# kenahm/se3-icp

Measured on AMD Instinct MI355X. Metric: ICP iterations/sec + pairs/sec, ~120k-pt KITTI clouds, 1/2/4/8 GPU, higher is better.
Workload: dtype f32 sweep + f64 certify/solve

## Files before the change

include/se3icp.h:

```cpp
#ifndef SE3ICP_H
#define SE3ICP_H

#include <stdint.h>

#ifdef __cplusplus
extern "C" {
#endif

#define SE3ICP_ABI_VERSION 4

typedef enum se3icp_status {
    SE3ICP_OK = 0,
    SE3ICP_ERR_INVALID_ARG = -1,
    SE3ICP_ERR_INVALID_METHOD = -2,
    SE3ICP_ERR_EMPTY_CLOUD = -3,
    SE3ICP_ERR_K_TOO_LARGE = -4,
    SE3ICP_ERR_NO_DEVICE = -5,
    SE3ICP_ERR_HIP = -6,
    SE3ICP_ERR_NONFINITE = -7,
    SE3ICP_ERR_OUT_OF_MEMORY = -8,
    SE3ICP_ERR_INTERNAL = -9
} se3icp_status;

typedef enum se3icp_method {
    SE3ICP_PT2PT = 0,
    SE3ICP_PT2PL = 1,
    SE3ICP_GICP = 2,
    SE3ICP_SE3_PT2PT = 3,
    SE3ICP_SE3_PT2PL = 4,
    SE3ICP_SE3_GICP = 5,
    SE3ICP_SE3_GICP_WITH_CF = 6,
    SE3ICP_SE3_PURE_PT2PT = 7,
    SE3ICP_SE3_PURE_PT2PL = 8,
    SE3ICP_SE3_PURE_GICP = 9,
    SE3ICP_NUM_METHODS = 10
} se3icp_method;

typedef struct se3icp_params {
    int32_t max_num_iterations;
    int32_t max_num_se3_iterations;
    int32_t number_of_nn_for_LRF;
    int32_t _reserved;
    double mse;
    double mse_switch_error;
    double estimated_overlap;
    double alpha_rot;
    double beta_transl;
    double scale_preprocessing;
} se3icp_params;

typedef struct se3icp_result {
    double T[16];
    int32_t num_iterations;
    int32_t num_pure_se3_iterations;
    int32_t status;
    int32_t num_rechecked;
    double scaling_factor;
    double time_setup_ms;
    double time_loop_ms;
    double time_se3_correspondence_search_ms;
    double time_before_pure_icp_ms;
} se3icp_result;

int se3icp_abi_version(void);
const char* se3icp_status_string(int status);
int se3icp_method_from_name(const char* name);
const char* se3icp_method_name(int method);
void se3icp_default_params(se3icp_params* p);
int se3icp_device_count(void);

typedef struct se3icp_registration se3icp_registration;

se3icp_registration* se3icp_registration_new(void);
void se3icp_registration_free(se3icp_registration* r);
int se3icp_set_source_cloud(se3icp_registration* r, const double* xyz, int64_t n);
int se3icp_set_target_cloud(se3icp_registration* r, const double* xyz, int64_t n);
se3icp_params* se3icp_params_of(se3icp_registration* r);
int se3icp_run_icp(se3icp_registration* r, const char* variant);
int se3icp_run_se3_icp(se3icp_registration* r, const char* variant);
int se3icp_run_se3_icp_with_cf(se3icp_registration* r);
int se3icp_run_se3_pure(se3icp_registration* r, const char* variant);
int se3icp_get_result(const se3icp_registration* r, se3icp_result* out);

int se3icp_register_batch(int device, int32_t n_pairs, const double* const* src_xyz, const int64_t* n_src,
                          const double* const* tgt_xyz, const int64_t* n_tgt, int method,
                          const se3icp_params* params, se3icp_result* results);

int se3icp_register_batch_device(int device, int32_t n_pairs, const double* d_src_xyz, const int64_t* src_off,
                                 const double* d_tgt_xyz, const int64_t* tgt_off, int method,
                                 const se3icp_params* params, se3icp_result* results, void* hip_stream);

int se3icp_register_sweep(int device, int32_t n_pairs, const double* const* src_xyz, const int64_t* n_src,
                          const double* const* tgt_xyz, const int64_t* n_tgt, int method, int32_t n_variants,
                          const se3icp_params* variants, int32_t max_group, se3icp_result* results);
int se3icp_register_sweep_device(int device, int32_t n_pairs, const double* d_src_xyz, const int64_t* src_off,
                                 const double* d_tgt_xyz, const int64_t* tgt_off, int method, int32_t n_variants,
                                 const se3icp_params* variants, int32_t max_group, se3icp_result* results,
                                 void* hip_stream);

int se3icp_register_graph(int device, int32_t n_clouds, const double* const* xyz, const int64_t* n_pts,
                          int32_t n_pairs, const int32_t* src_cloud, const int32_t* tgt_cloud, int method,
                          const se3icp_params* params, int32_t sharing, se3icp_result* results);
int se3icp_register_graph_device(int device, int32_t n_clouds, const double* d_xyz, const int64_t* off,
                                 int32_t n_pairs, const int32_t* src_cloud, const int32_t* tgt_cloud, int method,
                                 const se3icp_params* params, int32_t sharing, se3icp_result* results,
                                 void* hip_stream);
struct se3icp_report_options;
struct se3icp_report;
int se3icp_register_graph_report(int device, int32_t n_clouds, const double* const* xyz, const int64_t* n_pts,
                                 int32_t n_pairs, const int32_t* src_cloud, const int32_t* tgt_cloud, int method,
                                 const se3icp_params* params, int32_t sharing, se3icp_result* results,
                                 const struct se3icp_report_options* opts, struct se3icp_report* reports);
int se3icp_register_graph_report_device(int device, int32_t n_clouds, const double* d_xyz, const int64_t* off,
                                        int32_t n_pairs, const int32_t* src_cloud, const int32_t* tgt_cloud,
                                        int method, const se3icp_params* params, int32_t sharing,
                                        se3icp_result* results, void* hip_stream,
                                        const struct se3icp_report_options* opts, struct se3icp_report* reports);
#define SE3ICP_GRAPH_STATS_N 9
int se3icp_last_graph_stats(int device, int64_t* out, int n);

int se3icp_set_batch_sharing(int device, int level);

int se3icp_set_lrf_seeding(int device, int mode);
#define SE3ICP_SEED_STATS_N 4
int se3icp_last_seed_stats(int device, int64_t* out, int n);

int se3icp_set_tree_sharing(int device, int mode);
#define SE3ICP_TREE_STATS_N 4
int se3icp_last_tree_stats(int device, int64_t* out, int n);

typedef enum se3icp_stop_reason {
    SE3ICP_STOP_CONVERGED = 0,
    SE3ICP_STOP_MAX_ITERATIONS = 1,
    SE3ICP_STOP_MAX_SE3_ITERATIONS = 2,
    SE3ICP_STOP_RUNAWAY = 3
} se3icp_stop_reason;

typedef struct se3icp_report_options {
    double max_correspondence_distance;
    int32_t* corr_idx;
    double* corr_dist;
    int32_t outputs_on_device;
    int32_t _reserved;
} se3icp_report_options;

typedef struct se3icp_report {
    double fitness;
    double inlier_rmse;
    double information[36];
    double final_mse;
    double final_mse_change;
    int64_t n_inliers;
    int32_t switched;
    int32_t stop_reason;
} se3icp_report;

int se3icp_report_version(void);

int se3icp_register_batch_report(int device, int32_t n_pairs, const double* const* src_xyz, const int64_t* n_src,
                                 const double* const* tgt_xyz, const int64_t* n_tgt, int method,
                                 const se3icp_params* params, se3icp_result* results,
                                 const se3icp_report_options* opts, se3icp_report* reports);
int se3icp_register_batch_report_device(int device, int32_t n_pairs, const double* d_src_xyz, const int64_t* src_off,
                                        const double* d_tgt_xyz, const int64_t* tgt_off, int method,
                                        const se3icp_params* params, se3icp_result* results, void* hip_stream,
                                        const se3icp_report_options* opts, se3icp_report* reports);
int se3icp_register_sweep_report(int device, int32_t n_pairs, const double* const* src_xyz, const int64_t* n_src,
                                 const double* const* tgt_xyz, const int64_t* n_tgt, int method, int32_t n_variants,
                                 const se3icp_params* variants, int32_t max_group, se3icp_result* results,
                                 const se3icp_report_options* opts, se3icp_report* reports);
int se3icp_register_sweep_report_device(int device, int32_t n_pairs, const double* d_src_xyz, const int64_t* src_off,
                                        const double* d_tgt_xyz, const int64_t* tgt_off, int method,
                                        int32_t n_variants, const se3icp_params* variants, int32_t max_group,
                                        se3icp_result* results, void* hip_stream,
                                        const se3icp_report_options* opts, se3icp_report* reports);
int se3icp_request_report(se3icp_registration* r, const se3icp_report_options* opts);
int se3icp_get_report(const se3icp_registration* r, se3icp_report* out);

int se3icp_init_version(void);
int se3icp_register_graph_init(int device, int32_t n_clouds, const double* const* xyz, const int64_t* n_pts,
                               int32_t n_pairs, const int32_t* src_cloud, const int32_t* tgt_cloud,
                               const double* T_init , int method,
                               const se3icp_params* params, int32_t sharing, se3icp_result* results,
                               const se3icp_report_options* opts, se3icp_report* reports);
int se3icp_register_graph_init_device(int device, int32_t n_clouds, const double* d_xyz, const int64_t* off,
                                      int32_t n_pairs, const int32_t* src_cloud, const int32_t* tgt_cloud,
                                      const double* T_init , int method,
                                      const se3icp_params* params, int32_t sharing, se3icp_result* results,
                                      void* hip_stream, const se3icp_report_options* opts, se3icp_report* reports);
int se3icp_set_initial_transform(se3icp_registration* r, const double* T);
int se3icp_set_pose_seeding(int device, int mode);
#define SE3ICP_INIT_STATS_N 3
int se3icp_last_init_stats(int device, int64_t* out, int n);
int se3icp_transform_points(const double* T, const double* xyz, int64_t n, double* out);
int se3icp_transform_device(int device, int32_t n_clouds, const double* d_xyz, const int64_t* off, const double* T,
                            double* d_out, void* hip_stream);

int se3icp_register(int device, const double* src_xyz, int64_t n_src, const double* tgt_xyz, int64_t n_tgt,
                    int method, const se3icp_params* params, se3icp_result* result);


int se3icp_toldi_frames(int device, const double* xyz, int64_t n, int k, double* frames);
int se3icp_knn_self(int device, const double* xyz, int64_t n, int k, int32_t* idx);
int se3icp_estimate_normals(int device, const double* xyz, int64_t n, int k, double* normals);
int se3icp_nn(int device, const double* query, int64_t nq, const double* data, int64_t nd, int dim,
              int32_t* idx, double* d2, int32_t* num_rechecked);

int64_t se3icp_synthetic_pairs(int device, const double* base, int64_t n, int32_t n_cases, const double* T,
                               double ratio, double noise_var, uint64_t seed, double* src_out, double* tgt_out,
                               int outputs_on_device);

#define SE3ICP_GEN_ARGS_LTR 1
int64_t se3icp_synthetic_reference(const double* cloud, int64_t n, int32_t n_cases, double ratio, double noise_var,
                                   double t_range, double r_range, int32_t flags, double* src_out, double* tgt_out,
                                   double* T_out);
int64_t se3icp_synthetic_reference_device(int device, const double* cloud, int64_t n, int32_t n_cases, double ratio,
                                          double noise_var, double t_range, double r_range, int32_t flags,
                                          double* src_out, double* tgt_out, double* T_out, int outputs_on_device);
int64_t se3icp_random_downsample(const double* xyz, int64_t n, double ratio, uint32_t seed, double* out);

int se3icp_voxel_version(void);
int se3icp_voxel_downsample_device(int device, int32_t n_clouds, const double* d_xyz, const int64_t* off,
                                   const double* voxel_size, double* d_out, int64_t* out_off, int32_t* d_count,
                                   int32_t* d_first, void* hip_stream);
int64_t se3icp_voxel_downsample(int device, const double* xyz, int64_t n, double voxel_size, double* out,
                                int32_t* count, int32_t* first);

int se3icp_set_profiling(int device, int on);
int se3icp_last_kernel_times(int device, double* out);
#define SE3ICP_KERNEL_TIMES_N 26
int se3icp_last_kernel_times_n(int device, double* out, int n);

typedef struct se3icp_trace {
    int32_t pair;
    int32_t max_iters;
    int32_t* corr_idx;
    float* corr_dist;
    uint64_t* trim_key;
    double* T;
    double* mse;
    int32_t* phase;
    int32_t iters_recorded;
    int32_t _reserved;
} se3icp_trace;
int se3icp_set_trace(int device, se3icp_trace* trace);

int se3icp_set_lrf_exact(int device, int exact_only);

int se3icp_set_nn_events(int device, int on);

#ifdef __cplusplus
}
#endif
#endif
```

se3-icp_amd/csrc/capi.cpp:

```cpp
#include <hip/hip_runtime.h>

#include <cmath>
#include <cstdio>
#include <cstring>
#include <iostream>
#include <mutex>
#include <string>
#include <vector>

#include "engine.hpp"
#include "graph.hpp"
#include "pose.hpp"
#include "se3icp.h"

using se3icp::Engine;
using se3icp::engine_for;
using se3icp::graph_check;
using se3icp::GS_COUNT;

namespace {

const char* kMethodNames[SE3ICP_NUM_METHODS] = {"pt2pt",     "pt2pl",     "gicp",
                                                "se3_pt2pt", "se3_pt2pl", "se3_gicp",
                                                "se3_gicp_with_cf", "se3_pure_pt2pt", "se3_pure_pt2pl",
// ... 270 lines not shown
static int cloud_ranges(int32_t n_clouds, const double* d_xyz, const int64_t* off, std::vector<const double*>& x,
                        std::vector<int64_t>& n) {
    if (n_clouds <= 0 || !d_xyz || !off) return SE3ICP_ERR_INVALID_ARG;
    x.resize(n_clouds);
    n.resize(n_clouds);
    for (int32_t c = 0; c < n_clouds; ++c) {
        x[c] = d_xyz + 3 * off[c];
        n[c] = off[c + 1] - off[c];
    }
    return SE3ICP_OK;
}

int se3icp_register_graph(int device, int32_t n_clouds, const double* const* xyz, const int64_t* n_pts,
                          int32_t n_pairs, const int32_t* src_cloud, const int32_t* tgt_cloud, int method,
                          const se3icp_params* params, int32_t sharing, se3icp_result* results) {
    if (!xyz) return SE3ICP_ERR_INVALID_ARG;
    return graph_run(device, n_clouds, xyz, n_pts, false, n_pairs, src_cloud, tgt_cloud, method, params, sharing, results,
                     nullptr, false, nullptr, nullptr);
}

int se3icp_register_graph_device(int device, int32_t n_clouds, const double* d_xyz, const int64_t* off,
                                 int32_t n_pairs, const int32_t* src_cloud, const int32_t* tgt_cloud, int method,
                                 const se3icp_params* params, int32_t sharing, se3icp_result* results,
                                 void* hip_stream) {
    std::vector<const double*> x;
    std::vector<int64_t> n;
    const int rc = cloud_ranges(n_clouds, d_xyz, off, x, n);
    if (rc) return rc;
    return graph_run(device, n_clouds, x.data(), n.data(), true, n_pairs, src_cloud, tgt_cloud, method, params, sharing,
                     results, hip_stream, false, nullptr, nullptr);
}

int se3icp_register_graph_report(int device, int32_t n_clouds, const double* const* xyz, const int64_t* n_pts,
                                 int32_t n_pairs, const int32_t* src_cloud, const int32_t* tgt_cloud, int method,
                                 const se3icp_params* params, int32_t sharing, se3icp_result* results,
                                 const se3icp_report_options* opts, se3icp_report* reports) {
    if (!xyz) return SE3ICP_ERR_INVALID_ARG;
    return graph_run(device, n_clouds, xyz, n_pts, false, n_pairs, src_cloud, tgt_cloud, method, params, sharing, results,
                     nullptr, true, opts, reports);
}

int se3icp_register_graph_report_device(int device, int32_t n_clouds, const double* d_xyz, const int64_t* off,
                                        int32_t n_pairs, const int32_t* src_cloud, const int32_t* tgt_cloud, int method,
                                        const se3icp_params* params, int32_t sharing, se3icp_result* results,
                                        void* hip_stream, const se3icp_report_options* opts, se3icp_report* reports) {
    std::vector<const double*> x;
    std::vector<int64_t> n;
    const int rc = cloud_ranges(n_clouds, d_xyz, off, x, n);
    if (rc) return rc;
    return graph_run(device, n_clouds, x.data(), n.data(), true, n_pairs, src_cloud, tgt_cloud, method, params, sharing,
                     results, hip_stream, true, opts, reports);
}

int se3icp_init_version(void) { return 1; }

int se3icp_register_graph_init(int device, int32_t n_clouds, const double* const* xyz, const int64_t* n_pts,
                               int32_t n_pairs, const int32_t* src_cloud, const int32_t* tgt_cloud, const double* T_init,
                               int method, const se3icp_params* params, int32_t sharing, se3icp_result* results,
                               const se3icp_report_options* opts, se3icp_report* reports) {
    if (!xyz || (opts == nullptr) != (reports == nullptr)) return SE3ICP_ERR_INVALID_ARG;
    return graph_run(device, n_clouds, xyz, n_pts, false, n_pairs, src_cloud, tgt_cloud, method, params, sharing, results,
                     nullptr, opts != nullptr, opts, reports, T_init);
}

int se3icp_register_graph_init_device(int device, int32_t n_clouds, const double* d_xyz, const int64_t* off,
                                      int32_t n_pairs, const int32_t* src_cloud, const int32_t* tgt_cloud,
                                      const double* T_init, int method, const se3icp_params* params, int32_t sharing,
                                      se3icp_result* results, void* hip_stream, const se3icp_report_options* opts,
                                      se3icp_report* reports) {
    if ((opts == nullptr) != (reports == nullptr)) return SE3ICP_ERR_INVALID_ARG;
    std::vector<const double*> x;
    std::vector<int64_t> n;
    const int rc = cloud_ranges(n_clouds, d_xyz, off, x, n);
    if (rc) return rc;
    return graph_run(device, n_clouds, x.data(), n.data(), true, n_pairs, src_cloud, tgt_cloud, method, params, sharing,
                     results, hip_stream, opts != nullptr, opts, reports, T_init);
}

int se3icp_set_pose_seeding(int device, int mode) {
    if (mode < se3icp::kPoseSeedingMin || mode > se3icp::kPoseSeedingMax) return SE3ICP_ERR_INVALID_ARG;
    Engine* e = usable_engine(device);
    if (!e) return SE3ICP_ERR_NO_DEVICE;
    std::lock_guard<std::mutex> lk(e->mutex());
    e->set_pose_seeding(mode);
    return SE3ICP_OK;
}

int se3icp_last_init_stats(int device, int64_t* out, int n) {
    if (!out || n < se3icp::IS_COUNT) return SE3ICP_ERR_INVALID_ARG;
    Engine* e = usable_engine(device);
    if (!e) return SE3ICP_ERR_NO_DEVICE;
    std::lock_guard<std::mutex> lk(e->mutex());
    for (int k = 0; k < se3icp::IS_COUNT; ++k) out[k] = e->init_stats()[k];
    return SE3ICP_OK;
}

int se3icp_transform_points(const double* T, const double* xyz, int64_t n, double* out) {
    if (!T || n < 0 || (n > 0 && (!xyz || !out)) || !se3icp::pose_is_valid(T)) return SE3ICP_ERR_INVALID_ARG;
    for (int64_t i = 0; i < n; ++i) se3icp::apply_pose(T, xyz + 3 * i, out + 3 * i);
    return SE3ICP_OK;
}

int se3icp_transform_device(int device, int32_t n_clouds, const double* d_xyz, const int64_t* off, const double* T,
                            double* d_out, void* hip_stream) {
    if (n_clouds <= 0 || n_clouds > 65535 || !d_xyz || !off || !T || !d_out) return SE3ICP_ERR_INVALID_ARG;
    for (int32_t c = 0; c < n_clouds; ++c)
        if (off[c + 1] < off[c] || !se3icp::pose_is_valid(T + 16 * (size_t)c)) return SE3ICP_ERR_INVALID_ARG;
    if (d_out != d_xyz) {
        const double* lo = d_xyz + 3 * off[0];
        const double* hi = d_xyz + 3 * off[n_clouds];
        const double* olo = d_out + 3 * off[0];
        const double* ohi = d_out + 3 * off[n_clouds];
        if (olo < hi && lo < ohi) return SE3ICP_ERR_INVALID_ARG;
    }
    Engine* e = usable_engine(device);
    if (!e) return SE3ICP_ERR_NO_DEVICE;
    std::lock_guard<std::mutex> lk(e->mutex());
    return e->transform_device(n_clouds, d_xyz, off, T, d_out, (hipStream_t)hip_stream);
}

int se3icp_last_graph_stats(int device, int64_t* out, int n) {
    if (!out || n < GS_COUNT) return SE3ICP_ERR_INVALID_ARG;
    Engine* e = usable_engine(device);
    if (!e) return SE3ICP_ERR_NO_DEVICE;
    std::lock_guard<std::mutex> lk(e->mutex());
    for (int k = 0; k < GS_COUNT; ++k) out[k] = e->graph_stats()[k];
    return SE3ICP_OK;
}

int se3icp_set_batch_sharing(int device, int level) {
    if (level < se3icp::kBatchSharingMin || level > se3icp::kBatchSharingMax) return SE3ICP_ERR_INVALID_ARG;
    Engine* e = usable_engine(device);
    if (!e) return SE3ICP_ERR_NO_DEVICE;
    std::lock_guard<std::mutex> lk(e->mutex());
    e->set_batch_sharing(level);
    return SE3ICP_OK;
}

int se3icp_set_lrf_seeding(int device, int mode) {
    if (mode < se3icp::kLrfSeedingMin || mode > se3icp::kLrfSeedingMax) return SE3ICP_ERR_INVALID_ARG;
    Engine* e = usable_engine(device);
    if (!e) return SE3ICP_ERR_NO_DEVICE;
    std::lock_guard<std::mutex> lk(e->mutex());
    e->set_lrf_seeding(mode);
    return SE3ICP_OK;
}

int se3icp_last_seed_stats(int device, int64_t* out, int n) {
    if (!out || n < 4) return SE3ICP_ERR_INVALID_ARG;
    Engine* e = usable_engine(device);
    if (!e) return SE3ICP_ERR_NO_DEVICE;
    std::lock_guard<std::mutex> lk(e->mutex());
    for (int k = 0; k < 4; ++k) out[k] = e->seed_stats()[k];
    return SE3ICP_OK;
}

int se3icp_set_tree_sharing(int device, int mode) {
    if (mode < se3icp::kTreeSharingMin || mode > se3icp::kTreeSharingMax) return SE3ICP_ERR_INVALID_ARG;
    Engine* e = usable_engine(device);
    if (!e) return SE3ICP_ERR_NO_DEVICE;
    std::lock_guard<std::mutex> lk(e->mutex());
    e->set_tree_sharing(mode);
    return SE3ICP_OK;
}

int se3icp_last_tree_stats(int device, int64_t* out, int n) {
    if (!out || n < 4) return SE3ICP_ERR_INVALID_ARG;
    Engine* e = usable_engine(device);
    if (!e) return SE3ICP_ERR_NO_DEVICE;
    std::lock_guard<std::mutex> lk(e->mutex());
    for (int k = 0; k < 4; ++k) out[k] = e->tree_stats()[k];
    return SE3ICP_OK;
}

int se3icp_register(int device, const double* src_xyz, int64_t n_src, const double* tgt_xyz, int64_t n_tgt,
                    int method, const se3icp_params* params, se3icp_result* result) {
    return se3icp_register_batch(device, 1, &src_xyz, &n_src, &tgt_xyz, &n_tgt, method, params, result);
}

se3icp_registration* se3icp_registration_new(void) {
    auto* r = new (std::nothrow) se3icp_registration;
    if (!r) return nullptr;
    se3icp_default_params(&r->prm);
    std::memset(&r->res, 0, sizeof(r->res));
    for (int i = 0; i < 4; ++i) r->res.T[i * 4 + i] = 1.0;
    r->res.num_pure_se3_iterations = -1;
    return r;
}

void se3icp_registration_free(se3icp_registration* r) { delete r; }

int se3icp_set_source_cloud(se3icp_registration* r, const double* xyz, int64_t n) {
    if (!r || (n > 0 && !xyz) || n < 0) return SE3ICP_ERR_INVALID_ARG;
    r->src.insert(r->src.end(), xyz, xyz + 3 * n);
    return 0;
}

int se3icp_set_target_cloud(se3icp_registration* r, const double* xyz, int64_t n) {
    if (!r || (n > 0 && !xyz) || n < 0) return SE3ICP_ERR_INVALID_ARG;
    r->tgt.insert(r->tgt.end(), xyz, xyz + 3 * n);
    return 0;
}

se3icp_params* se3icp_params_of(se3icp_registration* r) { return r ? &r->prm : nullptr; }

static int run_object(se3icp_registration* r, int method) {
    const int64_t ns = (int64_t)r->src.size() / 3, nt = (int64_t)r->tgt.size() / 3;
    if (ns <= 0 || nt <= 0) return SE3ICP_ERR_EMPTY_CLOUD;
    const double* s = r->src.data();
    const double* t = r->tgt.data();
    se3icp_result res;
    se3icp_report rep;
    if (r->have_init) {
        const double* const xyz[2] = {s, t};
        const int64_t n[2] = {ns, nt};
        const int32_t es = 0, et = 1;
        const int rc = se3icp_register_graph_init(current_device(), 2, xyz, n, 1, &es, &et, r->init, method, &r->prm, 0,
                                                  &res, r->want_report ? &r->ropts : nullptr,
                                                  r->want_report ? &rep : nullptr);
        if (rc == SE3ICP_OK || rc == SE3ICP_ERR_NONFINITE) {
            r->res = res;
            r->have_report = r->want_report;
            if (r->want_report) r->rep = rep;
        }
        return rc;
    }
    int rc = r->want_report ? se3icp_register_batch_report(current_device(), 1, &s, &ns, &t, &nt, method, &r->prm, &res,
                                                           &r->ropts, &rep)
                            : se3icp_register_batch(current_device(), 1, &s, &ns, &t, &nt, method, &r->prm, &res);
    if (rc == SE3ICP_OK || rc == SE3ICP_ERR_NONFINITE) {
        r->res = res;
        r->have_report = r->want_report;
        if (r->want_report) r->rep = rep;
    }
    return rc;
}

int se3icp_run_icp(se3icp_registration* r, const char* variant) {
    if (!r) return SE3ICP_ERR_INVALID_ARG;
    const int v = variant_index(variant);
    if (v < 0) {
        std::cerr << "Invalid ICP variant name. Valid names are pt2pt, pt2pl and gicp.\n";
        return SE3ICP_ERR_INVALID_METHOD;
    }
    return run_object(r, SE3ICP_PT2PT + v);
}

int se3icp_run_se3_icp(se3icp_registration* r, const char* variant) {
    if (!r) return SE3ICP_ERR_INVALID_ARG;
    const int v = variant_index(variant);
    if (v < 0) {
        std::cerr << "Invalid variant name. Choose one of: pt2pt, pt2pl, gicp \n";
        std::cout << "Unknown optimization strategy for SE(3) \n";
        const int64_t ns = (int64_t)r->src.size() / 3, nt = (int64_t)r->tgt.size() / 3;
        if (ns <= 0 || nt <= 0) return SE3ICP_ERR_EMPTY_CLOUD;
        double cs[3] = {0, 0, 0}, ct[3] = {0, 0, 0};
        for (int64_t i = 0; i < ns; ++i)
            for (int a = 0; a < 3; ++a) cs[a] += r->src[3 * i + a];
        for (int64_t i = 0; i < nt; ++i)
            for (int a = 0; a < 3; ++a) ct[a] += r->tgt[3 * i + a];
        std::memset(r->res.T, 0, sizeof(r->res.T));
        for (int a = 0; a < 4; ++a) r->res.T[a * 4 + a] = 1.0;
        for (int a = 0; a < 3; ++a) r->res.T[a * 4 + 3] = ct[a] / (double)nt - cs[a] / (double)ns;
        r->res.num_iterations = 1;
        r->res.num_pure_se3_iterations = 1;
        r->res.status = SE3ICP_ERR_INVALID_METHOD;
        return SE3ICP_ERR_INVALID_METHOD;
    }
    return run_object(r, SE3ICP_SE3_PT2PT + v);
}

int se3icp_run_se3_icp_with_cf(se3icp_registration* r) {
    if (!r) return SE3ICP_ERR_INVALID_ARG;
    const int rc = run_object(r, SE3ICP_SE3_GICP_WITH_CF);
    if (rc == SE3ICP_OK || rc == SE3ICP_ERR_NONFINITE)
        std::cout << "### scaling factor = " << r->res.scaling_factor << std::endl;
    return rc;
}

int se3icp_run_se3_pure(se3icp_registration* r, const char* variant) {
    if (!r) return SE3ICP_ERR_INVALID_ARG;
    const int v = variant_index(variant);
    if (v < 0) {
        std::cerr << "Invalid variant name. Choose one of: pt2pt, pt2pl, gicp \n";
        return SE3ICP_ERR_INVALID_METHOD;
    }
    const int rc = run_object(r, SE3ICP_SE3_PURE_PT2PT + v);
    if (rc == SE3ICP_OK || rc == SE3ICP_ERR_NONFINITE) std::cout << "pure se3 finished" << std::endl;
    return rc;
}

int se3icp_set_initial_transform(se3icp_registration* r, const double* T) {
    if (!r) return SE3ICP_ERR_INVALID_ARG;
    if (!T) {
        r->have_init = false;
        return 0;
    }
    if (!se3icp::pose_is_valid(T)) return SE3ICP_ERR_INVALID_ARG;
    std::memcpy(r->init, T, sizeof(r->init));
    r->have_init = true;
    return 0;
}

int se3icp_get_result(const se3icp_registration* r, se3icp_result* out) {
    if (!r || !out) return SE3ICP_ERR_INVALID_ARG;
    *out = r->res;
// ... 157 lines not shown
```

se3-icp_amd/csrc/common.hpp:

```cpp
#pragma once
#include <stdint.h>

namespace se3icp {

constexpr int kSmallK = 128;
constexpr int kBlock = 256;
constexpr int kRedVals = 28;
constexpr int kStatCols = 17;
constexpr int kStatUseSe3 = 15, kStatUseR3 = 16;
constexpr int kSeedStatCol = 14;
constexpr int kHist = 256;
constexpr int kTrimList = 4096;
constexpr int kTrimBlocks = 32;
constexpr int kChunkQ = 1024;

enum Phase : int32_t { PHASE_IDLE = 0, PHASE_SE3 = 1, PHASE_R3 = 2 };
enum Estimator : int32_t { EST_PT2PT = 0, EST_PT2PL = 1, EST_GICP = 2 };

struct CloudDev {
    int32_t off;
    int32_t n;
};

struct PairDev {
    double T[12];
    double f32_center[3];
    int32_t src, tgt;
    int32_t phase;
    int32_t est;
    int32_t cf;
    int32_t trim;
    int32_t nkeep;
    int32_t iter;
    float tgt_norm12;
    float tgt_norm3;
    int32_t phase_start;
    int32_t _pad;
};

constexpr int kRedThreads = 256;
constexpr int kRedPer = 1;
constexpr int kRedQ = kRedThreads * kRedPer;

struct BlockWork {
    int32_t pair;
    int32_t q0, q1;
    int32_t s_off, t_off;
    int32_t _pad[3];
};

}
```

se3-icp_amd/csrc/engine.cpp:

```cpp
#include "engine.hpp"

#include <algorithm>
#include <chrono>
#include <cmath>
#include <cstdio>
#include <cstdlib>
#include <cstring>
#include <map>
#include <memory>

#include "graph.hpp"
#include "pose.hpp"
#include "report.hpp"
#include "sweep.hpp"
#include "tree.hpp"

namespace se3icp {

namespace {

#define HIPCHK(x)                                                                                   \
    do {                                                                                            \
        hipError_t e_ = (x);                                                                        \
        if (e_ != hipSuccess) {                                                                     \
// ... 302 lines not shown
        if (tab->host.reserve(words) || !ensure<int32_t>(tab->dev, words)) return SE3ICP_ERR_OUT_OF_MEMORY;
        int32_t* h = tab->host;
        size_t at = (size_t)nclouds_;
        for (int c = 0; c < nclouds_; ++c) h[c] = (*role)[c];
        for (int c = 0; c < nclouds_; ++c)
            if ((*role)[c] == kTreeBuilds) h[at++] = c;
        for (int c = 0; c < nclouds_; ++c)
            if ((*role)[c] >= 0) h[at++] = c;
        HIPCHK(hipMemcpyAsync(tab->dev.p, h, sizeof(int32_t) * words, hipMemcpyHostToDevice, s));
        t.role = (const int32_t*)tab->dev.p;
        t.list = t.role + nclouds_;
        t.nbuild = nbuild;
        t.nadopt = nadopt;
    }
    tree_stats_[D == 12 ? 2 : 0] += nbuild;
    tree_stats_[D == 12 ? 3 : 1] += nadopt;
    if (build_trees(t, d_sort_tmp_.p, d_sort_tmp_.bytes, (uint32_t*)d_keys0_.p, (int32_t*)d_vals1_.p, s) != 0)
        return SE3ICP_ERR_HIP;
    return 0;
}

int Engine::upload_clouds(const std::vector<CloudReq>& clouds, bool on_device, hipStream_t s) {
    nclouds_ = (int)clouds.size();
    h_clouds_.assign(nclouds_, CloudDev{});
    h_setup_.resize(nclouds_);
    h_chunks_.clear();
    h_inptr_.assign(nclouds_, nullptr);
    int64_t off = 0;
    int max_n = 1;
    for (int c = 0; c < nclouds_; ++c) {
        h_clouds_[c].off = (int32_t)off;
        h_clouds_[c].n = (int32_t)clouds[c].n;
        h_setup_[c] = clouds[c].st;
        max_n = std::max<int>(max_n, (int)clouds[c].n);
        for (int64_t p0 = 0; p0 < clouds[c].n; p0 += kChunk) h_chunks_.push_back(ChunkWork{c, (int32_t)p0});
        off += clouds[c].n;
    }
    tree_L_ = tree_depth_for(max_n);
    double* d_in = (double*)d_in_.p;
    for (int c = 0; c < nclouds_; ++c) {
        if (on_device) {
            h_inptr_[c] = clouds[c].in;
        } else {
            double* dst = d_in + 3 * (size_t)h_clouds_[c].off;
            HIPCHK(hipMemcpyAsync(dst, clouds[c].in, sizeof(double) * 3 * clouds[c].n, hipMemcpyHostToDevice, s));
            h_inptr_[c] = dst;
        }
    }
    const int nch = (int)h_chunks_.size();
    if (!ensure<CloudDev>(d_clouds_, nclouds_) || !ensure<CloudSetup>(d_setup_, nclouds_) ||
        !ensure<ChunkWork>(d_chunks_, nch) || !ensure<const double*>(d_inptr_, nclouds_) ||
        !ensure<double>(d_partial_, (size_t)nch * 9) || !ensure<double>(d_centers_, 3 * (size_t)nclouds_))
        return SE3ICP_ERR_OUT_OF_MEMORY;
    if (h_partial_.reserve((size_t)nch * 9 + 8)) return SE3ICP_ERR_OUT_OF_MEMORY;
    HIPCHK(hipMemcpyAsync(d_clouds_.p, h_clouds_.data(), sizeof(CloudDev) * nclouds_, hipMemcpyHostToDevice, s));
    HIPCHK(hipMemcpyAsync(d_setup_.p, h_setup_.data(), sizeof(CloudSetup) * nclouds_, hipMemcpyHostToDevice, s));
    HIPCHK(hipMemcpyAsync(d_chunks_.p, h_chunks_.data(), sizeof(ChunkWork) * nch, hipMemcpyHostToDevice, s));
    HIPCHK(hipMemcpyAsync(d_inptr_.p, h_inptr_.data(), sizeof(double*) * nclouds_, hipMemcpyHostToDevice, s));
    return 0;
}

int Engine::host_centroids(hipStream_t s, std::vector<double>* cen) {
    const int nch = (int)h_chunks_.size();
    HIPCHK(hipMemcpyAsync(h_partial_, d_partial_.p, sizeof(double) * 9 * nch, hipMemcpyDeviceToHost, s));
    SYNC_STREAM(s);
    std::vector<double> sum(3 * (size_t)nclouds_, 0.0);
    for (int k = 0; k < nch; ++k)
        for (int a = 0; a < 3; ++a) sum[3 * (size_t)h_chunks_[k].cloud + a] += h_partial_[9 * (size_t)k + a];
    cen->assign(3 * (size_t)nclouds_, 0.0);
    for (int c = 0; c < nclouds_; ++c)
        for (int a = 0; a < 3; ++a)
            (*cen)[3 * (size_t)c + a] = h_clouds_[c].n > 0 ? sum[3 * (size_t)c + a] / (double)h_clouds_[c].n : 0.0;
    return 0;
}

int Engine::setup_clouds(const std::vector<CloudReq>& clouds, bool on_device, bool pairs, bool normalize,
                         double scale_pre, hipStream_t s) {
    int rc = upload_clouds(clouds, on_device, s);
    if (rc) return rc;
    const int nch = (int)h_chunks_.size();
    View v = view();

    launch_ingest(v, (const ChunkWork*)d_chunks_.p, nch, (double*)d_partial_.p, s);
    HIPCHK(hipGetLastError());
    if (normalize) {
        if (!ensure<double>(d_scales_, std::max(1, nclouds_ / 2))) return SE3ICP_ERR_OUT_OF_MEMORY;
        launch_pair_centers(v, (const ChunkWork*)d_chunks_.p, nch, (const double*)d_partial_.p, (double*)d_centers_.p,
                            s);
        launch_radius(v, (const ChunkWork*)d_chunks_.p, nch, (const double*)d_centers_.p, (double*)d_partial_.p, s);
        launch_pair_scales(v, (const ChunkWork*)d_chunks_.p, nch, (const double*)d_partial_.p,
                           (const double*)d_centers_.p, scale_pre, (double*)d_scales_.p, s);
        HIPCHK(hipGetLastError());
        for (int c = 0; c < nclouds_; ++c)
            for (int a = 0; a < 3; ++a) h_setup_[c].f32_center[a] = 0.0;
    } else {
        std::vector<double> cen;
        rc = host_centroids(s, &cen);
        if (rc) return rc;
        for (int c = 0; c < nclouds_; ++c) {
            const int cc = pairs ? (c | 1) : c;
            for (int a = 0; a < 3; ++a) {
                h_setup_[c].norm_center[a] = 0.0;
                h_setup_[c].f32_center[a] = cen[3 * cc + a];
            }
            h_setup_[c].norm_scale = 1.0;
        }
        HIPCHK(hipMemcpyAsync(d_setup_.p, h_setup_.data(), sizeof(CloudSetup) * nclouds_, hipMemcpyHostToDevice, s));
    }

    launch_normalize(v, (const ChunkWork*)d_chunks_.p, nch, (double*)d_partial_.p, s);
    HIPCHK(hipGetLastError());

    rc = build_tree(3, (const float*)d_xyz32_.p, s, (const double*)d_xyz64_.p);
    if (rc) return rc;
    rc = setup_knn(s);
    if (rc) return rc;
    HIPCHK(hipGetLastError());
    return 0;
}

int Engine::setup_knn(hipStream_t s) {
    const View v = view();
    bool any_knn = false;
    for (int c = 0; c < nclouds_; ++c) any_knn |= h_setup_[c].k_knn > 0;
    if (any_knn) {
        HIPCHK(hipMemsetAsync(d_stats_.p, 0, sizeof(unsigned long long) * kStatCols * kStatSlots, s));
        HIPCHK(hipEventRecord(ev_[6], s));
        int kw_big = 0, n_big = 0;
        for (int c = 0; c < nclouds_; ++c) {
            const int kw = std::min<int>(h_setup_[c].k_knn, h_clouds_[c].n);
            if (kw > kSmallK || lrf_exact_only_ == 2) {
                kw_big = std::max(kw_big, kw);
                n_big += h_clouds_[c].n;
            }
        }
        int big_cap = 0, big_blocks = 0;
        if (n_big > 0) {
            big_cap = knn_big_cap(kw_big);
            big_blocks = knn_big_blocks(big_cap, n_big);
            if (!ensure<double>(d_big_d_, (size_t)big_blocks * big_cap) || !ensure<int32_t>(d_big_i_, (size_t)big_blocks * big_cap))
                return SE3ICP_ERR_OUT_OF_MEMORY;
        }
        auto big = [&](const int32_t* qlist, const int32_t* qcount, int k_min) {
            if (n_big > 0)
                launch_knn_big(v, knn_list_ ? 1 : 0, k_min, qlist, qcount, big_blocks, (double*)d_big_d_.p,
                               (int32_t*)d_big_i_.p, big_cap, s);
        };
        if (lrf_exact_only_ == 2) {
            big(nullptr, nullptr, 0);
        } else if (knn_list_ || lrf_exact_only_ == 1) {
            launch_lrf(v, knn_list_ ? 1 : 0, s);
            big(nullptr, nullptr, kSmallK);
        } else {
            const bool seeding = seed_on_;
            const int nt = nclouds_ + 1;
            std::vector<int32_t> wb(2 * (size_t)nt, 0);
            for (int c = 0; c < nclouds_; ++c) {
                const int waves = h_setup_[c].k_knn > 0 ? (h_clouds_[c].n + 7) / 8 : 0;
                const bool sd = seeding && seed_ref_[c].load >= 0;
                wb[c + 1] = wb[c] + (sd ? 0 : waves);
                wb[nt + c + 1] = wb[nt + c] + (sd ? waves : 0);
            }
            const int nw = wb[nclouds_], nw_sd = wb[nt + nclouds_];
            if (!ensure<int32_t>(d_lrf_fb_, (size_t)8 * (nw + nw_sd) + 64) || !ensure<int32_t>(d_lrf_fbn_, 2 + 2 * (size_t)nt))
                return SE3ICP_ERR_OUT_OF_MEMORY;
            int32_t* d_wb = (int32_t*)d_lrf_fbn_.p + 2;
            int32_t* fb = (int32_t*)d_lrf_fb_.p;
            int32_t* fbn = (int32_t*)d_lrf_fbn_.p;
            HIPCHK(hipMemsetAsync(fbn, 0, 2 * sizeof(int32_t), s));
            HIPCHK(hipMemcpyAsync(d_wb, wb.data(), sizeof(int32_t) * 2 * nt, hipMemcpyHostToDevice, s));
            if (seeding) {
                if (!ensure<float>(d_seed_, (size_t)seed_floats_) || !ensure<SeedRef>(d_seed_ref_, nclouds_))
                    return SE3ICP_ERR_OUT_OF_MEMORY;
                HIPCHK(hipMemsetAsync(d_seed_.p, 0xff, sizeof(float) * (size_t)seed_floats_, s));
                HIPCHK(hipMemcpyAsync(d_seed_ref_.p, seed_ref_.data(), sizeof(SeedRef) * nclouds_, hipMemcpyHostToDevice, s));
                launch_lrf8(v, d_wb, 0, nw, fb, fbn, s, (const SeedRef*)d_seed_ref_.p, (float*)d_seed_.p, false, lrf_seeding_);
                launch_lrf8(v, d_wb + nt, 0, nw_sd, fb, fbn, s, (const SeedRef*)d_seed_ref_.p, (float*)d_seed_.p, true,
                            lrf_seeding_);
            } else {
                launch_lrf8(v, d_wb, 0, nw, fb, fbn, s);
            }
            launch_lrf_list(v, fb, fbn, s);
            big(fb, fbn, kSmallK);
        }
        HIPCHK(hipEventRecord(ev_[7], s));
        HIPCHK(hipGetLastError());
        if (h_lrf_stats_.reserve((size_t)kStatCols * kStatSlots)) return SE3ICP_ERR_OUT_OF_MEMORY;
        HIPCHK(hipMemcpyAsync(h_lrf_stats_, d_stats_.p, sizeof(unsigned long long) * kStatCols * kStatSlots,
                              hipMemcpyDeviceToHost, s));
        lrf_stats_pending_ = true;
    }
    return 0;
}

int Engine::read_lrf_stats() {
    if (!lrf_stats_pending_) return 0;
    lrf_stats_pending_ = false;
    double sum[kStatCols] = {};
    for (int i = 0; i < kStatSlots; ++i)
        for (int k = 0; k < kStatCols; ++k) sum[k] += (double)h_lrf_stats_[kStatCols * i + k];
    float ms = 0;
    HIPCHK(hipEventElapsedTime(&ms, ev_[6], ev_[7]));
    ktimes_.lrf_ms = ms;
    ktimes_.lrf_queries = sum[0];
    ktimes_.lrf_leaves = sum[1];
    ktimes_.lrf_merges = sum[2];
    ktimes_.lrf_box_tests = sum[3];
    ktimes_.lrf_candidates = sum[4];
    ktimes_.lrf_fallback = sum[6];
    for (int k = 0; k < 3; ++k) {
        unsigned long long q = 0;
        for (int i = 0; i < kStatSlots; ++i) q += h_lrf_stats_[kStatCols * i + kSeedStatCol + k];
        seed_stats_[1 + k] = (int64_t)q;
    }
#ifdef SE3ICP_PROF
    tree_prof_report();
    std::fprintf(stderr, "[prof] k_lrf cycles/query: knn|scan %.0f sort|tighten %.0f sums|final+sums %.0f finish %.0f "
                 "(queries %.0f, wave cycles summed over the kernel's waves)\n",
                 sum[8] / sum[0], sum[9] / sum[0], sum[10] / sum[0], sum[11] / sum[0], sum[0]);
    std::fprintf(stderr, "[prof] k_lrf8 per query: tightenings %.3f (overflow %.3f, final %.3f), leaf scans %.3f\n",
                 sum[2] / sum[0], sum[3] / sum[0], sum[7] / sum[0], sum[1] / sum[0]);
    {
        unsigned long long f = 0;
        for (int i = 0; i < kStatSlots; ++i) f += h_lrf_stats_[kStatCols * i + 5];
        std::fprintf(stderr, "[prof] k_lrf8 hand-overs: waves with the leaf table full %llu, no room %llu, > 128 at the end %llu; "
                     "queries with f32-equal f64-distinct ranks %llu\n",
                     f & 0xffff, (f >> 16) & 0xffff, (f >> 32) & 0xffff, f >> 48);
    }
#endif
    return 0;
}

int Engine::sync_stream(hipStream_t s) {
    HIPCHK(hipEventRecord(ev_[15], s));
    HIPCHK(spin_wait(ev_[15]));
    return read_lrf_stats();
}

int Engine::setup_chunks(int npairs, hipStream_t s) {
    chunk_level_ = std::max(0, tree_L_ - 4);
    nchunks_ = npairs << chunk_level_;
    if (!ensure<int32_t>(d_qlist_, (size_t)nchunks_ * kChunkQ) || !ensure<int32_t>(d_qcount_, (size_t)nchunks_ * (kChunkQ / 64)) ||
        !ensure<double>(d_hist_, (size_t)kHist * npairs * 12) || !ensure<uint32_t>(d_gcost_, (size_t)nchunks_ * 16) ||
        !ensure<int32_t>(d_cls_, nn_cls_words(nchunks_)))
        return SE3ICP_ERR_OUT_OF_MEMORY;
    if (h_hist_.reserve((size_t)npairs * 12)) return SE3ICP_ERR_OUT_OF_MEMORY;
    HIPCHK(hipMemsetAsync(d_cert_.p, 0xff, sizeof(NNCert) * ld_, s));
    HIPCHK(hipMemsetAsync(d_gcost_.p, 0, sizeof(uint32_t) * nchunks_ * 16, s));
    HIPCHK(hipMemsetAsync(d_cls_.p, 0, sizeof(int32_t) * 2 * 8 * 16, s));
    return 0;
}

int Engine::open_call(int args, int64_t nslots, int rest, hipStream_t user_stream, Call* c) {
    if (!ok_) return SE3ICP_ERR_NO_DEVICE;
    se3icp_trace* tr = c->tr = trace_;
    trace_ = nullptr;
    pose_raw_.clear();
    pose_rigid_.clear();
    if (args) return args;
    if (tr && (tr->pair < 0 || (int64_t)tr->pair >= nslots || tr->max_iters < 0)) return SE3ICP_ERR_INVALID_ARG;
    if (tr) tr->iters_recorded = 0;
    if (rest) return rest;
    HIPCHK(hipSetDevice(dev_));
    c->s = user_stream ? user_stream : stream_;
    ktimes_ = KernelTimes{};
    for (int64_t& x : seed_stats_) x = 0;
    for (int64_t& x : tree_stats_) x = 0;
    tree_donor_.clear();
    HIPCHK(hipEventRecord(ev_[12], c->s));
    return 0;
}

int Engine::run_pairs(const MethodPlan& mp, int npairs, const int64_t* ns, const int64_t* nt,
                      const se3icp_params* vprm, int pairs_per_variant, bool sweep, const Call& c, se3icp_result* out,
                      const se3icp_report_options* ropts, se3icp_report* reports) {
    hipStream_t s = c.s;
    int rc = 0;
    const bool adopt12 = (int)tree_donor_.size() == nclouds_;
    if (mp.se3)
        rc = build_tree(12, (const float*)d_fr32_.p, s, (const double*)d_fr64_.p, adopt12 ? &tree_donor_ : nullptr,
                        &tree_tab_12_);
    if (rc) return rc;
    rc = prepare_pairs(npairs, ns, nt, s);
    if (rc) return rc;
    rc = setup_chunks(npairs, s);
    if (rc) return rc;
    HIPCHK(hipMemsetAsync(d_corr_idx_.p, 0xff, sizeof(int32_t) * ld_, s));
    HIPCHK(hipMemsetAsync(d_stats_.p, 0, sizeof(unsigned long long) * kStatCols * kStatSlots, s));
    for (double& t : trace_prev_) t = 0;
    HIPCHK(hipEventRecord(ev_[13], s));
    const ReportReq rq{ropts, reports};
    return run_loop(npairs, ns, mp.kind, mp.est, vprm, pairs_per_variant, sweep, c.tr, out, s,
                    (ropts && reports) ? &rq : nullptr);
}

int Engine::register_batch(int npairs, const double* const* src, const int64_t* ns, const double* const* tgt,
                           const int64_t* nt, bool on_device, int method, const se3icp_params& prm,
                           se3icp_result* out, hipStream_t user_stream, const se3icp_report_options* ropts,
                           se3icp_report* reports) {
    const int args = (npairs <= 0 || !src || !tgt || !ns || !nt || !out) ? SE3ICP_ERR_INVALID_ARG : 0;
    MethodPlan mp{};
    const int rest = args ? 0 : plan_pairs(method, prm.number_of_nn_for_LRF, npairs, src, ns, tgt, nt, &mp);
    Call call;
    int rc = open_call(args, npairs, rest, user_stream, &call);
    if (rc) return rc;

    npairs_ = npairs;
    int64_t ntot = 0;
    for (int p = 0; p < npairs; ++p) ntot += ns[p] + nt[p];
    rc = alloc_points(ntot, mp.kmax);
    if (rc) return rc;
    std::vector<CloudReq> clouds(2 * npairs);
    for (int p = 0; p < npairs; ++p)
        for (int side = 0; side < 2; ++side)
            clouds[2 * p + side] = CloudReq{side == 0 ? src[p] : tgt[p], side == 0 ? ns[p] : nt[p],
                                            cloud_setup(mp, side, prm.alpha_rot, prm.beta_transl, true)};
    bool look = false;
    if (on_device && batch_sharing_ != 1) {
        std::vector<int64_t> n(clouds.size());
        for (size_t u = 0; u < clouds.size(); ++u) n[u] = clouds[u].n;
        look = clouds.size() <= kShareMaxSlots && share_any_equal_n((int32_t)n.size(), n.data());
        for (int64_t& g : graph_stats_) g = 0;
        graph_stats_[GS_CLOUDS] = graph_stats_[GS_USES] = graph_stats_[GS_CLASSES] = (int64_t)clouds.size();
        for (const CloudReq& c : clouds) graph_stats_[GS_FULL] += c.st.k_knn > 0;
    }
    rc = look ? setup_pairs_shared(clouds, mp, prm.scale_preprocessing, call.s)
              : setup_clouds(clouds, on_device, true, mp.se3, prm.scale_preprocessing, call.s);
    if (rc) return rc;
    return run_pairs(mp, npairs, ns, nt, &prm, npairs, false, call, out, ropts, reports);
}

int Engine::setup_pairs_shared(const std::vector<CloudReq>& clouds, const MethodPlan& mp, double scale_pre,
                               hipStream_t s) {
    const int U = (int)clouds.size();
    const bool se3 = mp.se3;
    int rc = upload_clouds(clouds, true, s);
    if (rc) return rc;
    const int nch = (int)h_chunks_.size();
    if (!ensure<uint64_t>(d_share_hash_, U) || !ensure<SharePair>(d_share_pairs_, U) ||
        !ensure<int32_t>(d_share_same_, U) || h_share_hash_.reserve(U) || h_share_same_.reserve(U) ||
        h_share_setup_.reserve(U))
        return SE3ICP_ERR_OUT_OF_MEMORY;
    View v = view();
    HIPCHK(hipMemsetAsync(d_share_hash_.p, 0, sizeof(uint64_t) * U, s));
    launch_share_hash(v, (unsigned long long*)d_share_hash_.p, s);
    HIPCHK(hipMemcpyAsync(h_share_hash_, d_share_hash_.p, sizeof(uint64_t) * U, hipMemcpyDeviceToHost, s));
    launch_ingest(v, (const ChunkWork*)d_chunks_.p, nch, (double*)d_partial_.p, s);
    HIPCHK(hipGetLastError());
    if (se3) {
        if (!ensure<double>(d_scales_, std::max(1, nclouds_ / 2))) return SE3ICP_ERR_OUT_OF_MEMORY;
        launch_pair_centers(v, (const ChunkWork*)d_chunks_.p, nch, (const double*)d_partial_.p, (double*)d_centers_.p,
                            s);
        launch_radius(v, (const ChunkWork*)d_chunks_.p, nch, (const double*)d_centers_.p, (double*)d_partial_.p, s);
        launch_pair_scales(v, (const ChunkWork*)d_chunks_.p, nch, (const double*)d_partial_.p,
                           (const double*)d_centers_.p, scale_pre, (double*)d_scales_.p, s);
        HIPCHK(hipGetLastError());
        HIPCHK(hipMemcpyAsync(h_share_setup_, d_setup_.p, sizeof(CloudSetup) * U, hipMemcpyDeviceToHost, s));
        HIPCHK(hipEventRecord(ev_[10], s));
        for (int c = 0; c < nclouds_; ++c)
            for (int a = 0; a < 3; ++a) h_setup_[c].f32_center[a] = 0.0;
    } else {
        std::vector<double> cen;
        rc = host_centroids(s, &cen);
        if (rc) return rc;
        for (int c = 0; c < nclouds_; ++c) {
            for (int a = 0; a < 3; ++a) {
                h_setup_[c].norm_center[a] = 0.0;
                h_setup_[c].f32_center[a] = cen[3 * (c | 1) + a];
            }
            h_setup_[c].norm_scale = 1.0;
        }
        HIPCHK(hipMemcpyAsync(d_setup_.p, h_setup_.data(), sizeof(CloudSetup) * nclouds_, hipMemcpyHostToDevice, s));
    }
    launch_normalize(v, (const ChunkWork*)d_chunks_.p, nch, (double*)d_partial_.p, s);
    HIPCHK(hipGetLastError());
    const bool adopt = tree_sharing_ != 1;
    if (!adopt) {
        rc = build_tree(3, (const float*)d_xyz32_.p, s, (const double*)d_xyz64_.p);
        if (rc) return rc;
    }
    if (se3) HIPCHK(spin_wait(ev_[10]));

    std::vector<int64_t> n(U);
    for (int u = 0; u < U; ++u) n[u] = clouds[u].n;
    std::vector<int32_t> first, cloud;
    const int ncand = share_candidates(U, n.data(), h_share_hash_, &first);
    int nc = U;
    if (ncand > 0) {
        share_pairs_.clear();
        for (int u = 0; u < U; ++u)
            if (first[u] != u) share_pairs_.push_back(SharePair{u, first[u]});
        HIPCHK(hipMemcpyAsync(d_share_pairs_.p, share_pairs_.data(), sizeof(SharePair) * ncand, hipMemcpyHostToDevice, s));
        HIPCHK(hipMemsetAsync(d_share_same_.p, 1, sizeof(int32_t) * U, s));
        launch_share_compare(v, (const SharePair*)d_share_pairs_.p, ncand, (int32_t*)d_share_same_.p, s);
        HIPCHK(hipGetLastError());
        HIPCHK(hipMemcpyAsync(h_share_same_, d_share_same_.p, sizeof(int32_t) * U, hipMemcpyDeviceToHost, s));
        HIPCHK(hipEventRecord(ev_[11], s));
        std::vector<int32_t> role(U);
        if (adopt) {
            for (int u = 0; u < U; ++u) role[u] = first[u] == u ? kTreeBuilds : kTreeAbsent;
            rc = build_tree(3, (const float*)d_xyz32_.p, s, (const double*)d_xyz64_.p, &role, &tree_tab_a_);
            if (rc) return rc;
        }
        HIPCHK(spin_wait(ev_[11]));
        nc = share_clouds(U, first.data(), h_share_same_, &cloud);
        if (adopt) {
            std::vector<int32_t> donor;
            const int nad = graph_plan_trees(U, cloud.data(), n.data(), true, &donor);
            for (int u = 0; u < U; ++u) role[u] = first[u] == u ? kTreeAbsent : donor[u];
            rc = build_tree(3, (const float*)d_xyz32_.p, s, (const double*)d_xyz64_.p, &role, &tree_tab_b_);
            if (rc) return rc;
            if (nad > 0) tree_donor_ = donor;
        }
    } else if (adopt) {
        rc = build_tree(3, (const float*)d_xyz32_.p, s, (const double*)d_xyz64_.p);
        if (rc) return rc;
    }
    if (nc == U) return setup_knn(s);

    const CloudSetup* dev_table = se3 ? (const CloudSetup*)h_share_setup_ : h_setup_.data();
    share_setup_.assign(dev_table, dev_table + U);
    std::vector<GraphUse> use(U);
    for (int u = 0; u < U; ++u) {
        const CloudSetup& st = share_setup_[u];
        use[u].cloud = cloud[u];
        use[u].k_nrm = st.k_nrm;
        use[u].norm_scale = st.norm_scale;
        for (int a = 0; a < 3; ++a) {
            use[u].norm_center[a] = st.norm_center[a];
            use[u].f32_center[a] = st.f32_center[a];
        }
    }
    GraphPlan plan;
    graph_plan_uses(U, use.data(), se3, true, &plan);
    graph_stats_[GS_CLOUDS] = nc;
    graph_stats_[GS_CLASSES] = (int64_t)plan.classes.size();
    return select_by_class(plan, share_setup_, mp, s);
}

int Engine::select_by_class(const GraphPlan& plan, const std::vector<CloudSetup>& batch, const MethodPlan& mp,
                            hipStream_t s) {
    const int U = (int)batch.size(), K = (int)plan.classes.size();
    const bool se3 = mp.se3;
    std::vector<int32_t> home(K, -1);
    for (int u = 0; u < U; ++u)
        if (home[plan.use_class[u]] < 0) home[plan.use_class[u]] = u;
    sel_batch_ = batch;
    sel_run_ = sel_batch_;
    sel_chunks_.clear();
    sel_seg_.assign(U, GraphSeg{});
    graph_stats_[GS_FULL] = 0;
    for (int u = 0; u < U; ++u) {
        const int k = plan.use_class[u];
        const GraphClass& gc = plan.classes[k];
        CloudSetup& st = sel_run_[u];
        const bool is_home = home[k] == u;
        st.k_lrf = is_home ? mp.k_lrf : 0;
        st.k_nrm = (is_home && gc.nrm_from == k) ? gc.k_nrm : 0;
        st.k_knn = std::max(st.k_lrf, st.k_nrm);
        graph_stats_[GS_FULL] += st.k_knn > 0;
        const int hf = home[k], hn = home[gc.nrm_from];
        sel_seg_[u] = GraphSeg{h_clouds_[hf].off, hf, h_clouds_[hn].off, (hf != u && se3) ? 1 : 0};
        if ((hf != u && se3) || hn != u)
            for (int64_t p0 = 0; p0 < h_clouds_[u].n; p0 += kChunk) sel_chunks_.push_back(ChunkWork{u, (int32_t)p0});
    }
    const int nchS = (int)sel_chunks_.size();
    if (!ensure<ChunkWork>(g_chunks_, nchS) || !ensure<GraphSeg>(g_seg_, U)) return SE3ICP_ERR_OUT_OF_MEMORY;
    seed_ref_.clear();
    seed_floats_ = 0;
    if (lrf_seeding_ != 1 && lrf_exact_only_ == 0 && !knn_list_) {
        std::vector<int32_t> kk(K);
        std::vector<int64_t> nn(K);
        for (int k = 0; k < K; ++k) {
            kk[k] = sel_run_[home[k]].k_knn;
            nn[k] = h_clouds_[home[k]].n;
        }
        std::vector<SeedClass> sc;
        int32_t cross = 0;
        const int seeded = pose_raw_.empty()
                               ? graph_plan_seeds(plan, kk.data(), nn.data(), &sc)
                               : graph_plan_seeds_posed(plan, kk.data(), nn.data(), pose_raw_.data(), pose_rigid_.data(),
                                                        pose_seeding_ == 0, &sc, &cross);
        int64_t total = 0;
        for (int k = 0; k < K; ++k)
            if (sc[k].from >= 0) total += nn[k];
        if (seeded > 0 && total <= INT32_MAX) {
            seed_ref_.assign(U, SeedRef{-1, -1, 1.0});
            for (int k = 0; k < K; ++k) {
                if (sc[k].from < 0) continue;
                SeedRef& src = seed_ref_[home[sc[k].from]];
                if (src.store < 0) {
                    src.store = (int32_t)seed_floats_;
                    seed_floats_ += nn[k];
                }
                seed_ref_[home[k]].load = src.store;
                seed_ref_[home[k]].rho2 = sc[k].rho2;
            }
            seed_stats_[0] = seeded;
            init_stats_[IS_CROSS_SEEDED] = cross;
            seed_on_ = true;
        }
    }
    h_setup_ = sel_run_;
    HIPCHK(hipMemcpyAsync(d_setup_.p, sel_run_.data(), sizeof(CloudSetup) * U, hipMemcpyHostToDevice, s));
    const int rc = setup_knn(s);
    seed_on_ = false;
    if (rc) return rc;
    HIPCHK(hipGetLastError());
    h_setup_ = sel_batch_;
    HIPCHK(hipMemcpyAsync(d_setup_.p, sel_batch_.data(), sizeof(CloudSetup) * U, hipMemcpyHostToDevice, s));
    if (nchS > 0) {
        HIPCHK(hipMemcpyAsync(g_chunks_.p, sel_chunks_.data(), sizeof(ChunkWork) * nchS, hipMemcpyHostToDevice, s));
        HIPCHK(hipMemcpyAsync(g_seg_.p, sel_seg_.data(), sizeof(GraphSeg) * U, hipMemcpyHostToDevice, s));
        launch_graph_share(view(), (const ChunkWork*)g_chunks_.p, nchS, (const GraphSeg*)g_seg_.p, s);
        HIPCHK(hipGetLastError());
    }
    return 0;
}

int Engine::prepare_pairs(int npairs, const int64_t* ns, const int64_t* nt, hipStream_t s) {
    int64_t soff = 0;
    h_work_.clear();
    h_wb_.assign(npairs, 0);
    h_wn_.assign(npairs, 0);
    for (int p = 0; p < npairs; ++p) {
        h_wb_[p] = (int32_t)h_work_.size();
        for (int64_t q0 = 0; q0 < ns[p]; q0 += kRedQ)
            h_work_.push_back(BlockWork{p, (int32_t)q0, (int32_t)std::min<int64_t>(q0 + kRedQ, ns[p]), (int32_t)soff,
                                        (int32_t)(soff + ns[p]), {0, 0, 0}});
        soff += ns[p] + nt[p];
        h_wn_[p] = (int32_t)h_work_.size() - h_wb_[p];
    }
    nwork_ = (int)h_work_.size();
    if (!ensure<PairDev>(d_pairs_, npairs) || !ensure<BlockWork>(d_work_, nwork_) || !ensure<int32_t>(d_wb_, npairs) ||
        !ensure<int32_t>(d_wn_, npairs) || !ensure<uint64_t>(d_trim_key_, 2 * (size_t)npairs) ||
        !ensure<unsigned long long>(d_trim_cand_, (size_t)npairs * kTrimList) || !ensure<unsigned>(d_trim_ctr_, 4 * (size_t)npairs) ||
        !ensure<unsigned>(d_trim_hist_, 4096 * (size_t)npairs) ||
        !ensure<double>(d_red_partial_, (size_t)nwork_ * kRedVals) || !ensure<double>(d_red_out_, (size_t)npairs * kRedVals) ||
        !ensure<int32_t>(d_rechecked_, npairs))
        return SE3ICP_ERR_OUT_OF_MEMORY;
    if (h_pairs_.reserve(npairs) || h_red_.reserve((size_t)npairs * kRedVals) || h_rechecked_.reserve(npairs))
        return SE3ICP_ERR_OUT_OF_MEMORY;
    HIPCHK(hipMemcpyAsync(d_work_.p, h_work_.data(), sizeof(BlockWork) * nwork_, hipMemcpyHostToDevice, s));
    HIPCHK(hipMemcpyAsync(d_wb_.p, h_wb_.data(), sizeof(int32_t) * npairs, hipMemcpyHostToDevice, s));
    HIPCHK(hipMemcpyAsync(d_wn_.p, h_wn_.data(), sizeof(int32_t) * npairs, hipMemcpyHostToDevice, s));
    HIPCHK(hipMemsetAsync(d_rechecked_.p, 0, sizeof(int32_t) * npairs, s));
    return 0;
}

int Engine::run_loop(int npairs, const int64_t* ns, int kind, int est, const se3icp_params* vprm,
                     int pairs_per_variant, bool sweep, se3icp_trace* tr, se3icp_result* out, hipStream_t s,
                     const ReportReq* rq) {
    const MethodInfo mi{(Kind)kind, est};
    const bool se3 = mi.kind != KIND_ICP;
    int rc = 0;

    if (!ensure<PairState>(d_state_, npairs) || h_state_.reserve(npairs))
        return SE3ICP_ERR_OUT_OF_MEMORY;
    if (h_phase_cap_ < (size_t)npairs * kLoopRing) {
        if (h_phase_) (void)hipHostFree(h_phase_);
        h_phase_ = nullptr;
        h_phase_cap_ = 0;
        const size_t want = std::max<size_t>((size_t)npairs * kLoopRing, 64);
        if (hipHostMalloc((void**)&h_phase_, want * sizeof(int32_t), hipHostMallocMapped | hipHostMallocCoherent) !=
                hipSuccess ||
            hipHostGetDevicePointer((void**)&d_phase_, h_phase_, 0) != hipSuccess)
            return SE3ICP_ERR_OUT_OF_MEMORY;
        h_phase_cap_ = want;
    }
    int se3_limit = 0;
    for (int k = 0; k * pairs_per_variant < npairs; ++k) {
        const int m = vprm[k].max_num_se3_iterations;
        se3_limit = (m < 1 || se3_limit < 0) ? -1 : std::max(se3_limit, m);
    }
    int n_se3 = 0, n_r3 = 0;
    bool any_trim = false;
    for (int p = 0; p < npairs; ++p) {
        const se3icp_params& prm = vprm[p / pairs_per_variant];
        const float ratio = std::min(1.0f, std::max(0.0f, (float)prm.estimated_overlap));
        PairState& S = h_state_[p];
        std::memset(&S, 0, sizeof(S));
        S.T = M4::eye();
        S.mse_prev = S.mse_cur = S.rel = 1e7;
        S.sf = 1.0;
        S.mse = prm.mse;
        S.mse_switch = prm.mse_switch_error;
        S.kind = mi.kind;
        S.max_iter = prm.max_num_iterations;
        S.max_se3 = prm.max_num_se3_iterations;
        S.phase = PHASE_IDLE;
        S.phase_start = 1;
        const unsigned nv = (unsigned)std::floor(ratio * (float)ns[p]);
        const bool trim = (int64_t)nv < ns[p];
        S.K = trim ? (double)nv : (double)ns[p];
        PairDev& P = h_pairs_[p];
        std::memset(&P, 0, sizeof(P));
        P.src = 2 * p;
        P.tgt = 2 * p + 1;
        P.est = mi.est;
        P.cf = mi.kind == KIND_CF;
        P.trim = trim;
        P.nkeep = (int)nv;
        for (int a = 0; a < 3; ++a) P.f32_center[a] = h_setup_[2 * p].f32_center[a];
        pair_open_iteration(S, P);
        std::memcpy(h_hist_ + 12 * (size_t)p, P.T, sizeof(P.T));
        n_se3 += P.phase == PHASE_SE3;
        n_r3 += P.phase == PHASE_R3;
        any_trim |= trim;
    }
    HIPCHK(hipMemcpyAsync(d_pairs_.p, h_pairs_, sizeof(PairDev) * npairs, hipMemcpyHostToDevice, s));
    HIPCHK(hipMemcpyAsync(d_state_.p, h_state_, sizeof(PairState) * npairs, hipMemcpyHostToDevice, s));
    HIPCHK(hipMemcpyAsync((double*)d_hist_.p + (size_t)(1 % kHist) * npairs * 12, h_hist_, sizeof(double) * 12 * npairs,
                          hipMemcpyHostToDevice, s));
    HIPCHK(hipMemsetAsync(d_flag_count_.p, 0, 3 * sizeof(int32_t), s));
    launch_pair_norms(view(), 2 << t3_.L, se3 ? 2 << t12_.L : 0, se3 ? (const double*)d_scales_.p : nullptr,
                      (double*)((char*)d_state_.p + offsetof(PairState, sf)), (int)(sizeof(PairState) / sizeof(double)),
                      s);
    HIPCHK(hipGetLastError());
    HIPCHK(hipMemsetAsync((uint64_t*)d_trim_key_.p + npairs, 0, sizeof(uint64_t) * npairs, s));
    HIPCHK(hipMemsetAsync(d_trim_ctr_.p, 0, sizeof(unsigned) * 4 * npairs, s));
    launch_geo_rows(view(), s);
    HIPCHK(hipMemsetAsync(d_trim_hist_.p, 0, sizeof(unsigned) * 4096 * npairs, s));
    View v = view();
    double nn_ms = 0;
    const int lag = (nn_trace_ || tr) ? 0 : 1;
    int trace_phase = tr ? h_pairs_[tr->pair].phase : 0;
    auto enqueue = [&](int it) -> int {
        hipEvent_t* ev = &loop_ev_[(it % kLoopRing) * kLoopEv];
        for (int p = 0; p < npairs; ++p) h_phase_[(size_t)(it % kLoopRing) * npairs + p] = -1;
        const bool do_se3 =
            n_se3 > 0 && (se3_limit < 1 || it <= se3_limit);
        const bool do_r3 = n_r3 > 0 || (mi.kind != KIND_ICP && mi.kind != KIND_PURE && it >= 2);
        const bool detail = profile_ || nn_trace_;
        const bool t_se3 = detail || (do_se3 && nn_events_);
        if (detail) HIPCHK(hipEventRecord(ev[0], s));
        launch_nn_prep(v, (lag == 1 && it >= 2) ? d_phase_ + (size_t)((it - 1) % kLoopRing) * npairs : nullptr, s);
        if (t_se3) HIPCHK(hipEventRecord(ev[1], s));
        if (do_se3) launch_nn(v, 12, s);
        if (t_se3) HIPCHK(hipEventRecord(ev[2], s));
        if (do_r3) launch_nn(v, 3, s);
        if (detail) HIPCHK(hipEventRecord(ev[3], s));
        if (detail) HIPCHK(hipEventRecord(ev[4], s));
        if (any_trim) launch_trim(v, s);
        if (detail) HIPCHK(hipEventRecord(ev[5], s));
        launch_reduce(v, (const int32_t*)d_wb_.p, (const int32_t*)d_wn_.p, (PairState*)d_state_.p, (double*)d_hist_.p,
                      lag == 0 ? d_phase_ + (size_t)(it % kLoopRing) * npairs : nullptr, s);
        HIPCHK(hipGetLastError());
        if (detail) HIPCHK(hipEventRecord(ev[6], s));
        loop_detail_[it % kLoopRing] = detail;
        loop_flags_[it % kLoopRing] = (do_se3 ? 1 : 0) | (do_r3 ? 2 : 0) | (t_se3 ? 4 : 0);
        return 0;
    };
    auto finish = [&](int it, bool last) -> int {
        hipEvent_t* ev = &loop_ev_[(it % kLoopRing) * kLoopEv];
        if (loop_detail_[it % kLoopRing]) HIPCHK(spin_wait(ev[6]));
        if (last && lag == 1) {
            if (!loop_detail_[it % kLoopRing]) {
                HIPCHK(hipEventRecord(ev_[15], s));
                HIPCHK(spin_wait(ev_[15]));
// ... 959 lines not shown
```

se3-icp_amd/csrc/engine.hpp:

```cpp
#pragma once
#include <hip/hip_runtime.h>

#include <mutex>
#include <stdint.h>
#include <vector>

#include "graph.hpp"
#include "pairmath.hpp"
#include "pose.hpp"
#include "se3icp.h"
#include "view.hpp"
#include "voxel.hpp"

namespace se3icp {

void launch_voxel(const VoxelArgs& a, int max_chunks, int64_t n_points, int64_t n_slots, hipStream_t s);

struct DevBuf {
    void* p = nullptr;
    size_t bytes = 0;
    explicit DevBuf(std::vector<DevBuf*>& owner) { owner.push_back(this); }
};
struct PinnedMem {
    void* mem = nullptr;
    size_t cap = 0;
};
template <class T>
struct Pinned : PinnedMem {
    explicit Pinned(std::vector<PinnedMem*>& owner) { owner.push_back(this); }
    operator T*() const { return static_cast<T*>(mem); }
    int reserve(size_t count) {
        if (cap >= count && mem) return 0;
        if (mem) (void)hipHostFree(mem);
        mem = nullptr;
        cap = 0;
        const size_t want = count > 16 ? count : 16;
        if (hipHostMalloc(&mem, want * sizeof(T), hipHostMallocDefault) != hipSuccess) return SE3ICP_ERR_OUT_OF_MEMORY;
        cap = want;
        return 0;
    }
};

struct KernelTimes {
    double nn_se3_ms = 0, nn_r3_ms = 0, recheck_ms = 0, trim_ms = 0, reduce_ms = 0;
    double setup_ms = 0;
    int64_t nn_se3_launches = 0, nn_r3_launches = 0;
    double se3_dist_evals = 0, se3_box_tests = 0, r3_dist_evals = 0, r3_box_tests = 0;
    double se3_useful_evals = 0, r3_useful_evals = 0;
    double lrf_ms = 0, lrf_queries = 0, lrf_leaves = 0, lrf_merges = 0, lrf_box_tests = 0, lrf_candidates = 0;
    double lrf_fallback = 0;
    double nn_prep_ms = 0, se3_queries = 0, se3_searched = 0, r3_queries = 0, r3_searched = 0;
};

struct MethodPlan {
    Kind kind;
    int est;
    bool se3;
    int k_lrf, k_nrm_s, k_nrm_t, kmax;
};

class Engine {
  public:
    explicit Engine(int device);
    ~Engine();
    Engine(const Engine&) = delete;
    Engine& operator=(const Engine&) = delete;

    int device() const { return dev_; }
    std::mutex& mutex() { return mu_; }
    void set_profiling(bool on) { profile_ = on; }
    void set_trace(se3icp_trace* t) { trace_ = t; }
    void set_lrf_exact(int mode) { lrf_exact_only_ = mode; }
    void set_nn_events(bool on) { nn_events_ = on; }
    void set_batch_sharing(int level) { batch_sharing_ = level; }
    void set_lrf_seeding(int mode) { lrf_seeding_ = mode; }
    void set_tree_sharing(int mode) { tree_sharing_ = mode; }
    const KernelTimes& kernel_times() const { return ktimes_; }

    int register_batch(int npairs, const double* const* src, const int64_t* ns, const double* const* tgt,
                       const int64_t* nt, bool on_device, int method, const se3icp_params& prm,
                       se3icp_result* out, hipStream_t user_stream, const se3icp_report_options* ropts = nullptr,
                       se3icp_report* reports = nullptr);
    int register_sweep(int npairs, const double* const* src, const int64_t* ns, const double* const* tgt,
                       const int64_t* nt, bool on_device, int method, int nvariants, const se3icp_params* variants,
                       int max_group, se3icp_result* out, hipStream_t user_stream,
                       const se3icp_report_options* ropts = nullptr, se3icp_report* reports = nullptr);

    int register_graph(int nclouds, const double* const* xyz, const int64_t* npts, int npairs, const int32_t* src,
                       const int32_t* tgt, bool on_device, int method, const se3icp_params& prm, int sharing,
                       se3icp_result* out, hipStream_t user_stream, const se3icp_report_options* ropts = nullptr,
                       se3icp_report* reports = nullptr, const double* T_init = nullptr);
    const int64_t* init_stats() const { return init_stats_; }
    void set_pose_seeding(int mode) { pose_seeding_ = mode; }
    int transform_device(int nclouds, const double* d_xyz, const int64_t* off, const double* T, double* d_out,
                         hipStream_t user_stream);
    const int64_t* graph_stats() const { return graph_stats_; }
    const int64_t* seed_stats() const { return seed_stats_; }
    const int64_t* tree_stats() const { return tree_stats_; }

    int knn_self(const double* xyz, int64_t n, int k, int32_t* idx);
    int toldi_frames(const double* xyz, int64_t n, int k, double* frames);
    int estimate_normals(const double* xyz, int64_t n, int k, double* normals);
    int nn(const double* query, int64_t nq, const double* data, int64_t nd, int dim, int32_t* idx, double* d2,
           int32_t* num_rechecked);

    int voxel_downsample(int nclouds, const double* d_xyz, const int64_t* off, const double* vs, double* d_out,
                         int64_t* out_off, int32_t* d_count, int32_t* d_first, hipStream_t user_stream);
    int voxel_downsample_host(const double* xyz, int64_t n, double vs, double* out, int32_t* count, int32_t* first,
                              int64_t* n_out);

  private:
    struct CloudReq {
        const double* in = nullptr;
        int64_t n = 0;
        CloudSetup st{};
    };
    struct TreeBufs {
        DevBuf perm, pos, vec, vec64, vec64a, blo, bhi, lo, hi, scr, vecT;
        int L = 0;
        explicit TreeBufs(std::vector<DevBuf*>& o)
            : perm(o), pos(o), vec(o), vec64(o), vec64a(o), blo(o), bhi(o), lo(o), hi(o), scr(o), vecT(o) {}
    };
    int init();
    template <class T>
    T* ensure(DevBuf& b, size_t count);
    int alloc_points(int64_t ntot, int kmax, bool knn_list = false);
    struct TreeTab {
        Pinned<int32_t> host;
        DevBuf dev;
        TreeTab(std::vector<PinnedMem*>& p, std::vector<DevBuf*>& o) : host(p), dev(o) {}
    };
    int build_tree(int D, const float* vec, hipStream_t s, const double* vec64 = nullptr,
                   const std::vector<int32_t>* role = nullptr, TreeTab* tab = nullptr);
    struct Call {
        se3icp_trace* tr = nullptr;
        hipStream_t s = nullptr;
    };
    int open_call(int args, int64_t nslots, int rest, hipStream_t user_stream, Call* c);
    int upload_clouds(const std::vector<CloudReq>& clouds, bool on_device, hipStream_t s);
    int host_centroids(hipStream_t s, std::vector<double>* cen);
    int setup_clouds(const std::vector<CloudReq>& clouds, bool on_device, bool pairs, bool normalize, double scale_pre,
                     hipStream_t s);
    int setup_knn(hipStream_t s);
    int setup_pairs_shared(const std::vector<CloudReq>& clouds, const MethodPlan& mp, double scale_pre, hipStream_t s);
    int select_by_class(const GraphPlan& plan, const std::vector<CloudSetup>& batch, const MethodPlan& mp,
                        hipStream_t s);
    int setup_chunks(int npairs, hipStream_t s);
    int run_pairs(const MethodPlan& mp, int npairs, const int64_t* ns, const int64_t* nt,
                  const se3icp_params* vprm, int pairs_per_variant, bool sweep, const Call& c, se3icp_result* out,
                  const se3icp_report_options* ropts, se3icp_report* reports);
    int prepare_pairs(int npairs, const int64_t* ns, const int64_t* nt, hipStream_t s);
    struct ReportReq {
        const se3icp_report_options* opts;
        se3icp_report* out;
    };
    int run_loop(int npairs, const int64_t* ns, int kind, int est, const se3icp_params* vprm, int pairs_per_variant,
                 bool sweep, se3icp_trace* tr, se3icp_result* out, hipStream_t s, const ReportReq* rq = nullptr);
    int queue_report(int npairs, const int64_t* ns, const ReportReq& rq, hipStream_t s);
    int read_lrf_stats();
    int sync_stream(hipStream_t s);
    View view() const;

    int dev_;
    bool ok_ = false;
    bool profile_ = false;
    std::mutex mu_;
    hipStream_t stream_ = nullptr;
    KernelTimes ktimes_;

    int nclouds_ = 0, npairs_ = 0;
    int64_t ntot_ = 0;
    int ld_ = 0, kmax_ = 1, nwork_ = 0, tree_L_ = 0;
    int chunk_level_ = 0, nchunks_ = 0;
    bool knn_list_ = false;
    bool nn_trace_ = false;
    int lrf_exact_only_ = 0;
    bool nn_events_ = true;
    int batch_sharing_ = 0;
    int lrf_seeding_ = 0;
    int tree_sharing_ = 0;
    se3icp_trace* trace_ = nullptr;
    int record_trace(se3icp_trace* tr, int it, int& phase_of_it, hipStream_t s);
    double trace_prev_[kStatCols] = {};
    std::vector<CloudDev> h_clouds_;
    std::vector<CloudSetup> h_setup_;
    std::vector<BlockWork> h_work_;
    std::vector<int32_t> h_wb_, h_wn_;
    std::vector<ChunkWork> h_chunks_;
    std::vector<const double*> h_inptr_;

    std::vector<DevBuf*> bufs_;
    std::vector<PinnedMem*> pins_;
    DevBuf d_clouds_{bufs_}, d_setup_{bufs_}, d_pairs_{bufs_}, d_cloud_of_{bufs_}, d_inptr_{bufs_}, d_in_{bufs_},
        d_xyz64_{bufs_}, d_xyz32_{bufs_}, d_fr64_{bufs_}, d_fr32_{bufs_}, d_nrm64_{bufs_}, d_tgeo_{bufs_},
        d_conf64_{bufs_}, d_knn_{bufs_}, d_corr_idx_{bufs_}, d_corr_dist_{bufs_}, d_flag_count_{bufs_},
        d_gcost_{bufs_}, d_cls_{bufs_}, d_trim_key_{bufs_}, d_red_partial_{bufs_}, d_red_out_{bufs_}, d_work_{bufs_},
        d_wb_{bufs_}, d_wn_{bufs_}, d_chunks_{bufs_}, d_partial_{bufs_}, d_centers_{bufs_}, d_rechecked_{bufs_},
        d_keys0_{bufs_}, d_vals1_{bufs_}, d_sort_tmp_{bufs_}, d_stats_{bufs_}, d_qlist_{bufs_}, d_qcount_{bufs_},
        d_hist_{bufs_}, d_cert_{bufs_}, d_sqlist_{bufs_}, d_state_{bufs_}, d_trim_cand_{bufs_}, d_trim_ctr_{bufs_},
        d_scales_{bufs_}, d_trim_hist_{bufs_},
        d_lrf_fb_{bufs_}, d_lrf_fbn_{bufs_},
        d_big_d_{bufs_}, d_big_i_{bufs_},
        d_raw_{bufs_}, d_sweep_w_{bufs_},
        d_rep_partial_{bufs_}, d_rep_out_{bufs_}, d_rep_off_{bufs_}, d_rep_idx_{bufs_}, d_rep_dist_{bufs_};
    TreeBufs t3_{bufs_}, t12_{bufs_};
    DevBuf g_raw_xyz_{bufs_}, g_raw_conf_{bufs_}, g_seg_{bufs_}, g_chunks_{bufs_};
    DevBuf d_share_hash_{bufs_}, d_share_pairs_{bufs_}, d_share_same_{bufs_};
    Pinned<uint64_t> h_share_hash_{pins_};
    Pinned<int32_t> h_share_same_{pins_};
    Pinned<CloudSetup> h_share_setup_{pins_};
    std::vector<SharePair> share_pairs_;
    std::vector<CloudSetup> share_setup_;
    std::vector<CloudSetup> sel_batch_, sel_run_;
    std::vector<ChunkWork> sel_chunks_;
    std::vector<GraphSeg> sel_seg_;
    int64_t graph_stats_[9] = {};
    bool seed_on_ = false;
    std::vector<SeedRef> seed_ref_;
    int64_t seed_floats_ = 0;
    DevBuf d_seed_{bufs_}, d_seed_ref_{bufs_};
    int64_t seed_stats_[4] = {};
    std::vector<int32_t> tree_donor_;
    TreeTab tree_tab_a_{pins_, bufs_}, tree_tab_b_{pins_, bufs_}, tree_tab_12_{pins_, bufs_};
    int64_t tree_stats_[4] = {};
    std::vector<int32_t> pose_of_, pose_raw_, pose_rigid_;
    std::vector<double> pose_tab_;
    DevBuf d_pose_of_{bufs_}, d_pose_tab_{bufs_};
    int pose_seeding_ = 0;
    int64_t init_stats_[3] = {};
    Pinned<PoseCloud> h_tf_clouds_{pins_};
    Pinned<double> h_tf_poses_{pins_};
    DevBuf d_tf_clouds_{bufs_}, d_tf_poses_{bufs_};
    DevBuf v_clouds_{bufs_}, v_grids_{bufs_}, v_minmax_{bufs_}, v_sums_{bufs_}, v_table_{bufs_},
        v_vid_{bufs_}, v_members_{bufs_}, v_recs_{bufs_}, v_big_{bufs_}, v_flags_{bufs_},
        v_out_off_{bufs_}, v_in_{bufs_}, v_out_{bufs_}, v_oc_{bufs_}, v_of_{bufs_};
    Pinned<VoxelCloud> h_vclouds_{pins_};
    Pinned<long long> h_vout_{pins_};
    Pinned<int32_t> h_vflags_{pins_};
    Pinned<PairDev> h_pairs_{pins_};
    Pinned<double> h_red_{pins_}, h_partial_{pins_};
    Pinned<int32_t> h_rechecked_{pins_};
    Pinned<double> h_hist_{pins_};
    Pinned<double> h_rep_{pins_};
    std::vector<int64_t> h_rep_off_;
    Pinned<PairState> h_state_{pins_};
    int32_t* h_phase_ = nullptr;
    int32_t* d_phase_ = nullptr;
    size_t h_phase_cap_ = 0;
    Pinned<unsigned long long> h_lrf_stats_{pins_};
    Pinned<unsigned long long> h_loop_stats_{pins_};
    bool lrf_stats_pending_ = false;
    hipEvent_t ev_[16];
    static constexpr int kLoopRing = 4, kLoopEv = 7;
    hipEvent_t loop_ev_[kLoopRing * kLoopEv];
    int loop_flags_[kLoopRing] = {};
    bool loop_detail_[kLoopRing] = {};
};

Engine* engine_for(int device);

}
```

se3-icp_amd/csrc/graph.hpp:

```cpp
#pragma once
#include <hip/hip_runtime.h>
#include <stdint.h>

#include <cmath>
#include <cstring>
#include <map>
#include <utility>
#include <vector>

namespace se3icp {

constexpr int kGraphSharingMin = 0, kGraphSharingMax = 3;
enum GraphStat : int {
    GS_CLOUDS = 0,
    GS_USES,
    GS_CLASSES,
    GS_FULL,
    GS_ADOPTED,
    GS_REJ_ORDER,
    GS_REJ_GAP,
    GS_NO_LIST,
    GS_BYTES_UPLOADED,
    GS_COUNT
};

inline double graph_pair_scale(double scale_pre, double r_src, double r_tgt) {
    const double rmax = std::fmax(r_src, r_tgt);
    return scale_pre * (1.0 / rmax);
}

struct GraphClass {
    int32_t cloud;
    int32_t k_nrm;
    int32_t n_uses;
    int32_t nrm_from;
    double norm_center[3];
    double norm_scale;
    double f32_center[3];
};

struct GraphPlan {
    std::vector<int32_t> use_class;
    std::vector<GraphClass> classes;
    bool normalize = false, dedupe = false;
};

struct GraphUse {
    int32_t cloud;
    int32_t k_nrm;
    double norm_center[3];
    double norm_scale;
    double f32_center[3];
};

inline void graph_plan_uses(int32_t n_uses, const GraphUse* use, bool normalize, bool dedupe, GraphPlan* plan) {
    struct Key {
        int32_t cloud;
        uint64_t b[7];
        bool operator<(const Key& o) const {
            if (cloud != o.cloud) return cloud < o.cloud;
            return std::memcmp(b, o.b, sizeof(b)) < 0;
        }
    };
    std::map<Key, int32_t> seen;
    plan->use_class.assign((size_t)n_uses, -1);
    plan->classes.clear();
    plan->normalize = normalize;
    plan->dedupe = dedupe;
    for (int32_t u = 0; u < n_uses; ++u) {
        GraphClass g{};
        g.cloud = use[u].cloud;
        g.k_nrm = use[u].k_nrm;
        g.n_uses = 1;
        g.norm_scale = use[u].norm_scale;
        for (int a = 0; a < 3; ++a) {
            g.norm_center[a] = use[u].norm_center[a];
            g.f32_center[a] = use[u].f32_center[a];
        }
        Key k{};
        k.cloud = g.cloud;
        std::memcpy(&k.b[0], &g.norm_scale, 8);
        std::memcpy(&k.b[1], g.f32_center, 24);
        std::memcpy(&k.b[4], g.norm_center, 24);
        int32_t id = -1;
        if (dedupe) {
            auto it = seen.find(k);
            if (it != seen.end()) id = it->second;
        }
        if (id < 0) {
            id = (int32_t)plan->classes.size();
            plan->classes.push_back(g);
            if (dedupe) seen[k] = id;
        } else {
            GraphClass& h = plan->classes[id];
            h.k_nrm = h.k_nrm > g.k_nrm ? h.k_nrm : g.k_nrm;
            h.n_uses++;
        }
        plan->use_class[u] = id;
    }
    std::map<int32_t, int32_t> owner;
    for (int32_t k = 0; k < (int32_t)plan->classes.size(); ++k) {
        GraphClass& g = plan->classes[k];
        g.nrm_from = k;
        if (normalize || !dedupe || g.k_nrm <= 0) continue;
        auto it = owner.find(g.cloud);
        if (it == owner.end()) owner[g.cloud] = k;
        else if (plan->classes[it->second].k_nrm == g.k_nrm) g.nrm_from = it->second;
    }
}

constexpr int kLrfSeedingMin = 0, kLrfSeedingMax = 3;
struct SeedClass {
    int32_t from;
    double rho2;
};
inline int32_t graph_plan_seeds(const GraphPlan& plan, const int32_t* k_knn, const int64_t* n_pts,
                                std::vector<SeedClass>* seed) {
    const int32_t K = (int32_t)plan.classes.size();
    seed->assign((size_t)K, SeedClass{-1, 1.0});
    if (!plan.normalize || !plan.dedupe) return 0;
    auto uncentred = [](const GraphClass& g) { return g.f32_center[0] == 0.0 && g.f32_center[1] == 0.0 && g.f32_center[2] == 0.0; };
    std::map<int32_t, int32_t> source;
    int32_t seeded = 0;
    for (int32_t k = 0; k < K; ++k) {
        if (k_knn[k] <= 0) continue;
        const GraphClass& g = plan.classes[k];
        auto it = source.find(g.cloud);
        if (it == source.end()) {
            source[g.cloud] = k;
            continue;
        }
        const int32_t a = it->second;
        const GraphClass& ga = plan.classes[a];
        const int64_t kw = k_knn[k] < n_pts[k] ? k_knn[k] : n_pts[k], kwa = k_knn[a] < n_pts[a] ? k_knn[a] : n_pts[a];
        const double rho = g.norm_scale / ga.norm_scale;
        if (std::memcmp(g.norm_center, ga.norm_center, sizeof(g.norm_center)) != 0 || !uncentred(g) || !uncentred(ga) ||
            n_pts[k] != n_pts[a] || kw > kwa || !(rho > 0.0) || !std::isfinite(rho * rho))
            continue;
        (*seed)[k] = SeedClass{a, rho * rho};
        ++seeded;
    }
    return seeded;
}

constexpr int kPoseSeedingMin = 0, kPoseSeedingMax = 1;
enum InitStat : int { IS_EDGES = 0, IS_VARIANTS, IS_CROSS_SEEDED, IS_COUNT };
struct VariantPlan {
    std::vector<int32_t> edge_src, edge_tgt;
    std::vector<int32_t> cloud;
    std::vector<int32_t> pose_edge;
    int32_t posed_edges = 0, posed_variants = 0;
};
inline void graph_plan_variants(int32_t n_pairs, const int32_t* src, const int32_t* tgt, const double* T_init,
                                VariantPlan* vp) {
    static const double ident[16] = {1, 0, 0, 0, 0, 1, 0, 0, 0, 0, 1, 0, 0, 0, 0, 1};
    struct Key {
        int32_t cloud;
        int32_t posed;
        uint64_t b[16];
        bool operator<(const Key& o) const {
            if (cloud != o.cloud) return cloud < o.cloud;
            if (posed != o.posed) return posed < o.posed;
            return std::memcmp(b, o.b, sizeof(b)) < 0;
        }
    };
    std::map<Key, int32_t> seen;
    vp->edge_src.assign((size_t)n_pairs, -1);
    vp->edge_tgt.assign((size_t)n_pairs, -1);
    vp->cloud.clear();
    vp->pose_edge.clear();
    vp->posed_edges = vp->posed_variants = 0;
    for (int32_t p = 0; p < n_pairs; ++p)
        for (int side = 0; side < 2; ++side) {
            Key k{};
            k.cloud = side == 0 ? src[p] : tgt[p];
            const double* M = (side == 0 && T_init) ? T_init + 16 * (size_t)p : nullptr;
            if (M && std::memcmp(M, ident, sizeof(ident)) == 0) M = nullptr;
            if (M) {
                k.posed = 1;
                std::memcpy(k.b, M, sizeof(k.b));
                vp->posed_edges++;
            }
            auto it = seen.find(k);
            int32_t id;
            if (it == seen.end()) {
                id = (int32_t)vp->cloud.size();
                seen[k] = id;
                vp->cloud.push_back(k.cloud);
                vp->pose_edge.push_back(M ? p : -1);
                vp->posed_variants += M ? 1 : 0;
            } else {
                id = it->second;
            }
            (side == 0 ? vp->edge_src : vp->edge_tgt)[p] = id;
        }
}

inline int32_t graph_plan_seeds_posed(const GraphPlan& plan, const int32_t* k_knn, const int64_t* n_pts,
                                      const int32_t* raw, const int32_t* rigid, bool cross,
                                      std::vector<SeedClass>* seed, int32_t* n_cross) {
    const int32_t K = (int32_t)plan.classes.size();
    seed->assign((size_t)K, SeedClass{-1, 1.0});
    if (n_cross) *n_cross = 0;
    if (!plan.normalize || !plan.dedupe) return 0;
    auto uncentred = [](const GraphClass& g) { return g.f32_center[0] == 0.0 && g.f32_center[1] == 0.0 && g.f32_center[2] == 0.0; };
    std::map<std::pair<int32_t, int32_t>, int32_t> source;
    int32_t seeded = 0;
    for (int32_t k = 0; k < K; ++k) {
        if (k_knn[k] <= 0) continue;
        const GraphClass& g = plan.classes[k];
        const int32_t v = g.cloud;
        const std::pair<int32_t, int32_t> key{raw[v], (cross && rigid[v]) ? -1 : v};
        auto it = source.find(key);
        if (it == source.end()) {
            source[key] = k;
            continue;
        }
        const int32_t a = it->second;
        const GraphClass& ga = plan.classes[a];
        const int64_t kw = k_knn[k] < n_pts[k] ? k_knn[k] : n_pts[k], kwa = k_knn[a] < n_pts[a] ? k_knn[a] : n_pts[a];
        const double rho = g.norm_scale / ga.norm_scale;
        const bool same_variant = ga.cloud == v;
        if ((same_variant && std::memcmp(g.norm_center, ga.norm_center, sizeof(g.norm_center)) != 0) || !uncentred(g) ||
            !uncentred(ga) || n_pts[k] != n_pts[a] || kw > kwa || !(rho > 0.0) || !std::isfinite(rho * rho))
            continue;
        (*seed)[k] = SeedClass{a, rho * rho};
        ++seeded;
        if (!same_variant && n_cross) ++*n_cross;
    }
    return seeded;
}

constexpr int kTreeSharingMin = 0, kTreeSharingMax = 1;
inline int32_t graph_plan_trees(int32_t n_slots, const int32_t* cloud, const int64_t* n_pts, bool share,
                                std::vector<int32_t>* donor) {
    donor->assign((size_t)n_slots, -1);
    if (!share) return 0;
    std::map<int32_t, int32_t> first;
    int32_t adopters = 0;
    for (int32_t u = 0; u < n_slots; ++u) {
        if (cloud[u] < 0) continue;
        auto it = first.find(cloud[u]);
        if (it == first.end()) {
            first[cloud[u]] = u;
        } else if (n_pts[it->second] == n_pts[u]) {
            (*donor)[u] = it->second;
            ++adopters;
        }
    }
    return adopters;
}

inline void graph_plan(int32_t n_pairs, const int32_t* src, const int32_t* tgt, bool normalize, double scale_pre,
                       const double* center, const double* radius, int k_nrm_src, int k_nrm_tgt, bool dedupe,
                       GraphPlan* plan) {
    std::vector<GraphUse> use(2 * (size_t)n_pairs);
    for (int32_t p = 0; p < n_pairs; ++p) {
        const double scale = normalize ? graph_pair_scale(scale_pre, radius[src[p]], radius[tgt[p]]) : 1.0;
        for (int side = 0; side < 2; ++side) {
            const int32_t c = side == 0 ? src[p] : tgt[p];
            GraphUse& g = use[2 * (size_t)p + side];
            g.cloud = c;
            g.k_nrm = side == 0 ? k_nrm_src : k_nrm_tgt;
            g.norm_scale = scale;
            for (int a = 0; a < 3; ++a) {
                g.norm_center[a] = normalize ? center[3 * c + a] : 0.0;
                g.f32_center[a] = normalize ? 0.0 : center[3 * tgt[p] + a];
            }
        }
    }
    graph_plan_uses(2 * n_pairs, use.data(), normalize, dedupe, plan);
}

constexpr int kBatchSharingMin = 0, kBatchSharingMax = 2;

inline bool share_any_equal_n(int32_t n_slots, const int64_t* n) {
    std::map<int64_t, int32_t> seen;
    for (int32_t u = 0; u < n_slots; ++u)
        if (++seen[n[u]] > 1) return true;
    return false;
}

inline int32_t share_candidates(int32_t n_slots, const int64_t* n, const uint64_t* hash, std::vector<int32_t>* first) {
    std::map<std::pair<int64_t, uint64_t>, int32_t> seen;
    first->assign((size_t)n_slots, -1);
    int32_t cand = 0;
    for (int32_t u = 0; u < n_slots; ++u) {
        auto it = seen.find({n[u], hash[u]});
        if (it == seen.end()) {
            seen[{n[u], hash[u]}] = u;
            (*first)[u] = u;
        } else {
            (*first)[u] = it->second;
            ++cand;
        }
// ... 41 lines not shown
```

se3-icp_amd/csrc/k_lrf8.hip:

```cpp
#include <hip/hip_runtime.h>

#include <cfloat>
#include <climits>

#include "devmath.hpp"
#include "knn_util.hpp"
#include "tree.hpp"
#include "view.hpp"
#include "wave.hpp"

namespace se3icp {

namespace {

using namespace knn;

#ifndef SE3ICP_LRF8_WAVES
#define SE3ICP_LRF8_WAVES 4
#endif
constexpr int kW = SE3ICP_LRF8_WAVES;
constexpr int kQ = 8;
#ifndef SE3ICP_LRF8_CAP
#define SE3ICP_LRF8_CAP 192
#endif
constexpr int kCap = SE3ICP_LRF8_CAP;
#ifndef SE3ICP_LRF8_FILL
#define SE3ICP_LRF8_FILL SE3ICP_LRF8_CAP
#endif
constexpr int kFill = SE3ICP_LRF8_FILL;
constexpr int kStride = kCap + 4;
static_assert(((kStride / 4) & 1) == 1, "an odd number of 16-B slots per list");
constexpr int kLeaves = 64;
constexpr unsigned kIdBits = 0xfffu;
constexpr unsigned kAll = 0x7f7fffffu;
constexpr unsigned kPad = 0xffffffffu;

enum Park8 {
    P8_SUM = 0,
    P8_R = 21, P8_KK = 22, P8_GP = 23, P8_FLAGS = 24, P8_K = 25, P8_NTOP = 26, P8_ZN = 27,
    P8_W = 30,
    P8_N = 31
};
constexpr int kParkAt = 128;
static_assert(kCap >= kParkAt + 2 * P8_N && kStride >= kCap, "the park overlays the list tail");

__device__ __forceinline__ unsigned gx(unsigned x, int m) {
    switch (m) {
    case 1: return (unsigned)__builtin_amdgcn_mov_dpp((int)x, 0xB1, 0xF, 0xF, true);
    case 2: return (unsigned)__builtin_amdgcn_mov_dpp((int)x, 0x4E, 0xF, 0xF, true);
    case 3: return (unsigned)__builtin_amdgcn_mov_dpp((int)x, 0x1B, 0xF, 0xF, true);
    case 4: return (unsigned)__builtin_amdgcn_ds_swizzle((int)x, 0x101F);
    case 7: return (unsigned)__builtin_amdgcn_mov_dpp((int)x, 0x141, 0xF, 0xF, true);
    default: return (unsigned)__shfl_xor((int)x, m, 64);
    }
}
__device__ __forceinline__ double gxd(double x, int m) {
    const unsigned long long u = (unsigned long long)__double_as_longlong(x);
    const unsigned lo = gx((unsigned)u, m), hi = gx((unsigned)(u >> 32), m);
    return __longlong_as_double((long long)(((unsigned long long)hi << 32) | lo));
}

__device__ __forceinline__ unsigned med3u(unsigned a, unsigned b, unsigned x) {
    unsigned r;
    asm("v_med3_u32 %0, %1, %2, %3" : "=v"(r) : "v"(a), "v"(b), "v"(x));
    return r;
}

template <int PER, int KK, int JD>
__device__ __forceinline__ void stage8(unsigned (&k)[PER], int l) {
    if constexpr (JD == 0) {
        if constexpr (KK <= PER) {
#pragma unroll
            for (int s = 0; s < PER; ++s) {
                const int t = s ^ (KK - 1);
                if (s < t) {
                    const unsigned a = k[s], b = k[t];
                    k[s] = min(a, b);
                    k[t] = max(a, b);
                }
            }
        } else {
            constexpr int lm = KK / PER - 1;
            const unsigned x = (l & (KK / PER / 2)) == 0 ? 0u : ~0u;
#pragma unroll
            for (int s = 0; s < PER / 2; ++s) {
                const int t = PER - 1 - s;
                const unsigned a = gx(k[t], lm), b = gx(k[s], lm);
                k[s] = med3u(k[s], a, x);
                k[t] = med3u(k[t], b, x);
            }
        }
    } else if constexpr (JD < PER) {
#pragma unroll
        for (int s = 0; s < PER; ++s) {
            if ((s & JD) == 0) {
                const int t = s | JD;
                const unsigned a = k[s], b = k[t];
                k[s] = min(a, b);
                k[t] = max(a, b);
            }
        }
    } else {
        constexpr int lm = JD / PER;
        const unsigned x = (l & lm) == 0 ? 0u : ~0u;
#pragma unroll
        for (int s = 0; s < PER; ++s) k[s] = med3u(k[s], gx(k[s], lm), x);
    }
}
template <int PER, int N, int KK = 2, int JD = 0>
__device__ __forceinline__ void net8(unsigned (&k)[PER], int l) {
    stage8<PER, KK, JD>(k, l);
    constexpr int next_jd = JD == 0 ? KK / 4 : JD / 2;
    if constexpr (next_jd > 0) net8<PER, N, KK, next_jd>(k, l);
    else if constexpr (KK < N) net8<PER, N, KK * 2, 0>(k, l);
}
template <int PER>
__device__ __forceinline__ void sort8(unsigned (&k)[PER], int l) {
    net8<PER, 8 * PER>(k, l);
}

template <int PER>
__device__ __forceinline__ void load_head(const unsigned* list, int len, int l, unsigned (&k)[PER]) {
#pragma unroll
    for (int q = 0; q < PER / 4; ++q) {
        const int e0 = l * PER + 4 * q;
        uint4 x = make_uint4(kPad, kPad, kPad, kPad);
        if (e0 < len) x = *reinterpret_cast<const uint4*>(list + e0);
        k[4 * q] = x.x;
        k[4 * q + 1] = e0 + 1 < len ? x.y : kPad;
        k[4 * q + 2] = e0 + 2 < len ? x.z : kPad;
        k[4 * q + 3] = e0 + 3 < len ? x.w : kPad;
    }
}
template <int PER>
__device__ __forceinline__ void store_head(unsigned* list, int len, int l, const unsigned (&k)[PER], unsigned add = 0u) {
#pragma unroll
    for (int q = 0; q < PER / 4; ++q) {
        const int e0 = l * PER + 4 * q;
        if (e0 < len)
            *reinterpret_cast<uint4*>(list + e0) =
                make_uint4(k[4 * q] + add, k[4 * q + 1] + add, k[4 * q + 2] + add, k[4 * q + 3] + add);
    }
}
template <int PER = 16>
__device__ __forceinline__ void sort_head(unsigned* list, int len, int l) {
    unsigned k[PER];
    load_head<PER>(list, len, l, k);
    sort8<PER>(k, l);
    __builtin_amdgcn_wave_barrier();
    store_head<PER>(list, len, l, k);
    __builtin_amdgcn_wave_barrier();
}
template <int PER = 16>
__device__ __forceinline__ void sort_run(unsigned* list, int len, int l) {
    unsigned k[PER];
#pragma unroll
    for (int s = 0; s < PER; ++s) {
        const int e = l * PER + s;
        k[s] = e < len ? list[e] : kPad;
    }
    sort8<PER>(k, l);
    __builtin_amdgcn_wave_barrier();
#pragma unroll
    for (int s = 0; s < PER; ++s) {
        const int e = l * PER + s;
        if (e < len) list[e] = k[s];
    }
    __builtin_amdgcn_wave_barrier();
}
__device__ __forceinline__ float f32_err3(float d, float S) {
    const float u = 5.9604645e-08f;
    return 1.25f * (2.f * u * S * sqrtf(fmaxf(d, 0.f)) + 6.f * u * d + 4.f * u * u * S * S) + 1e-30f;
}
__device__ __forceinline__ unsigned widen_bound(unsigned t, float S) {
    if (t >= 0x7f800000u) return kAll;
    const float b = __uint_as_float(t);
    return min((__float_as_uint(fmaf(2.02f, f32_err3(b, S), b)) + 2u) | kIdBits, kAll);
}
__device__ __forceinline__ int upper_count(const unsigned* A, int n, unsigned t) {
    int lo = 0, hi = n;
    while (lo < hi) {
        const int m = (lo + hi) >> 1;
        if (A[m] <= t) lo = m + 1; else hi = m;
    }
    return lo;
}
__device__ __forceinline__ unsigned kth_of_two(const unsigned* A, int na, const unsigned* B, int nb, int r) {
    int lo = max(0, r + 1 - nb), hi = min(r + 1, na);
    while (lo < hi) {
        const int i = (lo + hi) >> 1;
        if (A[i] < B[r - i]) lo = i + 1; else hi = i;
    }
    const int j = r + 1 - lo;
    return max(lo > 0 ? A[lo - 1] : 0u, j > 0 ? B[j - 1] : 0u);
}
__device__ __forceinline__ uint3 tighten_group_sorted(unsigned* lists, int g, int l, int nbg, int mv, int nmax, int Kw,
                                                      bool presort, int tail_per, float S) {
    unsigned* list = lists + g * kStride;
    if (presort) {
        mv = min(nbg, 128);
        sort_head<16>(list, mv, l);
    }
    const int nb = nbg - mv;
    unsigned* B = list + mv;
    if (tail_per == 8) sort_run<8>(B, nb, l);
    else if (tail_per == 16) sort_run<16>(B, nb, l);
    const unsigned tg = nbg >= Kw ? widen_bound(kth_of_two(list, mv, B, nb, Kw - 1) | kIdBits, S) : kAll;
    const int ka = upper_count(list, mv, tg), kb = upper_count(B, nb, tg);
    const int kept = ka + kb;
    if (presort && tail_per == 0) return make_uint3(tg, (unsigned)ka, (unsigned)ka);
    if (__ballot(kept > 128) == 0ull) {
        unsigned k[16];
        load_head<16>(list, ka, l, k);
#pragma unroll
        for (int s = 0; s < 16; ++s) {
            const int e = l * 16 + s;
            if (e >= 128 - kb) k[s] = B[127 - e];
        }
        __builtin_amdgcn_wave_barrier();
        stage8<16, 128, 64>(k, l);
        stage8<16, 128, 32>(k, l);
        stage8<16, 128, 16>(k, l);
        stage8<16, 128, 8>(k, l);
        stage8<16, 128, 4>(k, l);
        stage8<16, 128, 2>(k, l);
        stage8<16, 128, 1>(k, l);
        store_head<16>(list, kept, l, k);
        __builtin_amdgcn_wave_barrier();
        return make_uint3(tg, (unsigned)kept, (unsigned)kept);
    }
    unsigned keep_n = 0;
    for (int r0 = 0; r0 < nmax; r0 += 8) {
        const int e = r0 + l;
        const unsigned ent = e < nbg ? list[e] : kPad;
        const bool keep = ent <= tg;
        const unsigned long long m = __ballot(keep);
        const unsigned gm = (unsigned)(m >> (8 * g)) & 0xffu;
        __builtin_amdgcn_wave_barrier();
        if (keep) list[(int)keep_n + __popc(gm & ((1u << l) - 1u))] = ent;
        keep_n += (unsigned)__popc(gm);
        __builtin_amdgcn_wave_barrier();
    }
    return make_uint3(tg, keep_n, 0u);
}

struct p3 { double x, y, z; };
__device__ __forceinline__ p3 ld3(const double4* __restrict__ P4, int i) {
    const double2 xy = *reinterpret_cast<const double2*>(P4 + i);
    const double z = reinterpret_cast<const double*>(P4 + i)[2];
    return p3{xy.x, xy.y, z};
}

__device__ __forceinline__ bool final_group(unsigned* lists, const int* leaf_slot, const double4* __restrict__ P4,
                                            const int32_t* __restrict__ perm, double qx, double qy, double qz, int off,
                                            int g, int l, int nbg, int mv, int fmode, int lim) {
    unsigned* list = lists + g * kStride;
    unsigned long long k[16];
    bool unsorted = false;
    {
        unsigned k32[16];
        if (fmode == 0) {
            load_head<16>(list, nbg, l, k32);
            sort8<16>(k32, l);
        } else {
            const int nb = nbg - mv;
            unsigned* B = list + mv;
            if (fmode == 1) sort_run<8>(B, nb, l);
            load_head<16>(list, mv, l, k32);
            if (fmode == 1) {
#pragma unroll
                for (int s = 0; s < 16; ++s) {
                    const int e = l * 16 + s;
                    if (e >= 128 - nb) k32[s] = B[127 - e];
                }
                __builtin_amdgcn_wave_barrier();
                stage8<16, 128, 64>(k32, l);
                stage8<16, 128, 32>(k32, l);
                stage8<16, 128, 16>(k32, l);
                stage8<16, 128, 8>(k32, l);
                stage8<16, 128, 4>(k32, l);
                stage8<16, 128, 2>(k32, l);
                stage8<16, 128, 1>(k32, l);
            }
        }
#pragma unroll
        for (int s = 0; s < 16; ++s) {
            const int e = l * 16 + s;
            unsigned long long x = ~0ull;
            if (e < nbg) {
                const unsigned id = k32[s] & kIdBits;
                const int slot = leaf_slot[id >> 6] + (int)(id & 63u);
                const p3 p = ld3(P4, slot);
                const unsigned key = __float_as_uint((float)l2_3(qx, qy, qz, p.x, p.y, p.z));
                x = ((unsigned long long)key << 32) | (unsigned)(slot - off);
            }
            k[s] = x;
        }
    }
    auto ce = [](unsigned long long& a, unsigned long long& b) __attribute__((always_inline)) {
        const bool sw = b < a;
        const unsigned long long lo = sw ? b : a, hi = sw ? a : b;
        a = lo;
        b = hi;
    };
    const int me = (int)(threadIdx.x & 63);
    auto next_first = [&]() __attribute__((always_inline)) {
        return ((unsigned long long)(unsigned)__shfl((int)(unsigned)(k[0] >> 32), me + 1, 64) << 32) |
               (unsigned)__shfl((int)(unsigned)k[0], me + 1, 64);
    };
#pragma unroll
    for (int s = 0; s < 16; s += 2) ce(k[s], k[s + 1]);
    {
#pragma unroll
        for (int s = 1; s + 1 < 16; s += 2) ce(k[s], k[s + 1]);
        const unsigned long long nx = next_first();
        const unsigned long long pv = ((unsigned long long)(unsigned)__shfl((int)(unsigned)(k[15] >> 32), me - 1, 64) << 32) |
                                      (unsigned)__shfl((int)(unsigned)k[15], me - 1, 64);
        if (l < 7 && nx < k[15]) k[15] = nx;
        if (l > 0 && k[0] < pv) k[0] = pv;
    }
#pragma unroll
    for (int s = 0; s < 16; s += 2) ce(k[s], k[s + 1]);
    const unsigned long long nx = next_first();
#pragma unroll
    for (int s = 0; s + 1 < 16; ++s) unsorted |= k[s + 1] < k[s];
    unsorted |= (l < 7) && nx < k[15];
    unsigned tall = 0u;
#pragma unroll
    for (int s = 0; s + 1 < 16; ++s) {
        const int e = l * 16 + s;
        if ((int)(e + 1 < nbg) & (int)((unsigned)(k[s] >> 32) == (unsigned)(k[s + 1] >> 32))) tall |= 1u << s;
    }
    {
        const int e = l * 16 + 15;
        if ((int)(l < 7) & (int)(e + 1 < nbg) & (int)((unsigned)(k[15] >> 32) == (unsigned)(nx >> 32))) tall |= 1u << 15;
    }
    const int nlim = lim - 1 - l * 16;
    unsigned tied = tall & (nlim >= 16 ? 0xffffu : nlim > 0 ? (1u << nlim) - 1u : 0u);
    const unsigned tprev = (unsigned)__shfl((int)tall, me - 1, 64), tnext = (unsigned)__shfl((int)tall, me + 1, 64);
    const unsigned tall_lo = (tall << 1) | (l > 0 ? (tprev >> 15) & 1u : 0u);
    const unsigned tall_hi = (tall >> 1) | (l < 7 ? (tnext & 1u) << 15 : 0u);
    const unsigned isolated = ~(tall_lo | tall_hi);
    __builtin_amdgcn_wave_barrier();
    {
        unsigned sl[16];
#pragma unroll
        for (int s = 0; s < 16; ++s) sl[s] = (unsigned)k[s];
        store_head<16>(list, nbg, l, sl, (unsigned)off);
    }
    __builtin_amdgcn_wave_barrier();
    bool bad = unsorted;
    while (tied) {
        const int sb = __builtin_ctz(tied);
        const int e = l * 16 + sb;
        tied &= tied - 1u;
        const int a = (int)list[e], b = (int)list[e + 1];
        const p3 pa = ld3(P4, a), pb = ld3(P4, b);
        const double da = l2_3(qx, qy, qz, pa.x, pa.y, pa.z), db = l2_3(qx, qy, qz, pb.x, pb.y, pb.z);
        const bool wrong = (bool)((int)(da > db) | ((int)(da == db) & (int)(perm[a] > perm[b])));
        bad |= (bool)((int)(e + 2 >= lim) & (int)((tall_hi >> sb) & 1u));
        if (wrong) {
            if ((isolated >> sb) & 1u) {
                list[e] = (unsigned)b;
                list[e + 1] = (unsigned)a;
            } else {
                bad = true;
            }
        } else if (!((isolated >> sb) & 1u)) {
            bad |= da != db;
        }
    }
    const bool ok = !(bool)(unsigned)((__ballot(bad) >> (8 * g)) & 0xffull);
    return ok;
}

#ifdef SE3ICP_PROF
#define PROF8_NOW(t) const unsigned long long t = __builtin_readcyclecounter()
#define PROF8_ADD(acc, a, b) acc += (b) - (a)
#else
#define PROF8_NOW(t) do {} while (0)
#define PROF8_ADD(acc, a, b) do {} while (0)
#endif

static_assert(kW >= 2 && kW * kQ <= 64, "the per-block epilogue: waves 0 and 1, a lane per query");

template <bool SD, bool ST>
__global__ __launch_bounds__(64 * kW) __attribute__((amdgpu_waves_per_eu(kCap <= 192 ? 6 : (kCap <= 224 ? 5 : 4)))) void k_lrf8(
    View v, const int32_t* __restrict__ cloud_of, const CloudSetup* __restrict__ setup,
    const CloudDev* __restrict__ clouds, const float* __restrict__ tlo, const float* __restrict__ thi,
    const double4* __restrict__ P4, const int32_t* __restrict__ wave_base, int w_lo, int nwaves,
    int32_t* __restrict__ fb_list, int32_t* __restrict__ fb_count, const SeedRef* __restrict__ seed,
    float* __restrict__ seedbuf, int seed_mode) {
    __shared__ __attribute__((aligned(16))) unsigned s_list[kW][kQ][kStride];
    auto park_of = [&](int w, int j) __attribute__((always_inline)) {
        return reinterpret_cast<double*>(&s_list[w][j][kParkAt]);
    };
    __shared__ int s_leaf[kW][kLeaves];
    __shared__ __attribute__((aligned(16))) float s_q[kW][3 * kQ];
    const int lane = threadIdx.x & 63, wid = __builtin_amdgcn_readfirstlane(threadIdx.x >> 6);
    const int g = lane >> 3, l = lane & 7;
    const int bid = xcd_block(blockIdx.x, gridDim.x);
    const TreeRef T = v.t3;
    const int first_leaf = (1 << T.L) - 1;
    unsigned* lists = &s_list[wid][0][0];
    int* leaves = s_leaf[wid];
    unsigned n_leaves = 0, n_sel = 0, n_cand = 0, n_q = 0;
#ifdef SE3ICP_PROF
    unsigned long long c_scan = 0, c_tight = 0, c_sums = 0, c_epi = 0;
    unsigned n_tover = 0, n_tend = 0;
    unsigned long long fb_cause = 0;
#define PROF8_FB(field) fb_cause += 1ull << (16 * (field))
#else
#define PROF8_FB(field) do {} while (0)
#endif
    PROF8_NOW(t_a0);

    const int wv = __builtin_amdgcn_readfirstlane(w_lo + bid * kW + wid);
    int mode = 0, c = 0, w0 = 0, qn = 0;
    CloudSetup st{};
    CloudDev cl{0, 0};
    int K = 0, Kw = 0;
    if (wv < nwaves) {
        int lo = 0, hi = v.nclouds - 1;
        while (lo < hi) {
            const int mid = (lo + hi + 1) >> 1;
            if (wave_base[mid] <= wv) lo = mid; else hi = mid - 1;
        }
        c = lo;
        cl = clouds[c];
        st = setup[c];
        K = st.k_knn;
        w0 = cl.off + kQ * (wv - wave_base[c]);
        qn = min(kQ, cl.off + cl.n - w0);
        if (K > 0 && qn > 0) {
            Kw = min(K, cl.n);
            mode = (qn == kQ && Kw <= 128) ? 1 : 2;
        }
    }
    bool fb_wave = mode == 2;
    unsigned Tq[kQ], nbq[kQ];
#pragma unroll
    for (int j = 0; j < kQ; ++j) { Tq[j] = kAll; nbq[j] = 0u; }
    auto group_len = [&]() __attribute__((always_inline)) {
        int x = 0;
#pragma unroll
        for (int j = 0; j < kQ; ++j) asm volatile("v_writelane_b32 %0, %1, %2" : "+v"(x) : "s"(nbq[j]), "n"(8 * j));
        return (unsigned)__shfl(x, lane & ~7, 64);
    };
    int mvv = 0;
    float* qv = s_q[wid];
    float fqlo[3] = {0.f, 0.f, 0.f}, fqhi[3] = {0.f, 0.f, 0.f};
    int nlist = 0;
    const int n = cl.n;
    float s_norm = 0.f;
    if (mode == 1) {
        const float fx = lane < kQ ? T.tvec[w0 + lane] : 0.f;
        const float fy = lane < kQ ? T.tvec[v.ld + w0 + lane] : 0.f;
        const float fz = lane < kQ ? T.tvec[2 * (size_t)v.ld + w0 + lane] : 0.f;
        if (lane < kQ) {
            qv[lane] = fx;
            qv[kQ + lane] = fy;
            qv[2 * kQ + lane] = fz;
        }
        {
            const float* rlo = tlo + (size_t)c * T.nnodes * 3;
            const float* rhi = thi + (size_t)c * T.nnodes * 3;
            float r2 = 0.f;
#pragma unroll
            for (int a = 0; a < 3; ++a) r2 += fmaxf(rlo[a] * rlo[a], rhi[a] * rhi[a]);
            s_norm = 2.f * sqrtf(r2) * 1.0001f;
        }
        __builtin_amdgcn_wave_barrier();
        fqlo[0] = fqhi[0] = __shfl(fx, 0, 64);
        fqlo[1] = fqhi[1] = __shfl(fy, 0, 64);
        fqlo[2] = fqhi[2] = __shfl(fz, 0, 64);
#pragma unroll
        for (int j = 1; j < kQ; ++j) {
            const float a = __shfl(fx, j, 64), b = __shfl(fy, j, 64), d = __shfl(fz, j, 64);
            fqlo[0] = fminf(fqlo[0], a); fqhi[0] = fmaxf(fqhi[0], a);
            fqlo[1] = fminf(fqlo[1], b); fqhi[1] = fmaxf(fqhi[1], b);
            fqlo[2] = fminf(fqlo[2], d); fqhi[2] = fmaxf(fqhi[2], d);
        }
        n_q = kQ;
    }
    bool sd_open = false, sd_close = false, t_cert = true;
    unsigned n_sdq = 0, n_sda = 0, n_sdf = 0;
    if constexpr (SD) {
        if (mode == 2) n_sda = (unsigned)qn;
        if (mode == 1) {
            const SeedRef sr = seed[c];
            float sv = 0.f;
            if (lane < kQ) sv = seedbuf[sr.load + T.perm[w0 + lane]];
            if (seed_mode == 2) sv *= 0.5f;
            if (seed_mode == 3) sv *= 4.f;
            if (__ballot(!(bool)((int)(sv >= 0.f) & (int)(sv < INFINITY))) == 0ull) {
                const unsigned t0 = f32_up_bits((double)sv * sr.rho2 * (1.0 + 0x1p-20)) | kIdBits;
                const unsigned tb = widen_bound(widen_bound(t0, s_norm), s_norm);
#pragma unroll
                for (int j = 0; j < kQ; ++j) Tq[j] = (unsigned)__builtin_amdgcn_readlane((int)tb, j);
                sd_open = true;
                n_sdq = kQ;
            } else {
                n_sda = kQ;
            }
        }
    }

    auto tighten = [&]() __attribute__((always_inline)) {
        ++n_sel;
        unsigned nmax = 0;
#pragma unroll
        for (int j = 0; j < kQ; ++j) nmax = max(nmax, nbq[j]);
        __builtin_amdgcn_wave_barrier();
        int dmax = 0;
        bool anyz = false;
#pragma unroll
        for (int j = 0; j < kQ; ++j) {
            const int mj = __builtin_amdgcn_readlane(mvv, 8 * j);
            dmax = max(dmax, (int)nbq[j] - mj);
            anyz |= mj == 0;
        }
        const bool presort = anyz || dmax > 128;
        const int tail_per = presort ? (nmax <= 128 ? 0 : (nmax <= 192 ? 8 : 16)) : (dmax == 0 ? 0 : dmax <= 64 ? 8 : 16);
        const uint3 r3 = tighten_group_sorted(lists, g, l, (int)group_len(), mvv, (int)nmax, Kw, presort, tail_per, s_norm);
        mvv = (int)r3.z;
        __builtin_amdgcn_wave_barrier();
        if constexpr (SD) {
            bool cert = true;
#pragma unroll
            for (int j = 0; j < kQ; ++j) {
                const unsigned tn = (unsigned)__builtin_amdgcn_readlane((int)r3.x, 8 * j);
                cert &= tn <= Tq[j];
                Tq[j] = min(Tq[j], tn);
                nbq[j] = (unsigned)__builtin_amdgcn_readlane((int)r3.y, 8 * j);
            }
            t_cert = cert;
        } else {
#pragma unroll
            for (int j = 0; j < kQ; ++j) {
                Tq[j] = (unsigned)__builtin_amdgcn_readlane((int)r3.x, 8 * j);
                nbq[j] = (unsigned)__builtin_amdgcn_readlane((int)r3.y, 8 * j);
            }
        }
    };

    auto scan_leaf = [&](int i, int part) __attribute__((always_inline)) -> bool {
        if (nlist >= kLeaves) { fb_wave = true; PROF8_FB(0); return true; }
        const int li = nlist++;
        ++n_leaves;
        const int a = __builtin_amdgcn_readfirstlane(tree_first(n, T.L, i));
        const int b = __builtin_amdgcn_readfirstlane(tree_first(n, T.L, i + 1));
        if (lane == 0) leaves[li] = cl.off + a;
        const bool valid = (bool)((int)(lane < b - a) & (int)(part == 0 || (part == 1) == (lane < 32)));
        const int slot = cl.off + a + (valid ? lane : 0);
        const unsigned id = (unsigned)((li << 6) | lane);
        unsigned ent[kQ];
        unsigned long long m[kQ];
        bool over = false;
        float dq[kQ];
        {
            typedef float f2 __attribute__((ext_vector_type(2)));
            const float px = valid ? T.tvec[slot] : INFINITY;
            const float py = valid ? T.tvec[v.ld + slot] : INFINITY;
            const float pz = valid ? T.tvec[2 * (size_t)v.ld + slot] : INFINITY;
            const f2* qf2 = reinterpret_cast<const f2*>(qv);
            const f2 pxx = f2{px, px}, pyy = f2{py, py}, pzz = f2{pz, pz};
            auto pk_sub = [](f2 a, f2 b) __attribute__((always_inline)) {
                f2 r;
                asm("v_pk_add_f32 %0, %1, %2 neg_lo:[0,1] neg_hi:[0,1]" : "=v"(r) : "v"(a), "v"(b));
                return r;
            };
#pragma unroll
            for (int jp = 0; jp < kQ / 2; ++jp) {
                const f2 ex = pk_sub(qf2[jp], pxx), ey = pk_sub(qf2[kQ / 2 + jp], pyy), ez = pk_sub(qf2[kQ + jp], pzz);
                f2 s2 = ex * ex;
                s2 = __builtin_elementwise_fma(ey, ey, s2);
                s2 = __builtin_elementwise_fma(ez, ez, s2);
                dq[2 * jp] = s2.x;
                dq[2 * jp + 1] = s2.y;
            }
        }
#pragma unroll
        for (int j = 0; j < kQ; ++j) {
            ent[j] = (__float_as_uint(dq[j]) & ~kIdBits) | id;
            m[j] = __ballot(ent[j] <= Tq[j]);
            over |= nbq[j] + (unsigned)__popcll(m[j]) > (unsigned)kCap;
        }
        if (over) {
            --nlist;
            --n_leaves;
            return false;
        }
#pragma unroll
        for (int j = 0; j < kQ; ++j) {
            if (ent[j] <= Tq[j]) {
                const int at = (int)nbq[j] + __builtin_amdgcn_mbcnt_hi((unsigned)(m[j] >> 32), __builtin_amdgcn_mbcnt_lo((unsigned)m[j], 0u));
                lists[j * kStride + at] = ent[j];
            }
            nbq[j] += (unsigned)__popcll(m[j]);
        }
        __builtin_amdgcn_wave_barrier();
        return true;
    };

    if (mode == 1) {
        const int lf0 = tree_node_of(w0 - cl.off, n, T.L), lf1 = tree_node_of(w0 + kQ - 1 - cl.off, n, T.L);
        const int nleaf = 1 << T.L;
        int s_lo = lf0, s_hi = lf1;
        auto thr_f = [&]() __attribute__((always_inline)) {
            unsigned tm = 0u;
#pragma unroll
            for (int j = 0; j < kQ; ++j) tm = max(tm, Tq[j]);
            return __uint_as_float(f32_up_bits((double)__uint_as_float(tm) * (1.0 + 2e-6)));
        };
        auto box_lb = [&](int h) __attribute__((always_inline)) {
            const float* lo = tlo + ((size_t)c * T.nnodes + h) * 3;
            const float* hi = thi + ((size_t)c * T.nnodes + h) * 3;
            float s = 0.f;
#pragma unroll
            for (int a = 0; a < 3; ++a) {
                const float e = fmaxf(fmaxf(lo[a] - fqhi[a], fqlo[a] - hi[a]), 0.f);
                s += e * e;
            }
            return s;
        };
        const int sh = T.L > 6 ? 6 : T.L;
        const int nA = 1 << (T.L - sh), firstA = nA - 1;
        int stage = 0, nxt = lf0, c0 = 0, l0 = 0;
        bool up = true, haveA = false;
        float lbA = INFINITY, lbL = INFINITY;
        OutwardBits itA(0ull, 0), itL(0ull, 0);
        int cur = -1, part = 0;
        bool do_tighten = false, retried = false;
        float tf = INFINITY;
        if constexpr (SD) {
            if (sd_open) tf = thr_f();
        }
        while (!fb_wave) {
            if (do_tighten) {
                PROF8_NOW(t_t0);
                tighten();
                PROF8_NOW(t_t1);
                PROF8_ADD(c_tight, t_t0, t_t1);
                do_tighten = false;
                if constexpr (SD) {
                    if (sd_close) {
                        sd_close = false;
                        if (!t_cert) {
                            fb_wave = true;
                            n_sdf = kQ;
                            continue;
                        }
                    }
                }
                tf = thr_f();
#if defined(SE3ICP_LRF8_CUT) && SE3ICP_LRF8_CUT == 4
                if (stage == 2) break;
#endif
            }
            if (cur >= 0) {
#if defined(SE3ICP_LRF8_CUT) && SE3ICP_LRF8_CUT == 5
                if (stage >= 2) { cur = -1; part = 0; ++n_leaves; continue; }
#endif
                if (scan_leaf(cur, part)) {
                    if (part == 1) part = 2;
                    else { cur = -1; part = 0; }
                    retried = false;
                } else if (!retried && (int)nbq[0] >= Kw) {
                    do_tighten = true;
                    retried = true;
#ifdef SE3ICP_PROF
                    ++n_tover;
#endif
                } else if (part == 0) {
                    part = 1;
                    retried = false;
                } else {
                    fb_wave = true;
                    PROF8_FB(1);
                }
                continue;
            }
            int leaf = -1;
            if (stage == 0) {
                leaf = nxt++;
                if (nxt > lf1) stage = (SD && sd_open) ? 2 : 1;
            } else if (stage == 1) {
                const bool more_hi = s_hi < nleaf - 1, more_lo = s_lo > 0;
                const int cand = (more_hi && (up || !more_lo)) ? s_hi + 1 : s_lo - 1;
                const int csz = (more_hi || more_lo) ? tree_first(n, T.L, cand + 1) - tree_first(n, T.L, cand) : 0;
                if ((more_hi || more_lo) && ((int)nbq[0] < Kw || (int)nbq[0] + csz <= kFill)) {
                    leaf = cand;
                    if (cand > s_hi) s_hi = cand; else s_lo = cand;
                    up = !up;
                } else {
                    do_tighten = true;
                    stage = 2;
                    continue;
                }
            } else if (stage == 2) {
                if (!haveA) {
                    if (c0 >= nA) {
                        if constexpr (SD) {
                            if (sd_open) {
                                sd_open = false;
                                sd_close = true;
                                do_tighten = true;
                                retried = true;
                                continue;
                            }
                        }
                        unsigned nmax = 0;
#pragma unroll
                        for (int j = 0; j < kQ; ++j) nmax = max(nmax, nbq[j]);
                        if (nmax > 128 && !retried) {
#ifdef SE3ICP_PROF
                            ++n_tend;
#endif
                            do_tighten = true;
                            retried = true;
                            continue;
                        }
                        if (nmax > 128) { fb_wave = true; PROF8_FB(2); }
                        break;
                    }
                    const int ai = c0 + lane;
                    lbA = ai < nA ? box_lb(firstA + ai) : INFINITY;
                    itA = OutwardBits(__ballot(lbA <= tf), (lf0 >> sh) - c0);
                    haveA = true;
                }
                const int j = itA.next();
                if (j < 0) { haveA = false; c0 += 64; continue; }
                if (!(__int_as_float(__builtin_amdgcn_readlane(__float_as_int(lbA), j)) <= tf)) continue;
                l0 = (c0 + j) << sh;
                const int li = l0 + lane;
                lbL = INFINITY;
                if ((int)(lane < (1 << sh)) & ((int)(li < s_lo) | (int)(li > s_hi))) lbL = box_lb(first_leaf + li);
                itL = OutwardBits(__ballot(lbL <= tf), lf0 - l0);
                stage = 3;
                continue;
            } else {
                const int t = itL.next();
                if (t < 0) { stage = 2; continue; }
                if (!(__int_as_float(__builtin_amdgcn_readlane(__float_as_int(lbL), t)) <= tf)) continue;
                leaf = l0 + t;
            }
            cur = leaf;
        }
    }
    __builtin_amdgcn_wave_barrier();

    PROF8_NOW(t_a1);
#if defined(SE3ICP_LRF8_CUT) && (SE3ICP_LRF8_CUT == 1 || SE3ICP_LRF8_CUT == 4 || SE3ICP_LRF8_CUT == 5)
    if (lane == 0 && n_leaves == 12345u) v.stats[0] = nlist;
    return;
#endif
    PROF8_ADD(c_scan, t_a0, t_a1);
    const int kl = st.k_lrf, kn_want = st.k_nrm;
    const bool want_t = kl > 0, want_n = kn_want > 0;
    bool fb_q = fb_wave;
    const int nbg = (int)group_len();
    const int nTop = min(Kw, nbg);
    const int kk = min(kl, nTop), kn = min(kn_want, nTop);
    const int wq = w0 + g;
    p3 qg{0.0, 0.0, 0.0};
    if (mode == 1) qg = ld3(P4, wq);
    if (mode == 1 && !fb_wave) {
        __builtin_amdgcn_wave_barrier();
        int fmode = 0;
        {
            int dmax = 0;
            bool anyz = false;
#pragma unroll
            for (int j = 0; j < kQ; ++j) {
                const int mj = __builtin_amdgcn_readlane(mvv, 8 * j);
                dmax = max(dmax, (int)nbq[j] - mj);
                anyz |= mj == 0;
            }
            fmode = anyz || dmax > 64 ? 0 : dmax == 0 ? 2 : 1;
        }
        const bool exact = final_group(lists, leaves, P4, T.perm, qg.x, qg.y, qg.z, cl.off, g, l, nbg, mvv, fmode,
                                       min(nbg, max(kk, kn) + 1));
        fb_q = (bool)((int)!exact | (int)(nTop < Kw));
        n_cand += (unsigned)nbg;
#ifdef SE3ICP_PROF
        fb_cause += (unsigned long long)__popcll(__ballot((int)fb_q & (int)(l == 0) & (int)(g < qn))) << 48;
#endif
    }
    if ((int)(mode != 0) & (int)fb_q & (int)(l == 0) & (int)(g < qn)) {
        const int at = atomicAdd(fb_count, 1);
        fb_list[at] = wq;
        atomicAdd(v.stats + kStatCols * (wv & 63) + 6, 1ull);
    }
    const bool mine = (bool)((int)(mode == 1) & (int)!fb_q);

#if defined(SE3ICP_LRF8_CUT) && SE3ICP_LRF8_CUT == 2
    if (lane == 0 && n_cand == 12345u) v.stats[0] = n_cand;
    return;
#endif
    const unsigned* rl = lists + g * kStride;
    double* pj = park_of(wid, g);
    if constexpr (ST) {
        if (mode == 1) {
            const int so = seed[c].store;
            if ((int)(so >= 0) & (int)mine & (int)(l == 0)) {
                const p3 f = ld3(P4, (int)rl[Kw - 1]);
                seedbuf[so + T.perm[wq]] = (float)l2_3(qg.x, qg.y, qg.z, f.x, f.y, f.z);
            }
        }
    }
    {
        double x[12];
#pragma unroll
        for (int i = 0; i < 12; ++i) x[i] = 0.0;
        double Rf = 0.0;
        if ((int)mine & (int)want_t) {
            const int rz = kk / 3;
            const int hi = min(rz, kk - 1);
            p3 pn = ld3(P4, (int)rl[max(min(1 + l, hi), 0)]);
            for (int rk = 1 + l; rk <= hi; rk += 8) {
                const p3 p = pn;
                pn = ld3(P4, (int)rl[min(rk + 8, hi)]);
                const double vx = p.x - qg.x, vy = p.y - qg.y, vz = p.z - qg.z;
                if (rk < rz) { x[0] += vx; x[1] += vy; x[2] += vz; }
                x[3] += vx; x[4] += vy; x[5] += vz;
                x[6] += vx * vx; x[7] += vx * vy; x[8] += vx * vz;
                x[9] += vy * vy; x[10] += vy * vz; x[11] += vz * vz;
            }
            if (l == 0) {
                const p3 f = ld3(P4, (int)rl[kk - 1]);
                const double fdx = qg.x - f.x, fdy = qg.y - f.y, fdz = qg.z - f.z;
                Rf = sqrt(fdx * fdx + fdy * fdy + fdz * fdz);
            }
        }
#pragma unroll
        for (int i = 0; i < 12; ++i) {
            x[i] += gxd(x[i], 1);
            x[i] += gxd(x[i], 2);
            x[i] += gxd(x[i], 4);
        }
        __builtin_amdgcn_wave_barrier();
        if ((int)(l == 0) & (int)mine) {
#pragma unroll
            for (int i = 0; i < 12; ++i) pj[P8_SUM + i] = x[i];
            pj[P8_R] = Rf;
        }
    }
    {
        double x[9];
#pragma unroll
        for (int i = 0; i < 9; ++i) x[i] = 0.0;
        if ((int)mine & (int)want_n) {
            p3 pn = ld3(P4, (int)rl[max(min(l, kn - 1), 0)]);
            for (int r = l; r < kn; r += 8) {
                const p3 p = pn;
                pn = ld3(P4, (int)rl[min(r + 8, kn - 1)]);
                const double px = p.x, py = p.y, pz = p.z;
                x[0] += px; x[1] += py; x[2] += pz;
                x[3] += px * px; x[4] += px * py; x[5] += px * pz;
                x[6] += py * py; x[7] += py * pz; x[8] += pz * pz;
            }
        }
#pragma unroll
        for (int i = 0; i < 9; ++i) {
            x[i] += gxd(x[i], 1);
            x[i] += gxd(x[i], 2);
            x[i] += gxd(x[i], 4);
        }
        __builtin_amdgcn_wave_barrier();
        if (l == 0) {
            const int flags = mine ? ((want_t ? 1 : 0) | (want_n ? 2 : 0)) : 0;
            pj[P8_FLAGS] = (double)flags;
            if (mine) {
#pragma unroll
                for (int i = 0; i < 9; ++i) pj[P8_SUM + 12 + i] = x[i];
                pj[P8_KK] = (double)kk;
                pj[P8_GP] = (double)(cl.off + T.perm[wq]);
                pj[P8_K] = (double)K;
                pj[P8_NTOP] = (double)nTop;
                pj[P8_W] = (double)wq;
            }
        }
        __builtin_amdgcn_wave_barrier();
    }
    PROF8_NOW(t_a2);
    PROF8_ADD(c_sums, t_a1, t_a2);
    unsigned long long* ctr = v.stats + kStatCols * (wv & 63);
    if (lane == 0) {
        atomicAdd(ctr + 0, (unsigned long long)n_q);
        atomicAdd(ctr + 1, (unsigned long long)n_leaves);
        atomicAdd(ctr + 2, (unsigned long long)n_sel);
        atomicAdd(ctr + 4, (unsigned long long)n_cand);
        if constexpr (SD) {
            if (n_sdq) atomicAdd(ctr + kSeedStatCol, (unsigned long long)n_sdq);
            if (n_sda) atomicAdd(ctr + kSeedStatCol + 1, (unsigned long long)n_sda);
            if (n_sdf) atomicAdd(ctr + kSeedStatCol + 2, (unsigned long long)n_sdf);
        }
    }

#if defined(SE3ICP_LRF8_CUT) && SE3ICP_LRF8_CUT == 3
    return;
#endif
    auto toldi_eig = [&](double* pb) __attribute__((always_inline)) {
        const p3 q = ld3(P4, (int)pb[P8_W]);
        const double rz = (double)((int)pb[P8_KK] / 3);
        const double q3[3] = {q.x, q.y, q.z};
        double cq[3], S[3];
#pragma unroll
        for (int a = 0; a < 3; ++a) {
            cq[a] = (pb[P8_SUM + a] - q3[a]) / rz;
            S[a] = pb[P8_SUM + 3 + a];
        }
        const double* M = pb + P8_SUM + 6;
        const int ia[6] = {0, 0, 0, 1, 1, 2}, ib[6] = {0, 1, 2, 1, 2, 2};
        double c6[6];
#pragma unroll
        for (int k = 0; k < 6; ++k)
            c6[k] = M[k] - S[ia[k]] * cq[ib[k]] - cq[ia[k]] * S[ib[k]] + rz * cq[ia[k]] * cq[ib[k]];
        const d3 zn = jacobi_smallest_evec(c6[0], c6[1], c6[2], c6[3], c6[4], c6[5]);
        pb[P8_ZN] = zn.x;
        pb[P8_ZN + 1] = zn.y;
        pb[P8_ZN + 2] = zn.z;
    };
    auto normal_eig = [&](const double* pb) __attribute__((always_inline)) {
        const int wb = (int)pb[P8_W];
        const int cc = cloud_of[wb];
        const int knb = min(setup[cc].k_nrm, (int)pb[P8_NTOP]);
        double n6[6] = {1, 0, 0, 1, 0, 1};
        if (knb >= 3) {
            double cu[9];
#pragma unroll
            for (int i = 0; i < 9; ++i) cu[i] = pb[P8_SUM + 12 + i] / (double)knb;
            n6[0] = cu[3] - cu[0] * cu[0];
            n6[1] = cu[4] - cu[0] * cu[1];
            n6[2] = cu[5] - cu[0] * cu[2];
            n6[3] = cu[6] - cu[1] * cu[1];
            n6[4] = cu[7] - cu[1] * cu[2];
            n6[5] = cu[8] - cu[2] * cu[2];
        }
        d3 nm = fast_eigen3x3(n6[0], n6[1], n6[2], n6[3], n6[4], n6[5]);
        if (sqrt(dot3(nm, nm)) == 0.0) nm = d3{0, 0, 1};
        const int gp = (int)pb[P8_GP];
        v.nrm64[gp] = nm.x;
        v.nrm64[v.ld + gp] = nm.y;
        v.nrm64[2 * (size_t)v.ld + gp] = nm.z;
    };
    __syncthreads();
    if (wid <= 1) {
        double* pb = park_of(lane < kW * kQ ? lane / kQ : 0, lane % kQ);
        const int b_flags = lane < kW * kQ ? (int)pb[P8_FLAGS] : 0;
        if ((b_flags & 1) && wid == 0) toldi_eig(pb);
        if ((b_flags & 2) && wid == 1) normal_eig(pb);
    }
    __syncthreads();

    {
        const int flags = (int)pj[P8_FLAGS];
        double x6[6] = {0.0, 0.0, 0.0, 0.0, 0.0, 0.0};
        if (flags & 1) {
            const double nx = pj[P8_ZN], ny = pj[P8_ZN + 1], nz = pj[P8_ZN + 2];
            const double R = pj[P8_R];
            const int kkq = (int)pj[P8_KK];
            p3 pn = ld3(P4, (int)rl[max(min(1 + l, kkq - 1), 0)]);
            for (int r = 1 + l; r < kkq; r += 8) {
                const p3 p = pn;
                pn = ld3(P4, (int)rl[min(r + 8, kkq - 1)]);
                const double vx = p.x - qg.x, vy = p.y - qg.y, vz = p.z - qg.z;
                x6[0] += vx; x6[1] += vy; x6[2] += vz;
                const double an = nx * vx + ny * vy + nz * vz;
                const double rr = R - sqrt(vx * vx + vy * vy + vz * vz);
                const double wgt = (rr * rr) * (an * an);
                x6[3] += wgt * vx; x6[4] += wgt * vy; x6[5] += wgt * vz;
            }
        }
#pragma unroll
        for (int i = 0; i < 6; ++i) {
            x6[i] += gxd(x6[i], 1);
            x6[i] += gxd(x6[i], 2);
            x6[i] += gxd(x6[i], 4);
        }
        __builtin_amdgcn_wave_barrier();
        if ((int)(l == 0) & (int)((flags & 1) != 0)) {
#pragma unroll
            for (int i = 0; i < 6; ++i) pj[P8_SUM + i] = x6[i];
        }
    }
    __syncthreads();
    if (wid == 0) {
        const double* pb = park_of(lane < kW * kQ ? lane / kQ : 0, lane % kQ);
        const int b_flags = lane < kW * kQ ? (int)pb[P8_FLAGS] : 0;
        if (b_flags & 1) {
            const int w = (int)pb[P8_W];
            const CloudSetup sw = setup[cloud_of[w]];
            const p3 q = ld3(P4, w);
            d3 nrm{pb[P8_ZN], pb[P8_ZN + 1], pb[P8_ZN + 2]};
            if (nrm.x * pb[P8_SUM] + nrm.y * pb[P8_SUM + 1] + nrm.z * pb[P8_SUM + 2] < 0.0)
                nrm = d3{-nrm.x, -nrm.y, -nrm.z};
            const d3 zax = nrm;
            const d3 accs{pb[P8_SUM + 3], pb[P8_SUM + 4], pb[P8_SUM + 5]};
            d3 xax = accs - dot3(accs, zax) * zax;
            xax = (1.0 / sqrt(dot3(xax, xax))) * xax;
            const d3 yax = cross3(zax, xax);
            const double al = sw.alpha, be = sw.beta;
            const double f12[12] = {al * xax.x, al * xax.y, al * xax.z, al * yax.x, al * yax.y, al * yax.z,
                                    al * zax.x, al * zax.y, al * zax.z, be * q.x, be * q.y, be * q.z};
            store_frame_rows(v.fr64, v.fr32, (int)pb[P8_GP], f12, sw.cf_target, q.x, q.y, q.z);
        }
    }
#ifdef SE3ICP_PROF
    PROF8_NOW(t_a3);
    PROF8_ADD(c_epi, t_a2, t_a3);
    if (lane == 0) {
        atomicAdd(ctr + 8, c_scan - c_tight);
        atomicAdd(ctr + 9, c_tight);
        atomicAdd(ctr + 10, c_sums);
        atomicAdd(ctr + 11, c_epi);
        atomicAdd(ctr + 3, (unsigned long long)n_tover);
        atomicAdd(ctr + 7, (unsigned long long)n_tend);
        atomicAdd(ctr + 5, fb_cause);
    }
#endif
}

}

void launch_lrf8(const View& v, const int32_t* wave_base, int w_lo, int w_hi, int32_t* fb_list, int32_t* fb_count,
                 hipStream_t s, const SeedRef* seed, float* seedbuf, bool seeded, int seed_mode) {
    const int nb = (w_hi - w_lo + kW - 1) / kW;
    if (nb <= 0) return;
    if (seeded)
        hipLaunchKernelGGL((k_lrf8<true, false>), dim3(nb), dim3(64 * kW), 0, s, v, v.cloud_of, v.setup, v.clouds, v.t3.lo,
                           v.t3.hi, v.t3.tpt64, wave_base, w_lo, w_hi, fb_list, fb_count, seed, seedbuf, seed_mode);
    else if (seed != nullptr)
        hipLaunchKernelGGL((k_lrf8<false, true>), dim3(nb), dim3(64 * kW), 0, s, v, v.cloud_of, v.setup, v.clouds, v.t3.lo,
                           v.t3.hi, v.t3.tpt64, wave_base, w_lo, w_hi, fb_list, fb_count, seed, seedbuf, seed_mode);
    else
        hipLaunchKernelGGL((k_lrf8<false, false>), dim3(nb), dim3(64 * kW), 0, s, v, v.cloud_of, v.setup, v.clouds, v.t3.lo,
                           v.t3.hi, v.t3.tpt64, wave_base, w_lo, w_hi, fb_list, fb_count, seed, seedbuf, seed_mode);
}

}
```

se3-icp_amd/csrc/view.hpp:

```cpp
#pragma once
#include <hip/hip_runtime.h>
#include <stdint.h>

#include "common.hpp"

namespace se3icp {

struct CloudSetup {
    int32_t k_knn;
    int32_t k_lrf;
    int32_t k_nrm;
    int32_t want_cov;
    int32_t want_conf;
    int32_t is_target;
    int32_t cf_target;
    int32_t _pad;
    double alpha, beta;
    double norm_center[3];
    double norm_scale;
    double f32_center[3];
};

struct TreeRef {
    int32_t L;
    int32_t GL;
    int32_t nnodes;
    const int32_t* perm;
    const int32_t* pos;
    const float* tvec;
    const double* tvec64;
    const double4* tpt64;
    const float* lo;
    const float* hi;
};

struct alignas(16) NNCert {
    float d1, l2;
    int32_t iter, j;
    double t[3];
    float margin;
    int32_t _pad;
};
static_assert(sizeof(NNCert) == 48, "three 16-B words");

struct View {
    int32_t ld;
    int32_t npts;
    int32_t nclouds;
    int32_t npairs;
    int32_t kmax;
    CloudDev* clouds;
    CloudSetup* setup;
    PairDev* pairs;
    int32_t* cloud_of;
    const double* const* in_ptr;
    double* xyz64;
    float* xyz32;
    double* fr64;
    float* fr32;
    double* nrm64;
    double* conf64;
    double* tgeo;
    int32_t* knn;
    int32_t* corr_idx;
    float* corr_dist;
    unsigned long long* stats;
    int32_t* flag_count;
    uint64_t* trim_key;
    unsigned long long* trim_cand;
    unsigned* trim_ctr;
    unsigned* trim_hist;
    double* red_partial;
    double* red_out;
    const BlockWork* work;
    int32_t nwork;
    int32_t* pair_rechecked;
    TreeRef t3, t12;
    int32_t chunk_level;
    int32_t nchunks;
    int32_t* qlist;
    int32_t* qcount;
    int32_t* sq_list;
    const double* hist;
    NNCert* cert;
    uint32_t* gcost;
    int32_t* cls;
};

constexpr int kChunk = 2048;
struct ChunkWork { int32_t cloud; int32_t p0; };

void launch_ingest(const View& v, const ChunkWork* chunks, int nchunks, double* partial , hipStream_t s);
void launch_ingest_posed(const View& v, const ChunkWork* chunks, int nchunks, double* partial ,
                         const int32_t* pose_of, const double* poses, hipStream_t s);
void launch_radius(const View& v, const ChunkWork* chunks, int nchunks, const double* centers ,
                   double* partial , hipStream_t s);
void launch_normalize(const View& v, const ChunkWork* chunks, int nchunks, double* partial ,
                      hipStream_t s);
void launch_pair_centers(const View& v, const ChunkWork* chunks, int nchunks, const double* partial, double* centers,
                         hipStream_t s);
void launch_pair_scales(const View& v, const ChunkWork* chunks, int nchunks, const double* partial,
                        const double* centers, double scale_pre, double* scales, hipStream_t s);
void launch_pair_norms(const View& v, int nnodes3, int nnodes12, const double* scales, double* state_sf,
                       int state_stride, hipStream_t s);
void launch_lrf(const View& v, int write_knn, hipStream_t s);
void launch_lrf_list(const View& v, const int32_t* qlist, const int32_t* qcount, hipStream_t s, int qpw = 0);
struct SeedRef { int32_t store; int32_t load; double rho2; };
void launch_lrf8(const View& v, const int32_t* wave_base, int w_lo, int w_hi, int32_t* fb_list, int32_t* fb_count,
                 hipStream_t s, const SeedRef* seed = nullptr, float* seedbuf = nullptr, bool seeded = false,
                 int seed_mode = 0);
int knn_big_cap(int kw_max);
int knn_big_blocks(int cap, int nq);
void launch_knn_big(const View& v, int write_knn, int k_min, const int32_t* qlist, const int32_t* qcount, int nblocks,
                    double* scratch_d, int32_t* scratch_i, int cap, hipStream_t s);

void launch_nn_prep(const View& v, int32_t* publish, hipStream_t s);
void nn_prof_report();
void trim_prof_report();
#ifdef SE3ICP_PROF
double nn_prep_span();
void nn_wave_report(int it);
#endif
void launch_nn(const View& v, int D, hipStream_t s);
size_t nn_cls_words(int nchunks);
void launch_trim(const View& v, hipStream_t s);
void launch_geo_rows(const View& v, hipStream_t s);
struct PairState;
void launch_reduce(const View& v, const int32_t* pair_wb, const int32_t* pair_wn, PairState* state, double* hist,
                   int32_t* next_phase, hipStream_t s);

}
```

se3-icp_amd/se3icp/__init__.py:

```python
from ._lib import (METHODS, Params, Result, Se3IcpError, default_params, device_count, load,
                   method_id, status_string)
from .io import read_ply_xyz, write_ply_xyz
from .registration import (DeviceBatchRunner, IterativeSE3Registration, PairResult, PipelinedBatchRunner,
                           cli_params,
                           estimate_normals,
                           kitti_params, knn_self, last_kernel_times, set_nn_events, set_profiling, lounge_params,
                           nearest_neighbors,
                           register_batch, register_batch_device, register_batch_traced, toldi_frames,
                           alpha_grid, register_sweep, register_sweep_device, register_sweep_traced, sweep_params,
                           PairReport, register_batch_report, register_batch_report_device, register_sweep_report,
                           register_sweep_report_device,
                           expand_edges, last_graph_stats, register_graph, register_graph_device,
                           register_graph_report, register_graph_traced, register_sequence, sequence_edges,
                           set_batch_sharing, set_lrf_seeding, last_seed_stats,
                           set_tree_sharing, last_tree_stats,
                           voxel_downsample, voxel_downsample_device,
                           edge_inits, last_init_stats, set_pose_seeding, transform_device, transform_points)
from ._lib import Report, ReportOptions

__all__ = [
    "IterativeSE3Registration", "register_batch", "register_batch_device", "DeviceBatchRunner", "PipelinedBatchRunner", "register_batch_traced", "toldi_frames", "knn_self",
    "estimate_normals", "nearest_neighbors", "default_params", "cli_params", "kitti_params", "lounge_params",
    "read_ply_xyz", "write_ply_xyz", "METHODS", "Se3IcpError",
    "register_sweep", "register_sweep_device", "register_sweep_traced", "alpha_grid", "sweep_params",
    "PairReport", "Report", "ReportOptions", "register_batch_report", "register_batch_report_device",
    "register_sweep_report", "register_sweep_report_device",
    "register_graph", "register_sequence", "sequence_edges", "expand_edges", "register_graph_device",
    "register_graph_report", "register_graph_traced", "last_graph_stats",
    "set_batch_sharing", "set_lrf_seeding", "last_seed_stats", "set_tree_sharing", "last_tree_stats",
    "voxel_downsample", "voxel_downsample_device",
    "edge_inits", "transform_points", "transform_device", "set_pose_seeding", "last_init_stats",
]
```

se3-icp_amd/se3icp/_lib.py:

```python
from __future__ import annotations

import ctypes as C
import os

_PKG = os.path.dirname(os.path.abspath(__file__))
_ROOT = os.path.dirname(_PKG)
LIB_PATH = os.environ.get("SE3ICP_LIB") or os.path.join(_ROOT, "lib", "libse3icp.so")

OK = 0
ERR_INVALID_ARG = -1
ERR_INVALID_METHOD = -2
ERR_EMPTY_CLOUD = -3
ERR_K_TOO_LARGE = -4
ERR_NO_DEVICE = -5
ERR_HIP = -6
ERR_NONFINITE = -7
ERR_OUT_OF_MEMORY = -8
ERR_INTERNAL = -9

METHODS = ["pt2pt", "pt2pl", "gicp", "se3_pt2pt", "se3_pt2pl", "se3_gicp", "se3_gicp_with_cf",
           "se3_pure_pt2pt", "se3_pure_pt2pl", "se3_pure_gicp"]

EXPORTED_SYMBOLS = [
    "se3icp_abi_version", "se3icp_status_string", "se3icp_method_from_name", "se3icp_method_name",
    "se3icp_default_params", "se3icp_device_count",
    "se3icp_registration_new", "se3icp_registration_free", "se3icp_set_source_cloud", "se3icp_set_target_cloud",
    "se3icp_params_of", "se3icp_run_icp", "se3icp_run_se3_icp", "se3icp_run_se3_icp_with_cf", "se3icp_run_se3_pure",
    "se3icp_get_result",
    "se3icp_register_batch", "se3icp_register_batch_device", "se3icp_register",
    "se3icp_register_sweep", "se3icp_register_sweep_device",
    "se3icp_register_graph", "se3icp_register_graph_device", "se3icp_register_graph_report",
    "se3icp_register_graph_report_device", "se3icp_last_graph_stats", "se3icp_set_batch_sharing",
    "se3icp_set_lrf_seeding", "se3icp_last_seed_stats", "se3icp_set_tree_sharing", "se3icp_last_tree_stats",
    "se3icp_report_version", "se3icp_register_batch_report", "se3icp_register_batch_report_device",
    "se3icp_register_sweep_report", "se3icp_register_sweep_report_device",
    "se3icp_request_report", "se3icp_get_report",
    "se3icp_toldi_frames", "se3icp_knn_self", "se3icp_estimate_normals", "se3icp_nn",
    "se3icp_synthetic_pairs", "se3icp_synthetic_reference", "se3icp_synthetic_reference_device",
    "se3icp_random_downsample",
    "se3icp_voxel_version", "se3icp_voxel_downsample_device", "se3icp_voxel_downsample",
    "se3icp_init_version", "se3icp_register_graph_init", "se3icp_register_graph_init_device",
    "se3icp_set_initial_transform", "se3icp_set_pose_seeding", "se3icp_last_init_stats",
    "se3icp_transform_points", "se3icp_transform_device",
    "se3icp_set_profiling", "se3icp_last_kernel_times", "se3icp_last_kernel_times_n", "se3icp_set_trace", "se3icp_set_lrf_exact",
    "se3icp_set_nn_events",
    "se3icp_cc_rot_3d", "se3icp_cc_angular_error_so3", "se3icp_cc_angular_error_so3_alt",
    "se3icp_cc_error_filterreg", "se3icp_cc_rot2euler", "se3icp_cc_avg_eul_error",
    "se3icp_cc_evaluate_lrf_quality", "se3icp_cc_evaluate_trajectory",
    "se3icp_cc_read_trajectory", "se3icp_cc_read_kitti_poses", "se3icp_cc_read_redwood_log",
    "se3icp_cc_write_trajectory", "se3icp_cc_write_redwood_log",
]


class Params(C.Structure):
    _fields_ = [
        ("max_num_iterations", C.c_int32),
        ("max_num_se3_iterations", C.c_int32),
        ("number_of_nn_for_LRF", C.c_int32),
        ("_reserved", C.c_int32),
        ("mse", C.c_double),
        ("mse_switch_error", C.c_double),
        ("estimated_overlap", C.c_double),
        ("alpha_rot", C.c_double),
        ("beta_transl", C.c_double),
        ("scale_preprocessing", C.c_double),
    ]


class Result(C.Structure):
    _fields_ = [
        ("T", C.c_double * 16),
        ("num_iterations", C.c_int32),
        ("num_pure_se3_iterations", C.c_int32),
        ("status", C.c_int32),
        ("num_rechecked", C.c_int32),
        ("scaling_factor", C.c_double),
        ("time_setup_ms", C.c_double),
        ("time_loop_ms", C.c_double),
        ("time_se3_correspondence_search_ms", C.c_double),
        ("time_before_pure_icp_ms", C.c_double),
    ]


STOP_CONVERGED = 0
STOP_MAX_ITERATIONS = 1
STOP_MAX_SE3_ITERATIONS = 2
STOP_RUNAWAY = 3
STOP_REASONS = ["converged", "max_iterations", "max_se3_iterations", "runaway"]


class ReportOptions(C.Structure):
    _fields_ = [
        ("max_correspondence_distance", C.c_double),
        ("corr_idx", C.c_void_p),
        ("corr_dist", C.c_void_p),
        ("outputs_on_device", C.c_int32),
        ("_reserved", C.c_int32),
    ]


class Report(C.Structure):
    _fields_ = [
        ("fitness", C.c_double),
        ("inlier_rmse", C.c_double),
        ("information", C.c_double * 36),
        ("final_mse", C.c_double),
        ("final_mse_change", C.c_double),
        ("n_inliers", C.c_int64),
        ("switched", C.c_int32),
        ("stop_reason", C.c_int32),
    ]


class Trace(C.Structure):
    _fields_ = [
        ("pair", C.c_int32),
        ("max_iters", C.c_int32),
        ("corr_idx", C.POINTER(C.c_int32)),
        ("corr_dist", C.POINTER(C.c_float)),
        ("trim_key", C.POINTER(C.c_uint64)),
        ("T", C.POINTER(C.c_double)),
        ("mse", C.POINTER(C.c_double)),
        ("phase", C.POINTER(C.c_int32)),
        ("iters_recorded", C.c_int32),
        ("_reserved", C.c_int32),
    ]


GRAPH_STATS = ["clouds", "uses", "classes", "classes_full", "adopted", "rejected_order", "rejected_gap", "no_list",
               "bytes_uploaded"]
SEED_STATS = ["classes_seeded", "queries_seeded", "queries_unseeded", "queries_failed"]
INIT_STATS = ["posed_edges", "posed_variants", "classes_seeded_across"]
TREE_STATS = ["built_3d", "adopted_3d", "built_12d", "adopted_12d"]


class Se3IcpError(RuntimeError):
    def __init__(self, code: int, what: str = ""):
        self.code = code
        msg = status_string(code) if _lib is not None else str(code)
        super().__init__(f"se3icp error {code} ({msg}){': ' + what if what else ''}")


_lib = None


def load():
    global _lib
    if _lib is not None:
        return _lib
    if not os.path.exists(LIB_PATH):
        raise ImportError(f"HIP engine library not built: {LIB_PATH} is missing "
                          "(run __graft_entry__.build() or `make -C se3-icp_amd`)")
    L = C.CDLL(LIB_PATH)
    dp, ip = C.POINTER(C.c_double), C.POINTER(C.c_int32)
    vp = C.c_void_p
    L.se3icp_abi_version.restype = C.c_int
    L.se3icp_status_string.restype = C.c_char_p
    L.se3icp_status_string.argtypes = [C.c_int]
    L.se3icp_method_from_name.argtypes = [C.c_char_p]
    L.se3icp_method_name.restype = C.c_char_p
    L.se3icp_method_name.argtypes = [C.c_int]
    L.se3icp_default_params.argtypes = [C.POINTER(Params)]
    L.se3icp_device_count.restype = C.c_int
    L.se3icp_registration_new.restype = vp
    L.se3icp_registration_free.argtypes = [vp]
    L.se3icp_set_source_cloud.argtypes = [vp, dp, C.c_int64]
    L.se3icp_set_target_cloud.argtypes = [vp, dp, C.c_int64]
    L.se3icp_params_of.restype = C.POINTER(Params)
    L.se3icp_params_of.argtypes = [vp]
    L.se3icp_run_icp.argtypes = [vp, C.c_char_p]
    L.se3icp_run_se3_icp.argtypes = [vp, C.c_char_p]
    L.se3icp_run_se3_icp_with_cf.argtypes = [vp]
    L.se3icp_run_se3_pure.argtypes = [vp, C.c_char_p]
    L.se3icp_get_result.argtypes = [vp, C.POINTER(Result)]
    L.se3icp_register_batch.argtypes = [C.c_int, C.c_int32, C.POINTER(dp), C.POINTER(C.c_int64), C.POINTER(dp),
                                        C.POINTER(C.c_int64), C.c_int, C.POINTER(Params), C.POINTER(Result)]
    L.se3icp_register_batch_device.argtypes = [C.c_int, C.c_int32, vp, C.POINTER(C.c_int64), vp,
                                               C.POINTER(C.c_int64), C.c_int, C.POINTER(Params), C.POINTER(Result), vp]
    L.se3icp_register_sweep.argtypes = [C.c_int, C.c_int32, C.POINTER(dp), C.POINTER(C.c_int64), C.POINTER(dp),
                                        C.POINTER(C.c_int64), C.c_int, C.c_int32, C.POINTER(Params), C.c_int32,
                                        C.POINTER(Result)]
    L.se3icp_register_sweep_device.argtypes = [C.c_int, C.c_int32, vp, C.POINTER(C.c_int64), vp,
                                               C.POINTER(C.c_int64), C.c_int, C.c_int32, C.POINTER(Params), C.c_int32,
                                               C.POINTER(Result), vp]
    rop, rep = C.POINTER(ReportOptions), C.POINTER(Report)
    L.se3icp_report_version.restype = C.c_int
    L.se3icp_register_batch_report.argtypes = L.se3icp_register_batch.argtypes + [rop, rep]
    L.se3icp_register_batch_report_device.argtypes = L.se3icp_register_batch_device.argtypes + [rop, rep]
    L.se3icp_register_sweep_report.argtypes = L.se3icp_register_sweep.argtypes + [rop, rep]
    L.se3icp_register_sweep_report_device.argtypes = L.se3icp_register_sweep_device.argtypes + [rop, rep]
    L.se3icp_register_graph.argtypes = [C.c_int, C.c_int32, C.POINTER(dp), C.POINTER(C.c_int64), C.c_int32, ip, ip,
                                        C.c_int, C.POINTER(Params), C.c_int32, C.POINTER(Result)]
    L.se3icp_register_graph_device.argtypes = [C.c_int, C.c_int32, vp, C.POINTER(C.c_int64), C.c_int32, ip, ip,
                                               C.c_int, C.POINTER(Params), C.c_int32, C.POINTER(Result), vp]
    L.se3icp_register_graph_report.argtypes = L.se3icp_register_graph.argtypes + [rop, rep]
    L.se3icp_register_graph_report_device.argtypes = L.se3icp_register_graph_device.argtypes + [rop, rep]
    L.se3icp_last_graph_stats.argtypes = [C.c_int, C.POINTER(C.c_int64), C.c_int]
    if hasattr(L, "se3icp_init_version"):
        L.se3icp_init_version.restype = C.c_int
        L.se3icp_register_graph_init.argtypes = [C.c_int, C.c_int32, C.POINTER(dp), C.POINTER(C.c_int64), C.c_int32,
                                                 ip, ip, dp, C.c_int, C.POINTER(Params), C.c_int32, C.POINTER(Result),
                                                 rop, rep]
        L.se3icp_register_graph_init_device.argtypes = [C.c_int, C.c_int32, vp, C.POINTER(C.c_int64), C.c_int32, ip, ip,
                                                        dp, C.c_int, C.POINTER(Params), C.c_int32, C.POINTER(Result),
                                                        vp, rop, rep]
        L.se3icp_set_initial_transform.argtypes = [vp, dp]
        L.se3icp_set_pose_seeding.argtypes = [C.c_int, C.c_int]
        L.se3icp_last_init_stats.argtypes = [C.c_int, C.POINTER(C.c_int64), C.c_int]
        L.se3icp_transform_points.argtypes = [dp, dp, C.c_int64, dp]
        L.se3icp_transform_device.argtypes = [C.c_int, C.c_int32, vp, C.POINTER(C.c_int64), dp, vp, vp]
    L.se3icp_request_report.argtypes = [vp, rop]
    L.se3icp_get_report.argtypes = [vp, rep]
    L.se3icp_register.argtypes = [C.c_int, dp, C.c_int64, dp, C.c_int64, C.c_int, C.POINTER(Params),
                                  C.POINTER(Result)]
    L.se3icp_toldi_frames.argtypes = [C.c_int, dp, C.c_int64, C.c_int, dp]
    L.se3icp_knn_self.argtypes = [C.c_int, dp, C.c_int64, C.c_int, ip]
    L.se3icp_estimate_normals.argtypes = [C.c_int, dp, C.c_int64, C.c_int, dp]
    L.se3icp_nn.argtypes = [C.c_int, dp, C.c_int64, dp, C.c_int64, C.c_int, ip, dp, ip]
    L.se3icp_synthetic_pairs.restype = C.c_int64
    L.se3icp_synthetic_pairs.argtypes = [C.c_int, dp, C.c_int64, C.c_int32, dp, C.c_double, C.c_double, C.c_uint64,
                                         vp, vp, C.c_int]
    L.se3icp_synthetic_reference.restype = C.c_int64
    L.se3icp_synthetic_reference.argtypes = [dp, C.c_int64, C.c_int32, C.c_double, C.c_double, C.c_double, C.c_double,
                                             C.c_int32, dp, dp, dp]
    L.se3icp_synthetic_reference_device.restype = C.c_int64
    L.se3icp_synthetic_reference_device.argtypes = [C.c_int, dp, C.c_int64, C.c_int32, C.c_double, C.c_double,
                                                    C.c_double, C.c_double, C.c_int32, vp, vp, dp, C.c_int]
    L.se3icp_random_downsample.restype = C.c_int64
    L.se3icp_random_downsample.argtypes = [dp, C.c_int64, C.c_double, C.c_uint32, dp]
    L.se3icp_voxel_version.restype = C.c_int
    L.se3icp_voxel_downsample_device.argtypes = [C.c_int, C.c_int32, vp, C.POINTER(C.c_int64), dp, vp,
                                                 C.POINTER(C.c_int64), vp, vp, vp]
    L.se3icp_voxel_downsample.restype = C.c_int64
    L.se3icp_voxel_downsample.argtypes = [C.c_int, dp, C.c_int64, C.c_double, dp, ip, ip]
    L.se3icp_set_profiling.argtypes = [C.c_int, C.c_int]
    L.se3icp_last_kernel_times.argtypes = [C.c_int, dp]
    L.se3icp_last_kernel_times_n.argtypes = [C.c_int, dp, C.c_int]
    L.se3icp_set_trace.argtypes = [C.c_int, C.POINTER(Trace)]
    L.se3icp_set_lrf_exact.argtypes = [C.c_int, C.c_int]
    L.se3icp_set_nn_events.argtypes = [C.c_int, C.c_int]
    _lib = L
    return L


def status_string(code: int) -> str:
    return load().se3icp_status_string(int(code)).decode()


def check(code: int, what: str = "") -> int:
    if code != OK:
        raise Se3IcpError(code, what)
    return code


def default_params(**overrides) -> Params:
    p = Params()
    load().se3icp_default_params(C.byref(p))
    for k, v in overrides.items():
        setattr(p, k, v)
    return p


def device_count() -> int:
    return load().se3icp_device_count()


def method_id(name: str) -> int:
    m = load().se3icp_method_from_name(name.encode())
    if m < 0:
        raise ValueError(f"unknown method {name!r}; valid: {', '.join(METHODS)}")
    return m
```

se3-icp_amd/se3icp/registration.py:

```python
from __future__ import annotations

import contextlib
import ctypes as C
import threading
import time
from dataclasses import dataclass

import numpy as np

from . import _lib
from .io import read_ply_xyz

_PARAM_FIELDS = {
    "max_num_iterations_": "max_num_iterations",
    "max_num_se3_iterations_": "max_num_se3_iterations",
    "number_of_nn_for_LRF_": "number_of_nn_for_LRF",
    "mse_": "mse",
    "mse_switch_error_": "mse_switch_error",
    "estimated_overlap_": "estimated_overlap",
    "alpha_rot": "alpha_rot",
    "beta_transl": "beta_transl",
    "scale_preprocessing": "scale_preprocessing",
}

# ... 618 lines not shown


def register_graph_device(xyz_ptr: int, off, edges, method: str, params: _lib.Params | None = None,
                          device: int = 0, stream: int = 0, sharing: int = 0, init=None) -> list[PairResult]:
    nc = len(off) - 1
    co = (C.c_int64 * (nc + 1))(*[int(x) for x in off])
    n, es, et = _edge_arrays(edges)
    res, _ = _outputs(n)
    T0 = _init_array(init, n)
    if T0 is not None:
        _registered(_lib.load().se3icp_register_graph_init_device(
            device, nc, C.c_void_p(xyz_ptr), co, n, es, et, T0.ctypes.data_as(_DP), _lib.method_id(method),
            _params_ref(params), int(sharing), res, _stream_arg(stream), None, None), "register_graph_init_device")
        return _results(res, n)
    _registered(_lib.load().se3icp_register_graph_device(device, nc, C.c_void_p(xyz_ptr), co, n, es, et,
                                                         _lib.method_id(method), _params_ref(params), int(sharing),
                                                         res, _stream_arg(stream)), "register_graph_device")
    return _results(res, n)


def register_graph_report(clouds, edges, method: str, params: _lib.Params | None = None, device: int = 0,
                          sharing: int = 0, max_correspondence_distance: float = 0.0, per_point: bool = False,
                          init=None):
    cl, cargs = _cloud_args(clouds)
    n, es, et = _edge_arrays(edges)
    counts = [cl[int(s)].shape[0] for s, _ in edges]
    res, rep = _outputs(n)
    opts, idx, dist = _per_point_options(max_correspondence_distance, counts, per_point)
    T0 = _init_array(init, n)
    if T0 is not None:
        _registered(_lib.load().se3icp_register_graph_init(device, *cargs, n, es, et, T0.ctypes.data_as(_DP),
                                                           _lib.method_id(method), _params_ref(params), int(sharing),
                                                           res, C.byref(opts), rep), "register_graph_init")
        return _results(res, n), _pair_reports(rep, counts, idx, dist)
    _registered(_lib.load().se3icp_register_graph_report(device, *cargs, n, es, et, _lib.method_id(method),
                                                         _params_ref(params), int(sharing), res, C.byref(opts), rep),
                "register_graph_report")
    return _results(res, n), _pair_reports(rep, counts, idx, dist)


def register_graph_traced(clouds, edges, method: str, params: _lib.Params | None = None, edge: int = 0,
                          max_iters: int = 160, device: int = 0, sharing: int = 0, init=None):
    with _armed_trace(device, edge, _as_xyz(clouds[int(edges[edge][0])]).shape[0], max_iters) as trace:
        res = register_graph(clouds, edges, method, params, device, sharing, init=init)
    return res, trace


_IP = C.POINTER(C.c_int32)


def voxel_downsample(xyz, voxel_size: float, device: int = 0, return_counts: bool = False):
    pts = _as_xyz(xyz)
    n = pts.shape[0]
    out = np.empty((max(n, 1), 3))
    cnt = np.empty(max(n, 1), dtype=np.int32)
    fst = np.empty(max(n, 1), dtype=np.int32)
    m = _lib.load().se3icp_voxel_downsample(int(device), pts.ctypes.data_as(_DP), n, float(voxel_size),
                                            out.ctypes.data_as(_DP), cnt.ctypes.data_as(_IP) if return_counts else None,
                                            fst.ctypes.data_as(_IP) if return_counts else None)
    if m < 0:
        raise _lib.Se3IcpError(int(m), "voxel_downsample")
    if return_counts:
        return out[:m].copy(), cnt[:m].copy(), fst[:m].copy()
    return out[:m].copy()


def voxel_downsample_device(xyz_ptr: int, off, voxel_size, out_ptr: int, device: int = 0, stream: int = 0,
                            count_ptr: int = 0, first_ptr: int = 0) -> list[int]:
    nc = len(off) - 1
    vs = np.ascontiguousarray(np.broadcast_to(np.asarray(voxel_size, dtype=np.float64), (max(nc, 0),)))
    co = (C.c_int64 * (max(nc, 0) + 1))(*[int(x) for x in off])
    oo = (C.c_int64 * (max(nc, 0) + 1))()
    _lib.check(_lib.load().se3icp_voxel_downsample_device(
        int(device), nc, C.c_void_p(xyz_ptr), co, vs.ctypes.data_as(_DP), C.c_void_p(out_ptr), oo,
        C.c_void_p(count_ptr) if count_ptr else None, C.c_void_p(first_ptr) if first_ptr else None,
        _stream_arg(stream)), "voxel_downsample_device")
    return [int(x) for x in oo]


def _register_graph_voxel(clouds, edges, method, params, device, sharing, voxel_size, init=None):
    import torch

    cl = [_as_xyz(c) for c in clouds]
    off = np.concatenate([[0], np.cumsum([a.shape[0] for a in cl])]).astype(np.int64)
    if len(cl) == 0 or off[-1] == 0:
        raise _lib.Se3IcpError(_lib.ERR_EMPTY_CLOUD, "register_graph(voxel_size=...)")
    dev = torch.device("cuda", int(device) & 0xff)
    raw = torch.from_numpy(np.concatenate(cl)).to(dev)
    down = torch.empty_like(raw)
    torch.cuda.synchronize(dev)
    out_off = voxel_downsample_device(raw.data_ptr(), off, voxel_size, down.data_ptr(), device=device)
    return register_graph_device(down.data_ptr(), out_off, edges, method, params, device=device, sharing=sharing,
                                 init=init)


def last_graph_stats(device: int = 0) -> dict:
    out = (C.c_int64 * len(_lib.GRAPH_STATS))()
    _lib.check(_lib.load().se3icp_last_graph_stats(device, out, len(_lib.GRAPH_STATS)), "last_graph_stats")
    return {k: int(out[i]) for i, k in enumerate(_lib.GRAPH_STATS)}


def set_batch_sharing(level: int, device: int = 0) -> None:
    _lib.check(_lib.load().se3icp_set_batch_sharing(int(device), int(level)), "set_batch_sharing")


def toldi_frames(pts, k: int, device: int = 0) -> np.ndarray:
    pts = _as_xyz(pts)
    out = np.zeros((pts.shape[0], 4, 4))
    _lib.check(_lib.load().se3icp_toldi_frames(device, pts.ctypes.data_as(C.POINTER(C.c_double)), pts.shape[0], k,
                                               out.ctypes.data_as(C.POINTER(C.c_double))), "toldi_frames")
    return out


def knn_self(pts, k: int, device: int = 0) -> np.ndarray:
    pts = _as_xyz(pts)
    out = np.zeros((pts.shape[0], k), np.int32)
    _lib.check(_lib.load().se3icp_knn_self(device, pts.ctypes.data_as(C.POINTER(C.c_double)), pts.shape[0], k,
                                           out.ctypes.data_as(C.POINTER(C.c_int32))), "knn_self")
    return out


def estimate_normals(pts, k: int = 30, device: int = 0) -> np.ndarray:
    pts = _as_xyz(pts)
    out = np.zeros_like(pts)
    _lib.check(_lib.load().se3icp_estimate_normals(device, pts.ctypes.data_as(C.POINTER(C.c_double)), pts.shape[0],
                                                   k, out.ctypes.data_as(C.POINTER(C.c_double))), "estimate_normals")
    return out


def nearest_neighbors(query, data, device: int = 0):
    q = np.ascontiguousarray(query, dtype=np.float64)
    d = np.ascontiguousarray(data, dtype=np.float64)
    dim = d.shape[1]
    idx = np.zeros(q.shape[0], np.int32)
    d2 = np.zeros(q.shape[0])
    nr = C.c_int32(0)
    dp = C.POINTER(C.c_double)
    _lib.check(_lib.load().se3icp_nn(device, q.ctypes.data_as(dp), q.shape[0], d.ctypes.data_as(dp), d.shape[0], dim,
                                     idx.ctypes.data_as(C.POINTER(C.c_int32)), d2.ctypes.data_as(dp), C.byref(nr)),
               "nn")
    return idx, d2, int(nr.value)


def set_lrf_seeding(mode: int, device: int = 0) -> None:
    _lib.check(_lib.load().se3icp_set_lrf_seeding(int(device), int(mode)), "set_lrf_seeding")


def last_seed_stats(device: int = 0) -> dict:
    out = (C.c_int64 * len(_lib.SEED_STATS))()
    _lib.check(_lib.load().se3icp_last_seed_stats(int(device), out, len(_lib.SEED_STATS)), "last_seed_stats")
    return {k: int(out[i]) for i, k in enumerate(_lib.SEED_STATS)}


def set_tree_sharing(mode: int, device: int = 0) -> None:
    _lib.check(_lib.load().se3icp_set_tree_sharing(int(device), int(mode)), "set_tree_sharing")


def last_tree_stats(device: int = 0) -> dict:
    out = (C.c_int64 * len(_lib.TREE_STATS))()
    _lib.check(_lib.load().se3icp_last_tree_stats(int(device), out, len(_lib.TREE_STATS)), "last_tree_stats")
    return {k: int(out[i]) for i, k in enumerate(_lib.TREE_STATS)}


def set_lrf_exact(mode, device: int = 0) -> None:
    _lib.check(_lib.load().se3icp_set_lrf_exact(device, int(mode)))


def set_nn_events(on: bool, device: int = 0) -> None:
    _lib.check(_lib.load().se3icp_set_nn_events(device, 1 if on else 0))


def set_profiling(on: bool, device: int = 0) -> None:
    _lib.check(_lib.load().se3icp_set_profiling(device, 1 if on else 0))


def last_kernel_times(device: int = 0) -> dict:
    keys = DeviceBatchRunner._KT_KEYS
    out = (C.c_double * len(keys))()
    _lib.check(_lib.load().se3icp_last_kernel_times_n(device, out, len(keys)))
    return dict(zip(keys, list(out)))
```

Measured before the change: 17920.

## Reuse donor kNN candidate lists for LRF queries in same-cloud seeded classes

Adds an LRF "taking" mode. When a seeded class shares its cloud, point count, k and tree donor group with its seed class, the donor's candidate lists are stored and reused. The dependent class then refines them under tightened error bounds instead of running a full kNN search. Default lrf_taking_=0 turns it on when lrf_seeding is 0 and tree donors are known. It adds a list buffer, a mask pass, two extra kernel launches and a redo/fallback path for queries whose bound check fails.

```diff
diff --git a/include/se3icp.h b/include/se3icp.h
--- a/include/se3icp.h
+++ b/include/se3icp.h
@@ -125,6 +125,10 @@
 #define SE3ICP_SEED_STATS_N 4
 int se3icp_last_seed_stats(int device, int64_t* out, int n);
 
+int se3icp_set_lrf_taking(int device, int mode);
+#define SE3ICP_TAKE_STATS_N 4
+int se3icp_last_take_stats(int device, int64_t* out, int n);
+
 int se3icp_set_tree_sharing(int device, int mode);
 #define SE3ICP_TREE_STATS_N 4
 int se3icp_last_tree_stats(int device, int64_t* out, int n);
diff --git a/se3-icp_amd/csrc/capi.cpp b/se3-icp_amd/csrc/capi.cpp
--- a/se3-icp_amd/csrc/capi.cpp
+++ b/se3-icp_amd/csrc/capi.cpp
@@ -446,6 +446,24 @@
     if (!e) return SE3ICP_ERR_NO_DEVICE;
     std::lock_guard<std::mutex> lk(e->mutex());
     for (int k = 0; k < 4; ++k) out[k] = e->seed_stats()[k];
+    return SE3ICP_OK;
+}
+
+int se3icp_set_lrf_taking(int device, int mode) {
+    if (mode < se3icp::kLrfTakingMin || mode > se3icp::kLrfTakingMax) return SE3ICP_ERR_INVALID_ARG;
+    Engine* e = usable_engine(device);
+    if (!e) return SE3ICP_ERR_NO_DEVICE;
+    std::lock_guard<std::mutex> lk(e->mutex());
+    e->set_lrf_taking(mode);
+    return SE3ICP_OK;
+}
+
+int se3icp_last_take_stats(int device, int64_t* out, int n) {
+    if (!out || n < se3icp::TS_COUNT) return SE3ICP_ERR_INVALID_ARG;
+    Engine* e = usable_engine(device);
+    if (!e) return SE3ICP_ERR_NO_DEVICE;
+    std::lock_guard<std::mutex> lk(e->mutex());
+    for (int k = 0; k < se3icp::TS_COUNT; ++k) out[k] = e->take_stats()[k];
     return SE3ICP_OK;
 }
 
diff --git a/se3-icp_amd/csrc/common.hpp b/se3-icp_amd/csrc/common.hpp
--- a/se3-icp_amd/csrc/common.hpp
+++ b/se3-icp_amd/csrc/common.hpp
@@ -9,6 +9,7 @@
 constexpr int kStatCols = 17;
 constexpr int kStatUseSe3 = 15, kStatUseR3 = 16;
 constexpr int kSeedStatCol = 14;
+constexpr int kTakeStatCol = 12;
 constexpr int kHist = 256;
 constexpr int kTrimList = 4096;
 constexpr int kTrimBlocks = 32;
diff --git a/se3-icp_amd/csrc/engine.cpp b/se3-icp_amd/csrc/engine.cpp
--- a/se3-icp_amd/csrc/engine.cpp
+++ b/se3-icp_amd/csrc/engine.cpp
@@ -478,31 +478,51 @@
             launch_lrf(v, knn_list_ ? 1 : 0, s);
             big(nullptr, nullptr, kSmallK);
         } else {
-            const bool seeding = seed_on_;
+            const bool seeding = seed_on_, taking = seed_on_ && take_on_;
             const int nt = nclouds_ + 1;
-            std::vector<int32_t> wb(2 * (size_t)nt, 0);
+            std::vector<int32_t> wb(3 * (size_t)nt, 0);
             for (int c = 0; c < nclouds_; ++c) {
                 const int waves = h_setup_[c].k_knn > 0 ? (h_clouds_[c].n + 7) / 8 : 0;
                 const bool sd = seeding && seed_ref_[c].load >= 0;
+                const bool tk = sd && taking && (take_flag_[c] & 2);
                 wb[c + 1] = wb[c] + (sd ? 0 : waves);
-                wb[nt + c + 1] = wb[nt + c] + (sd ? waves : 0);
+                wb[nt + c + 1] = wb[nt + c] + (sd && !tk ? waves : 0);
+                wb[2 * nt + c + 1] = wb[2 * nt + c] + (tk ? waves : 0);
             }
-            const int nw = wb[nclouds_], nw_sd = wb[nt + nclouds_];
-            if (!ensure<int32_t>(d_lrf_fb_, (size_t)8 * (nw + nw_sd) + 64) || !ensure<int32_t>(d_lrf_fbn_, 2 + 2 * (size_t)nt))
+            const int nw = wb[nclouds_], nw_sd = wb[nt + nclouds_], nw_tk = wb[2 * nt + nclouds_];
+            if (!ensure<int32_t>(d_lrf_fb_, (size_t)8 * ((size_t)nw + nw_sd + nw_tk) + 64) ||
+                !ensure<int32_t>(d_lrf_fbn_, 2 + 3 * (size_t)nt))
                 return SE3ICP_ERR_OUT_OF_MEMORY;
             int32_t* d_wb = (int32_t*)d_lrf_fbn_.p + 2;
             int32_t* fb = (int32_t*)d_lrf_fb_.p;
             int32_t* fbn = (int32_t*)d_lrf_fbn_.p;
             HIPCHK(hipMemsetAsync(fbn, 0, 2 * sizeof(int32_t), s));
-            HIPCHK(hipMemcpyAsync(d_wb, wb.data(), sizeof(int32_t) * 2 * nt, hipMemcpyHostToDevice, s));
+            HIPCHK(hipMemcpyAsync(d_wb, wb.data(), sizeof(int32_t) * 3 * nt, hipMemcpyHostToDevice, s));
             if (seeding) {
-                if (!ensure<float>(d_seed_, (size_t)seed_floats_) || !ensure<SeedRef>(d_seed_ref_, nclouds_))
+                const size_t nseed = (size_t)seed_floats_ * (taking ? 2 : 1);
+                if (!ensure<float>(d_seed_, nseed) || !ensure<SeedRef>(d_seed_ref_, nclouds_))
                     return SE3ICP_ERR_OUT_OF_MEMORY;
-                HIPCHK(hipMemsetAsync(d_seed_.p, 0xff, sizeof(float) * (size_t)seed_floats_, s));
+                HIPCHK(hipMemsetAsync(d_seed_.p, 0xff, sizeof(float) * nseed, s));
                 HIPCHK(hipMemcpyAsync(d_seed_ref_.p, seed_ref_.data(), sizeof(SeedRef) * nclouds_, hipMemcpyHostToDevice, s));
-                launch_lrf8(v, d_wb, 0, nw, fb, fbn, s, (const SeedRef*)d_seed_ref_.p, (float*)d_seed_.p, false, lrf_seeding_);
-                launch_lrf8(v, d_wb + nt, 0, nw_sd, fb, fbn, s, (const SeedRef*)d_seed_ref_.p, (float*)d_seed_.p, true,
-                            lrf_seeding_);
+                const SeedRef* sref = (const SeedRef*)d_seed_ref_.p;
+                float* sbuf = (float*)d_seed_.p;
+                TakeArgs tk{nullptr, nullptr, nullptr, 0, 0, 0};
+                if (taking && nw_tk > 0) {
+                    if (!ensure<uint32_t>(d_take_lists_, (size_t)seed_floats_ * (size_t)take_stride_) ||
+                        !ensure<int32_t>(d_take_flag_, nclouds_) || !ensure<unsigned char>(d_take_mask_, (size_t)nw_tk + 64))
+                        return SE3ICP_ERR_OUT_OF_MEMORY;
+                    HIPCHK(hipMemcpyAsync(d_take_flag_.p, take_flag_.data(), sizeof(int32_t) * nclouds_, hipMemcpyHostToDevice, s));
+                    HIPCHK(hipMemsetAsync(d_take_mask_.p, 0, (size_t)nw_tk + 64, s));
+                    tk = TakeArgs{(const int32_t*)d_take_flag_.p, (uint32_t*)d_take_lists_.p, nullptr, take_stride_,
+                                  (int32_t)seed_floats_, lrf_taking_};
+                }
+                launch_lrf8(v, d_wb, 0, nw, fb, fbn, s, sref, sbuf, false, lrf_seeding_, &tk);
+                launch_lrf8(v, d_wb + nt, 0, nw_sd, fb, fbn, s, sref, sbuf, true, lrf_seeding_);
+                if (tk.flag != nullptr) {
+                    tk.mask = (unsigned char*)d_take_mask_.p;
+                    launch_lrf8(v, d_wb + 2 * nt, 0, nw_tk, fb, fbn, s, sref, sbuf, true, lrf_seeding_, &tk, true);
+                    launch_lrf8(v, d_wb + 2 * nt, 0, nw_tk, fb, fbn, s, sref, sbuf, true, lrf_seeding_, &tk);
+                }
             } else {
                 launch_lrf8(v, d_wb, 0, nw, fb, fbn, s);
             }
@@ -539,6 +559,17 @@
         for (int i = 0; i < kStatSlots; ++i) q += h_lrf_stats_[kStatCols * i + kSeedStatCol + k];
         seed_stats_[1 + k] = (int64_t)q;
     }
+    {
+        unsigned long long t = 0, r = 0, f = 0;
+        for (int i = 0; i < kStatSlots; ++i) {
+            t += h_lrf_stats_[kStatCols * i + kTakeStatCol];
+            r += h_lrf_stats_[kStatCols * i + kTakeStatCol + 1] & 0xffffffffull;
+            f += h_lrf_stats_[kStatCols * i + kTakeStatCol + 1] >> 32;
+        }
+        take_stats_[TS_TAKEN] = (int64_t)t;
+        take_stats_[TS_REDONE] = (int64_t)r;
+        take_stats_[TS_FAILED] = (int64_t)f;
+    }
 #ifdef SE3ICP_PROF
     tree_prof_report();
     std::fprintf(stderr, "[prof] k_lrf cycles/query: knn|scan %.0f sort|tighten %.0f sums|final+sums %.0f finish %.0f "
@@ -591,6 +622,7 @@
     c->s = user_stream ? user_stream : stream_;
     ktimes_ = KernelTimes{};
     for (int64_t& x : seed_stats_) x = 0;
+    for (int64_t& x : take_stats_) x = 0;
     for (int64_t& x : tree_stats_) x = 0;
     tree_donor_.clear();
     HIPCHK(hipEventRecord(ev_[12], c->s));
@@ -825,12 +857,34 @@
             seed_stats_[0] = seeded;
             init_stats_[IS_CROSS_SEEDED] = cross;
             seed_on_ = true;
+            take_flag_.clear();
+            take_stride_ = 0;
+            if (lrf_seeding_ == 0 && lrf_taking_ != 1 && (int)tree_donor_.size() == U) {
+                std::vector<uint8_t> tk;
+                const int taking = graph_plan_takes(plan, sc, kk.data(), nn.data(), home.data(), tree_donor_, &tk);
+                int64_t kw_max = 0;
+                for (int k = 0; k < K; ++k)
+                    if (tk[k]) kw_max = std::max<int64_t>(kw_max, std::min<int64_t>(kk[k], nn[k]));
+                const int64_t stride = (std::min<int64_t>(kw_max, kSmallK) + 3) & ~(int64_t)3;
+                if (taking > 0 && 2 * seed_floats_ <= INT32_MAX) {
+                    take_flag_.assign(U, 0);
+                    for (int k = 0; k < K; ++k) {
+                        if (!tk[k]) continue;
+                        take_flag_[home[k]] |= 2;
+                        take_flag_[home[sc[k].from]] |= 1;
+                    }
+                    take_stride_ = (int)stride;
+                    take_stats_[TS_CLASSES] = taking;
+                    take_on_ = true;
+                }
+            }
         }
     }
     h_setup_ = sel_run_;
     HIPCHK(hipMemcpyAsync(d_setup_.p, sel_run_.data(), sizeof(CloudSetup) * U, hipMemcpyHostToDevice, s));
     const int rc = setup_knn(s);
     seed_on_ = false;
+    take_on_ = false;
     if (rc) return rc;
     HIPCHK(hipGetLastError());
     h_setup_ = sel_batch_;
diff --git a/se3-icp_amd/csrc/engine.hpp b/se3-icp_amd/csrc/engine.hpp
--- a/se3-icp_amd/csrc/engine.hpp
+++ b/se3-icp_amd/csrc/engine.hpp
@@ -75,6 +75,7 @@
     void set_batch_sharing(int level) { batch_sharing_ = level; }
     void set_lrf_seeding(int mode) { lrf_seeding_ = mode; }
     void set_tree_sharing(int mode) { tree_sharing_ = mode; }
+    void set_lrf_taking(int mode) { lrf_taking_ = mode; }
     const KernelTimes& kernel_times() const { return ktimes_; }
 
     int register_batch(int npairs, const double* const* src, const int64_t* ns, const double* const* tgt,
@@ -96,6 +97,7 @@
                          hipStream_t user_stream);
     const int64_t* graph_stats() const { return graph_stats_; }
     const int64_t* seed_stats() const { return seed_stats_; }
+    const int64_t* take_stats() const { return take_stats_; }
     const int64_t* tree_stats() const { return tree_stats_; }
 
     int knn_self(const double* xyz, int64_t n, int k, int32_t* idx);
@@ -220,6 +222,12 @@
     int64_t seed_floats_ = 0;
     DevBuf d_seed_{bufs_}, d_seed_ref_{bufs_};
     int64_t seed_stats_[4] = {};
+    int lrf_taking_ = 0;
+    bool take_on_ = false;
+    std::vector<int32_t> take_flag_;
+    int take_stride_ = 0;
+    DevBuf d_take_lists_{bufs_}, d_take_flag_{bufs_}, d_take_mask_{bufs_};
+    int64_t take_stats_[TS_COUNT] = {};
     std::vector<int32_t> tree_donor_;
     TreeTab tree_tab_a_{pins_, bufs_}, tree_tab_b_{pins_, bufs_}, tree_tab_12_{pins_, bufs_};
     int64_t tree_stats_[4] = {};
diff --git a/se3-icp_amd/csrc/graph.hpp b/se3-icp_amd/csrc/graph.hpp
--- a/se3-icp_amd/csrc/graph.hpp
+++ b/se3-icp_amd/csrc/graph.hpp
@@ -141,6 +141,31 @@
         ++seeded;
     }
     return seeded;
+}
+
+constexpr int kLrfTakingMin = 0, kLrfTakingMax = 2;
+enum TakeStat : int { TS_CLASSES = 0, TS_TAKEN, TS_REDONE, TS_FAILED, TS_COUNT };
+inline int32_t graph_plan_takes(const GraphPlan& plan, const std::vector<SeedClass>& seed, const int32_t* k_knn,
+                                const int64_t* n_pts, const int32_t* home, const std::vector<int32_t>& donor,
+                                std::vector<uint8_t>* take) {
+    const int32_t K = (int32_t)plan.classes.size();
+    take->assign((size_t)K, 0);
+    if (!plan.normalize || !plan.dedupe || (int32_t)seed.size() != K || donor.empty()) return 0;
+    const int32_t U = (int32_t)donor.size();
+    auto group = [&](int32_t u) { return (u < 0 || u >= U) ? -1 : (donor[u] >= 0 ? donor[u] : u); };
+    int32_t taking = 0;
+    for (int32_t k = 0; k < K; ++k) {
+        const int32_t a = seed[k].from;
+        if (a < 0 || a >= K || a == k) continue;
+        const int64_t kw = k_knn[k] < n_pts[k] ? k_knn[k] : n_pts[k], kwa = k_knn[a] < n_pts[a] ? k_knn[a] : n_pts[a];
+        const int32_t gk = group(home[k]), ga = group(home[a]);
+        if (plan.classes[k].cloud != plan.classes[a].cloud || n_pts[k] != n_pts[a] || kw != kwa || kw <= 0 || gk < 0 ||
+            gk != ga)
+            continue;
+        (*take)[k] = 1;
+        ++taking;
+    }
+    return taking;
 }
 
 constexpr int kPoseSeedingMin = 0, kPoseSeedingMax = 1;
diff --git a/se3-icp_amd/csrc/k_lrf8.hip b/se3-icp_amd/csrc/k_lrf8.hip
--- a/se3-icp_amd/csrc/k_lrf8.hip
+++ b/se3-icp_amd/csrc/k_lrf8.hip
@@ -5,6 +5,7 @@
 
 #include "devmath.hpp"
 #include "knn_util.hpp"
+#include "lrf_bounds.hpp"
 #include "tree.hpp"
 #include "view.hpp"
 #include "wave.hpp"
@@ -31,8 +32,6 @@
 constexpr int kStride = kCap + 4;
 static_assert(((kStride / 4) & 1) == 1, "an odd number of 16-B slots per list");
 constexpr int kLeaves = 64;
-constexpr unsigned kIdBits = 0xfffu;
-constexpr unsigned kAll = 0x7f7fffffu;
 constexpr unsigned kPad = 0xffffffffu;
 
 enum Park8 {
@@ -167,15 +166,6 @@
         if (e < len) list[e] = k[s];
     }
     __builtin_amdgcn_wave_barrier();
-}
-__device__ __forceinline__ float f32_err3(float d, float S) {
-    const float u = 5.9604645e-08f;
-    return 1.25f * (2.f * u * S * sqrtf(fmaxf(d, 0.f)) + 6.f * u * d + 4.f * u * u * S * S) + 1e-30f;
-}
-__device__ __forceinline__ unsigned widen_bound(unsigned t, float S) {
-    if (t >= 0x7f800000u) return kAll;
-    const float b = __uint_as_float(t);
-    return min((__float_as_uint(fmaf(2.02f, f32_err3(b, S), b)) + 2u) | kIdBits, kAll);
 }
 __device__ __forceinline__ int upper_count(const unsigned* A, int n, unsigned t) {
     int lo = 0, hi = n;
@@ -251,51 +241,21 @@
     return p3{xy.x, xy.y, z};
 }
 
-__device__ __forceinline__ bool final_group(unsigned* lists, const int* leaf_slot, const double4* __restrict__ P4,
+__device__ __forceinline__ bool final_exact(unsigned* list, const int (&slot)[16], bool bad0, const double4* __restrict__ P4,
                                             const int32_t* __restrict__ perm, double qx, double qy, double qz, int off,
-                                            int g, int l, int nbg, int mv, int fmode, int lim) {
-    unsigned* list = lists + g * kStride;
+                                            int g, int l, int nbg, int lim) {
     unsigned long long k[16];
-    bool unsorted = false;
-    {
-        unsigned k32[16];
-        if (fmode == 0) {
-            load_head<16>(list, nbg, l, k32);
-            sort8<16>(k32, l);
-        } else {
-            const int nb = nbg - mv;
-            unsigned* B = list + mv;
-            if (fmode == 1) sort_run<8>(B, nb, l);
-            load_head<16>(list, mv, l, k32);
-            if (fmode == 1) {
-#pragma unroll
-                for (int s = 0; s < 16; ++s) {
-                    const int e = l * 16 + s;
-                    if (e >= 128 - nb) k32[s] = B[127 - e];
-                }
-                __builtin_amdgcn_wave_barrier();
-                stage8<16, 128, 64>(k32, l);
-                stage8<16, 128, 32>(k32, l);
-                stage8<16, 128, 16>(k32, l);
-                stage8<16, 128, 8>(k32, l);
-                stage8<16, 128, 4>(k32, l);
-                stage8<16, 128, 2>(k32, l);
-                stage8<16, 128, 1>(k32, l);
-            }
-        }
-#pragma unroll
-        for (int s = 0; s < 16; ++s) {
-            const int e = l * 16 + s;
-            unsigned long long x = ~0ull;
-            if (e < nbg) {
-                const unsigned id = k32[s] & kIdBits;
-                const int slot = leaf_slot[id >> 6] + (int)(id & 63u);
-                const p3 p = ld3(P4, slot);
-                const unsigned key = __float_as_uint((float)l2_3(qx, qy, qz, p.x, p.y, p.z));
-                x = ((unsigned long long)key << 32) | (unsigned)(slot - off);
-            }
-            k[s] = x;
-        }
+    bool unsorted = bad0;
+#pragma unroll
+    for (int s = 0; s < 16; ++s) {
+        const int e = l * 16 + s;
+        unsigned long long x = ~0ull;
+        if (e < nbg) {
+            const p3 p = ld3(P4, slot[s]);
+            const unsigned key = __float_as_uint((float)l2_3(qx, qy, qz, p.x, p.y, p.z));
+            x = ((unsigned long long)key << 32) | (unsigned)(slot[s] - off);
+        }
+        k[s] = x;
     }
     auto ce = [](unsigned long long& a, unsigned long long& b) __attribute__((always_inline)) {
         const bool sw = b < a;
@@ -374,6 +334,46 @@
     return ok;
 }
 
+__device__ __forceinline__ bool final_group(unsigned* lists, const int* leaf_slot, const double4* __restrict__ P4,
+                                            const int32_t* __restrict__ perm, double qx, double qy, double qz, int off,
+                                            int g, int l, int nbg, int mv, int fmode, int lim) {
+    unsigned* list = lists + g * kStride;
+    {
+        unsigned k32[16];
+        if (fmode == 0) {
+            load_head<16>(list, nbg, l, k32);
+            sort8<16>(k32, l);
+        } else {
+            const int nb = nbg - mv;
+            unsigned* B = list + mv;
+            if (fmode == 1) sort_run<8>(B, nb, l);
+            load_head<16>(list, mv, l, k32);
+            if (fmode == 1) {
+#pragma unroll
+                for (int s = 0; s < 16; ++s) {
+                    const int e = l * 16 + s;
+                    if (e >= 128 - nb) k32[s] = B[127 - e];
+                }
+                __builtin_amdgcn_wave_barrier();
+                stage8<16, 128, 64>(k32, l);
+                stage8<16, 128, 32>(k32, l);
+                stage8<16, 128, 16>(k32, l);
+                stage8<16, 128, 8>(k32, l);
+                stage8<16, 128, 4>(k32, l);
+                stage8<16, 128, 2>(k32, l);
+                stage8<16, 128, 1>(k32, l);
+            }
+        }
+        int slot[16];
+#pragma unroll
+        for (int s = 0; s < 16; ++s) {
+            const unsigned id = k32[s] & kIdBits;
+            slot[s] = l * 16 + s < nbg ? leaf_slot[id >> 6] + (int)(id & 63u) : 0;
+        }
+        return final_exact(list, slot, false, P4, perm, qx, qy, qz, off, g, l, nbg, lim);
+    }
+}
+
 #ifdef SE3ICP_PROF
 #define PROF8_NOW(t) const unsigned long long t = __builtin_readcyclecounter()
 #define PROF8_ADD(acc, a, b) acc += (b) - (a)
@@ -384,13 +384,14 @@
 
 static_assert(kW >= 2 && kW * kQ <= 64, "the per-block epilogue: waves 0 and 1, a lane per query");
 
-template <bool SD, bool ST>
+template <bool SD, bool ST, bool TK = false>
 __global__ __launch_bounds__(64 * kW) __attribute__((amdgpu_waves_per_eu(kCap <= 192 ? 6 : (kCap <= 224 ? 5 : 4)))) void k_lrf8(
     View v, const int32_t* __restrict__ cloud_of, const CloudSetup* __restrict__ setup,
     const CloudDev* __restrict__ clouds, const float* __restrict__ tlo, const float* __restrict__ thi,
     const double4* __restrict__ P4, const int32_t* __restrict__ wave_base, int w_lo, int nwaves,
     int32_t* __restrict__ fb_list, int32_t* __restrict__ fb_count, const SeedRef* __restrict__ seed,
-    float* __restrict__ seedbuf, int seed_mode) {
+    float* __restrict__ seedbuf, int seed_mode, TakeArgs tk) {
+    static_assert(!TK || (SD && !ST), "a taking launch is a launch of seeded clouds");
     __shared__ __attribute__((aligned(16))) unsigned s_list[kW][kQ][kStride];
     auto park_of = [&](int w, int j) __attribute__((always_inline)) {
         return reinterpret_cast<double*>(&s_list[w][j][kParkAt]);
@@ -420,7 +421,20 @@
     CloudSetup st{};
     CloudDev cl{0, 0};
     int K = 0, Kw = 0;
-    if (wv < nwaves) {
+    bool redo_skip = false;
+    if constexpr (SD && !TK) {
+        if (tk.mask != nullptr) {
+            unsigned any = 0u;
+#pragma unroll
+            for (int j = 0; j < kW; ++j) {
+                const int wj = w_lo + bid * kW + j;
+                any |= wj < nwaves ? (unsigned)tk.mask[wj] : 0u;
+            }
+            if (any == 0u) return;
+            redo_skip = wv < nwaves && tk.mask[wv] == 0;
+        }
+    }
+    if (wv < nwaves && !redo_skip) {
         int lo = 0, hi = v.nclouds - 1;
         while (lo < hi) {
             const int mid = (lo + hi + 1) >> 1;
@@ -485,7 +499,9 @@
     }
     bool sd_open = false, sd_close = false, t_cert = true;
     unsigned n_sdq = 0, n_sda = 0, n_sdf = 0;
-    if constexpr (SD) {
+    unsigned n_tkq = 0, n_tkr = 0, n_tkf = 0;
+    if constexpr (SD && !TK) {
+        if (tk.mask != nullptr) n_tkr = (unsigned)qn;
         if (mode == 2) n_sda = (unsigned)qn;
         if (mode == 1) {
             const SeedRef sr = seed[c];
@@ -603,7 +619,7 @@
         return true;
     };
 
-    if (mode == 1) {
+    if (!TK && mode == 1) {
         const int lf0 = tree_node_of(w0 - cl.off, n, T.L), lf1 = tree_node_of(w0 + kQ - 1 - cl.off, n, T.L);
         const int nleaf = 1 << T.L;
         int s_lo = lf0, s_hi = lf1;
@@ -758,14 +774,64 @@
     PROF8_ADD(c_scan, t_a0, t_a1);
     const int kl = st.k_lrf, kn_want = st.k_nrm;
     const bool want_t = kl > 0, want_n = kn_want > 0;
+    if constexpr (TK) {
+        if (mode == 2) {
+            if (lane == 0) tk.mask[wv] = 1;
+            mode = 0;
+            fb_wave = false;
+        }
+    }
     bool fb_q = fb_wave;
-    const int nbg = (int)group_len();
+    const int nbg = TK ? (mode == 1 ? Kw : 0) : (int)group_len();
     const int nTop = min(Kw, nbg);
     const int kk = min(kl, nTop), kn = min(kn_want, nTop);
     const int wq = w0 + g;
     p3 qg{0.0, 0.0, 0.0};
     if (mode == 1) qg = ld3(P4, wq);
-    if (mode == 1 && !fb_wave) {
+    if constexpr (TK) {
+        if (mode == 1) {
+            const SeedRef sr = seed[c];
+            const size_t at = (size_t)sr.load + (size_t)(wq - cl.off);
+            float lb = seedbuf[(size_t)tk.lb_off + at];
+            if (tk.mode == 2) lb *= 0.5f;
+            const bool absent = !(bool)((int)(lb >= 0.f) & (int)(lb < INFINITY));
+            bool bad = absent;
+            const unsigned* src = tk.lists + at * (size_t)tk.stride;
+            int slot[16];
+#pragma unroll
+            for (int q4 = 0; q4 < 4; ++q4) {
+                const int e0 = l * 16 + 4 * q4;
+                uint4 x = make_uint4(0u, 0u, 0u, 0u);
+                if (e0 < Kw) x = *reinterpret_cast<const uint4*>(src + e0);
+                const unsigned xs[4] = {x.x, x.y, x.z, x.w};
+#pragma unroll
+                for (int i = 0; i < 4; ++i) {
+                    const bool in = (int)(e0 + i < Kw);
+                    const bool out = (bool)((int)in & (int)(xs[i] >= (unsigned)n));
+                    bad |= out;
+                    slot[4 * q4 + i] = cl.off + ((int)in & (int)!out ? (int)xs[i] : 0);
+                }
+            }
+            bool ok = final_exact(lists + g * kStride, slot, bad, P4, T.perm, qg.x, qg.y, qg.z, cl.off, g, l, nbg,
+                                  min(nbg, max(kk, kn) + 1));
+            __builtin_amdgcn_wave_barrier();
+            const p3 f = ld3(P4, (int)(ok ? lists[g * kStride + Kw - 1] : (unsigned)wq));
+            const double kb = l2_3(qg.x, qg.y, qg.z, f.x, f.y, f.z);
+            ok = (bool)((int)ok & (int)(kb < take_bound(sr.rho2, lb, s_norm)));
+            const unsigned long long failed = __ballot((int)!ok & (int)(l == 0));
+            if (failed != 0ull) {
+                if (lane == 0) tk.mask[wv] = 1;
+                n_tkf = (unsigned)__popcll(failed & ~__ballot(absent));
+                mode = 0;
+                n_q = 0;
+            } else {
+                n_cand += (unsigned)nbg;
+                n_tkq = kQ;
+                n_sdq = kQ;
+            }
+        }
+    }
+    if (!TK && mode == 1 && !fb_wave) {
         __builtin_amdgcn_wave_barrier();
         int fmode = 0;
         {
@@ -806,6 +872,33 @@
             if ((int)(so >= 0) & (int)mine & (int)(l == 0)) {
                 const p3 f = ld3(P4, (int)rl[Kw - 1]);
                 seedbuf[so + T.perm[wq]] = (float)l2_3(qg.x, qg.y, qg.z, f.x, f.y, f.z);
+            }
+            bool stores = false;
+            if (tk.flag != nullptr) stores = (bool)((int)(so >= 0) & (int)((tk.flag[c] & 1) != 0));
+            if ((int)stores & (int)mine) {
+                const size_t at = (size_t)so + (size_t)(wq - cl.off);
+                unsigned k[16];
+                load_head<16>(rl, Kw, l, k);
+                unsigned* dst = tk.lists + at * (size_t)tk.stride;
+#pragma unroll
+                for (int q4 = 0; q4 < 4; ++q4) {
+                    const int e0 = l * 16 + 4 * q4;
+                    const unsigned o = (unsigned)cl.off;
+                    if (e0 < Kw)
+                        *reinterpret_cast<uint4*>(dst + e0) =
+                            make_uint4(k[4 * q4] - o, k[4 * q4 + 1] - o, k[4 * q4 + 2] - o, k[4 * q4 + 3] - o);
+                }
+                if (l == 0) {
+                    unsigned tq = Tq[0];
+#pragma unroll
+                    for (int j = 1; j < kQ; ++j) tq = g == j ? Tq[j] : tq;
+                    float lb = narrow_bound(tq, s_norm);
+                    if (nbg > Kw) {
+                        const p3 f = ld3(P4, (int)rl[Kw]);
+                        lb = fminf(lb, key_floor((float)l2_3(qg.x, qg.y, qg.z, f.x, f.y, f.z)));
+                    }
+                    seedbuf[(size_t)tk.lb_off + at] = lb;
+                }
             }
         }
     }
@@ -895,6 +988,8 @@
             if (n_sdq) atomicAdd(ctr + kSeedStatCol, (unsigned long long)n_sdq);
             if (n_sda) atomicAdd(ctr + kSeedStatCol + 1, (unsigned long long)n_sda);
             if (n_sdf) atomicAdd(ctr + kSeedStatCol + 2, (unsigned long long)n_sdf);
+            if (n_tkq) atomicAdd(ctr + kTakeStatCol, (unsigned long long)n_tkq);
+            if (n_tkr | n_tkf) atomicAdd(ctr + kTakeStatCol + 1, (unsigned long long)n_tkr | ((unsigned long long)n_tkf << 32));
         }
     }
 
@@ -1025,18 +1120,23 @@
 }
 
 void launch_lrf8(const View& v, const int32_t* wave_base, int w_lo, int w_hi, int32_t* fb_list, int32_t* fb_count,
-                 hipStream_t s, const SeedRef* seed, float* seedbuf, bool seeded, int seed_mode) {
+                 hipStream_t s, const SeedRef* seed, float* seedbuf, bool seeded, int seed_mode, const TakeArgs* take,
+                 bool taking) {
     const int nb = (w_hi - w_lo + kW - 1) / kW;
     if (nb <= 0) return;
-    if (seeded)
+    const TakeArgs tk = take ? *take : TakeArgs{nullptr, nullptr, nullptr, 0, 0, 0};
+    if (taking)
+        hipLaunchKernelGGL((k_lrf8<true, false, true>), dim3(nb), dim3(64 * kW), 0, s, v, v.cloud_of, v.setup, v.clouds,
+                           v.t3.lo, v.t3.hi, v.t3.tpt64, wave_base, w_lo, w_hi, fb_list, fb_count, seed, seedbuf, seed_mode, tk);
+    else if (seeded)
         hipLaunchKernelGGL((k_lrf8<true, false>), dim3(nb), dim3(64 * kW), 0, s, v, v.cloud_of, v.setup, v.clouds, v.t3.lo,
-                           v.t3.hi, v.t3.tpt64, wave_base, w_lo, w_hi, fb_list, fb_count, seed, seedbuf, seed_mode);
+                           v.t3.hi, v.t3.tpt64, wave_base, w_lo, w_hi, fb_list, fb_count, seed, seedbuf, seed_mode, tk);
     else if (seed != nullptr)
         hipLaunchKernelGGL((k_lrf8<false, true>), dim3(nb), dim3(64 * kW), 0, s, v, v.cloud_of, v.setup, v.clouds, v.t3.lo,
-                           v.t3.hi, v.t3.tpt64, wave_base, w_lo, w_hi, fb_list, fb_count, seed, seedbuf, seed_mode);
+                           v.t3.hi, v.t3.tpt64, wave_base, w_lo, w_hi, fb_list, fb_count, seed, seedbuf, seed_mode, tk);
     else
         hipLaunchKernelGGL((k_lrf8<false, false>), dim3(nb), dim3(64 * kW), 0, s, v, v.cloud_of, v.setup, v.clouds, v.t3.lo,
-                           v.t3.hi, v.t3.tpt64, wave_base, w_lo, w_hi, fb_list, fb_count, seed, seedbuf, seed_mode);
-}
-
-}
+                           v.t3.hi, v.t3.tpt64, wave_base, w_lo, w_hi, fb_list, fb_count, seed, seedbuf, seed_mode, tk);
+}
+
+}
diff --git a/se3-icp_amd/csrc/lrf_bounds.hpp b/se3-icp_amd/csrc/lrf_bounds.hpp
--- /dev/null
+++ b/se3-icp_amd/csrc/lrf_bounds.hpp
@@ -0,0 +1,43 @@
+#pragma once
+#include <hip/hip_runtime.h>
+
+#include <cmath>
+#include <cstdint>
+
+namespace se3icp {
+namespace knn {
+
+constexpr unsigned kIdBits = 0xfffu;
+constexpr unsigned kAll = 0x7f7fffffu;
+
+__host__ __device__ __forceinline__ float bits_f32(unsigned u) { return __builtin_bit_cast(float, u); }
+__host__ __device__ __forceinline__ unsigned f32_bits(float f) { return __builtin_bit_cast(unsigned, f); }
+
+__host__ __device__ __forceinline__ float f32_err3(float d, float S) {
+    const float u = 5.9604645e-08f;
+    return 1.25f * (2.f * u * S * sqrtf(fmaxf(d, 0.f)) + 6.f * u * d + 4.f * u * u * S * S) + 1e-30f;
+}
+__host__ __device__ __forceinline__ unsigned widen_bound(unsigned t, float S) {
+    if (t >= 0x7f800000u) return kAll;
+    const float b = bits_f32(t);
+    const unsigned w = (f32_bits(fmaf(2.02f, f32_err3(b, S), b)) + 2u) | kIdBits;
+    return w < kAll ? w : kAll;
+}
+__host__ __device__ __forceinline__ float narrow_bound(unsigned t, float S) {
+    if (t >= kAll) return bits_f32(kAll);
+    const float b = bits_f32(t);
+    const float x = fmaf(-1.01f, f32_err3(b, S), b);
+    if (!(x > 0.f)) return 0.f;
+    const unsigned xb = f32_bits(x);
+    return xb > 2u ? bits_f32(xb - 2u) : 0.f;
+}
+__host__ __device__ __forceinline__ float key_floor(float key) { return key * 0.99999988079071044921875f; }
+
+__host__ __device__ __forceinline__ double take_bound(double rho2, float lb, float nb) {
+    double x = sqrt(rho2 * (double)lb) - 0x1p-48 * (double)nb;
+    x = x > 0.0 ? x : 0.0;
+    return (1.0 - 0x1p-40) * (x * x);
+}
+
+}
+}
diff --git a/se3-icp_amd/csrc/view.hpp b/se3-icp_amd/csrc/view.hpp
--- a/se3-icp_amd/csrc/view.hpp
+++ b/se3-icp_amd/csrc/view.hpp
@@ -106,9 +106,17 @@
 void launch_lrf(const View& v, int write_knn, hipStream_t s);
 void launch_lrf_list(const View& v, const int32_t* qlist, const int32_t* qcount, hipStream_t s, int qpw = 0);
 struct SeedRef { int32_t store; int32_t load; double rho2; };
+struct TakeArgs {
+    const int32_t* flag;
+    uint32_t* lists;
+    unsigned char* mask;
+    int32_t stride;
+    int32_t lb_off;
+    int32_t mode;
+};
 void launch_lrf8(const View& v, const int32_t* wave_base, int w_lo, int w_hi, int32_t* fb_list, int32_t* fb_count,
                  hipStream_t s, const SeedRef* seed = nullptr, float* seedbuf = nullptr, bool seeded = false,
-                 int seed_mode = 0);
+                 int seed_mode = 0, const TakeArgs* take = nullptr, bool taking = false);
 int knn_big_cap(int kw_max);
 int knn_big_blocks(int cap, int nq);
 void launch_knn_big(const View& v, int write_knn, int k_min, const int32_t* qlist, const int32_t* qcount, int nblocks,
diff --git a/se3-icp_amd/se3icp/__init__.py b/se3-icp_amd/se3icp/__init__.py
--- a/se3-icp_amd/se3icp/__init__.py
+++ b/se3-icp_amd/se3icp/__init__.py
@@ -13,7 +13,7 @@
                            expand_edges, last_graph_stats, register_graph, register_graph_device,
                            register_graph_report, register_graph_traced, register_sequence, sequence_edges,
                            set_batch_sharing, set_lrf_seeding, last_seed_stats,
-                           set_tree_sharing, last_tree_stats,
+                           set_tree_sharing, last_tree_stats, set_lrf_taking, last_take_stats,
                            voxel_downsample, voxel_downsample_device,
                            edge_inits, last_init_stats, set_pose_seeding, transform_device, transform_points)
 from ._lib import Report, ReportOptions
@@ -28,6 +28,7 @@
     "register_graph", "register_sequence", "sequence_edges", "expand_edges", "register_graph_device",
     "register_graph_report", "register_graph_traced", "last_graph_stats",
     "set_batch_sharing", "set_lrf_seeding", "last_seed_stats", "set_tree_sharing", "last_tree_stats",
+    "set_lrf_taking", "last_take_stats",
     "voxel_downsample", "voxel_downsample_device",
     "edge_inits", "transform_points", "transform_device", "set_pose_seeding", "last_init_stats",
 ]
diff --git a/se3-icp_amd/se3icp/_lib.py b/se3-icp_amd/se3icp/_lib.py
--- a/se3-icp_amd/se3icp/_lib.py
+++ b/se3-icp_amd/se3icp/_lib.py
@@ -32,6 +32,7 @@
     "se3icp_register_graph", "se3icp_register_graph_device", "se3icp_register_graph_report",
     "se3icp_register_graph_report_device", "se3icp_last_graph_stats", "se3icp_set_batch_sharing",
     "se3icp_set_lrf_seeding", "se3icp_last_seed_stats", "se3icp_set_tree_sharing", "se3icp_last_tree_stats",
+    "se3icp_set_lrf_taking", "se3icp_last_take_stats",
     "se3icp_report_version", "se3icp_register_batch_report", "se3icp_register_batch_report_device",
     "se3icp_register_sweep_report", "se3icp_register_sweep_report_device",
     "se3icp_request_report", "se3icp_get_report",
@@ -130,6 +131,7 @@
 GRAPH_STATS = ["clouds", "uses", "classes", "classes_full", "adopted", "rejected_order", "rejected_gap", "no_list",
                "bytes_uploaded"]
 SEED_STATS = ["classes_seeded", "queries_seeded", "queries_unseeded", "queries_failed"]
+TAKE_STATS = ["classes_taking", "queries_taken", "queries_redone", "queries_failed"]
 INIT_STATS = ["posed_edges", "posed_variants", "classes_seeded_across"]
 TREE_STATS = ["built_3d", "adopted_3d", "built_12d", "adopted_12d"]
 
diff --git a/se3-icp_amd/se3icp/registration.py b/se3-icp_amd/se3icp/registration.py
--- a/se3-icp_amd/se3icp/registration.py
+++ b/se3-icp_amd/se3icp/registration.py
@@ -794,6 +794,16 @@
     return {k: int(out[i]) for i, k in enumerate(_lib.SEED_STATS)}
 
 
+def set_lrf_taking(mode: int, device: int = 0) -> None:
+    _lib.check(_lib.load().se3icp_set_lrf_taking(int(device), int(mode)), "set_lrf_taking")
+
+
+def last_take_stats(device: int = 0) -> dict:
+    out = (C.c_int64 * len(_lib.TAKE_STATS))()
+    _lib.check(_lib.load().se3icp_last_take_stats(int(device), out, len(_lib.TAKE_STATS)), "last_take_stats")
+    return {k: int(out[i]) for i, k in enumerate(_lib.TAKE_STATS)}
+
+
 def set_tree_sharing(mode: int, device: int = 0) -> None:
     _lib.check(_lib.load().se3icp_set_tree_sharing(int(device), int(mode)), "set_tree_sharing")
 
```

Result: faster. 18540, median of 6 (+3.4%).
